# RinceWND/extPOM

Measured on AMD Instinct MI355X. Metric: 3D cell-updates/sec on internal mode (one internal step = the 3-D baroclinic step and its isplit 2-D external substeps; whole-step wall time), higher is better.
Workload: dtype f64

## Files before the change

### extpom_amd/csrc/k_adv.hip

```cpp
#include "pomgpu_internal.hpp"

#define dt_(i, j) F2(dt, i, j)
#define dx_(i, j) F2(dx, i, j)
#define dy_(i, j) F2(dy, i, j)
#define h_(i, j) F2(h, i, j)
#define u_(i, j, k) F3(u, i, j, k)
#define v_(i, j, k) F3(v, i, j, k)
#define ub_(i, j, k) F3(ub, i, j, k)
#define vb_(i, j, k) F3(vb, i, j, k)
#define w_(i, j, k) F3(w, i, j, k)
#define aam_(i, j, k) F3(aam, i, j, k)

#define MARCH3(call)                                                                  \
  const int g_ = (int)(blockIdx.x * blockDim.x + threadIdx.x);    \
  const int L_ = g_ >> 6, xcd_ = L_ & 7, m_ = L_ >> 3;                                \
  const int bpl_ = P.g_bpl, nbx_ = P.g_nbx;                                           \
  const int p_ = m_ % bpl_, t_ = m_ / bpl_;                                           \
  const int k = t_ % P.kb + 1;                                                        \
  const int band_ = (t_ / P.kb) * 8 + xcd_;                                           \
  const int i = (p_ % nbx_) * 64 + (g_ & 63) + 1;                                     \
  const int j = band_ * P.g_rb + (p_ / nbx_) * 4 + (int)threadIdx.y + 1;              \
  if (i > P.iml || j > P.jml) return;                                                 \
  call;
__device__ __forceinline__ void c_advct_a(const KP &P, const int i, const int j, const int k);
// ... 286 lines not shown
  G3(a, i, j, k) = G3(a, i, j, k) * G2(m2, i, j);
}
__device__ __forceinline__ void c_smol(const KP &P, const int i, const int j, const int k, const double *ff);
__global__ void k_smol(KP P, const double *ff) {
  MARCH3(c_smol(P, i, j, k, ff))
}
__device__ __forceinline__ void c_smol(const KP &P, const int i, const int j, const int k, const double *ff) {
  if (i > P.im || j > P.jm) return;
  const double value_min = 1.e-9, epsilon = 1.0e-14;
  double *xm = P.s3[0], *ym = P.s3[1], *zw = P.s3[2];
  const double fc = G3(ff, i, j, k);
  if (k <= P.kbm1 && j >= 2 && j <= P.jmm1 && i >= 2) {
    const double fw = G3(ff, i - 1, j, k);
    double r = 0.;
    if (!(fc < value_min || fw < value_min)) {
      const double m = G3(xm, i, j, k);
      const double udx = fabs(m);
      const double u2dt = P.dti2 * m * m * 2. / (F2(aru, i, j) * (dt_(i - 1, j) + dt_(i, j)));
      const double mol = (fc - fw) / (fw + fc + epsilon);
      r = (udx - u2dt) * mol * P.sw;
      if (fabs(udx) < fabs(u2dt)) r = 0.;
    }
    G3(xm, i, j, k) = r;
  }
  if (k <= P.kbm1 && j >= 2 && i >= 2 && i <= P.imm1) {
    const double fs = G3(ff, i, j - 1, k);
    double r = 0.;
    if (!(fc < value_min || fs < value_min)) {
      const double m = G3(ym, i, j, k);
      const double vdy = fabs(m);
      const double v2dt = P.dti2 * m * m * 2. / (F2(arv, i, j) * (dt_(i, j - 1) + dt_(i, j)));
      const double mol = (fc - fs) / (fs + fc + epsilon);
      r = (vdy - v2dt) * mol * P.sw;
      if (fabs(vdy) < fabs(v2dt)) r = 0.;
    }
    G3(ym, i, j, k) = r;
  }
  if (k >= 2 && k <= P.kbm1 && i >= 2 && i <= P.imm1 && j >= 2 && j <= P.jmm1) {
    const double fu = G3(ff, i, j, k - 1);
    double r = 0.;
    if (!(fc < value_min || fu < value_min)) {
      const double m = G3(zw, i, j, k);
      const double wdz = fabs(m);
      const double w2dt = P.dti2 * m * m / (F1(dzz, k - 1) * dt_(i, j));
      const double mol = (fu - fc) / (fc + fu + epsilon);
      r = (wdz - w2dt) * mol * P.sw;
      if (fabs(wdz) < fabs(w2dt)) r = 0.;
    }
    G3(zw, i, j, k) = r;
  }
}
__device__ __forceinline__ void c_copy3(const KP &P, const int i, const int j, const int k, double *dst, const double *src);
__global__ void k_copy3(KP P, double *dst, const double *src) {
  MARCH3(c_copy3(P, i, j, k, dst, src))
}
__device__ __forceinline__ void c_copy3(const KP &P, const int i, const int j, const int k, double *dst, const double *src) {
  G3(dst, i, j, k) = G3(src, i, j, k);
}
__device__ __forceinline__ double advt2_xdiff(const KP &P, const double *fb, const double *fc, int i, int j, int k) {
  const double am = 0.5 * (aam_(i, j, k) + aam_(i - 1, j, k));
  return -am * (h_(i, j) + h_(i - 1, j)) * P.tprni *
         ((G3(fb, i, j, k) - G3(fc, i, j, k)) - (G3(fb, i - 1, j, k) - G3(fc, i - 1, j, k))) * F2(dum, i, j) *
         (dy_(i, j) + dy_(i - 1, j)) * 0.5 / (dx_(i, j) + dx_(i - 1, j));
}
__device__ __forceinline__ double advt2_ydiff(const KP &P, const double *fb, const double *fc, int i, int j, int k) {
  const double am = 0.5 * (aam_(i, j, k) + aam_(i, j - 1, k));
  return -am * (h_(i, j) + h_(i, j - 1)) * P.tprni *
         ((G3(fb, i, j, k) - G3(fc, i, j, k)) - (G3(fb, i, j - 1, k) - G3(fc, i, j - 1, k))) * F2(dvm, i, j) *
         (dx_(i, j) + dx_(i, j - 1)) * 0.5 / (dy_(i, j) + dy_(i, j - 1));
}
__device__ __forceinline__ void c_advt2_diff(const KP &P, const int i, const int j, const int k, const double *fb, const double *fc, double *ff);
__global__ void k_advt2_diff(KP P, const double *fb, const double *fc, double *ff) {
  MARCH3(c_advt2_diff(P, i, j, k, fb, fc, ff))
}
__device__ __forceinline__ void c_advt2_diff(const KP &P, const int i, const int j, const int k, const double *fb, const double *fc, double *ff) {
  if (k > P.kbm1 || i < 2 || i > P.imm1 || j < 2 || j > P.jmm1) return;
  G3(ff, i, j, k) = G3(ff, i, j, k) -
                    P.dti2 * (advt2_xdiff(P, fb, fc, i + 1, j, k) - advt2_xdiff(P, fb, fc, i, j, k) +
                              advt2_ydiff(P, fb, fc, i, j + 1, k) - advt2_ydiff(P, fb, fc, i, j, k)) /
                        ((h_(i, j) + F2(etf, i, j)) * F2(art, i, j));
}

__device__ __forceinline__ double dens_point(const KP &P, double si, double ti, int i, int j, int k);
template <int TAU> __device__ __forceinline__ void c_ts_update(const KP &P, const int i, const int j, const int k, double fold, double fnew, int rt, int store_rst, double tau_b, double tau_f);
template <int TAU> __global__ void k_ts_update(KP P, double fold, double fnew, int rt, int store_rst, double tau_b, double tau_f) {
  MARCH3(c_ts_update<TAU>(P, i, j, k, fold, fnew, rt, store_rst, tau_b, tau_f))
}
__global__ void k_ts_update_same(KP P, double fold, double fnew, int rt, int store_rst) {
  MARCH3(c_ts_update<2>(P, i, j, k, fold, fnew, rt, store_rst, 0., 0.))
}
template <int TAU> __device__ __forceinline__ void c_ts_update(const KP &P, const int i, const int j, const int k, double fold, double fnew, int rt, int store_rst, double tau_b, double tau_f) {
  const bool act = (i <= P.im && j <= P.jm), lev = (k <= P.kbm1);
  const pomgpu_ct m = F2(fsm, i, j);
  pomgpu_ct uf = F3(uf, i, j, k), vf = F3(vf, i, j, k);
  if (lev && act) {
    uf = uf * m;
    vf = vf * m;
  }
  pomgpu_ct tb = F3(tb, i, j, k), sb = F3(sb, i, j, k);
  if (rt) {
    const pomgpu_ct tc = F3(tclim, i, j, k), sc = F3(sclim, i, j, k);
    tb = (tb - tc) + tc;
    sb = (sb - sc) + sc;
  }
  const pomgpu_ct t0 = F3(t, i, j, k), s0 = F3(s, i, j, k);
  pomgpu_ct tbn = t0 + CT(.5) * CT(P.smoth) * (uf + tb - CT(2.) * t0);
  pomgpu_ct sbn = s0 + CT(.5) * CT(P.smoth) * (vf + sb - CT(2.) * s0);
  pomgpu_ct tn = uf, sn = vf;
  if (lev) {
    if (act) {
      const pomgpu_ct tr = CT(fold) * CT(F3(trstrb, i, j, k)) + CT(fnew) * CT(F3(trstrf, i, j, k));
      const pomgpu_ct sr = CT(fold) * CT(F3(srstrb, i, j, k)) + CT(fnew) * CT(F3(srstrf, i, j, k));
      pomgpu_ct ta;
      if (TAU == 1) ta = CT(fold) * CT(tau_b) + CT(fnew) * CT(tau_f);
      else if (TAU == 2) { const pomgpu_ct x = CT(F3(taurstrf, i, j, k)); ta = CT(fold) * x + CT(fnew) * x; }
      else ta = CT(fold) * CT(F3(taurstrb, i, j, k)) + CT(fnew) * CT(F3(taurstrf, i, j, k));
      if (store_rst) {
        F3(trstr, i, j, k) = tr;
        F3(srstr, i, j, k) = sr;
        F3(taurstr, i, j, k) = ta;
      }
      const pomgpu_ct c = CT(2.) * CT(P.dti) / CT(86400.);
      tn = tn + c * ta * (tr - tn);
      tbn = tbn + c * ta * (tr - tbn);
      sn = sn + c * ta * (sr - sn);
      sbn = sbn + c * ta * (sr - sbn);
    }
    tn = tn * m; tbn = tbn * m; sn = sn * m; sbn = sbn * m;
  }
  F3(t, i, j, k) = tn;
  F3(tb, i, j, k) = tbn;
  F3(s, i, j, k) = sn;
  F3(sb, i, j, k) = sbn;
  if (lev && act) F3(rho, i, j, k) = dens_point(P, sn, tn, i, j, k);
}
template <int NF> struct TrUpds { TrUpd u[NF]; };
template <int NF> __device__ __forceinline__ void c_tr_update(const KP &P, const int i, const int j, const int k, const TrUpds<NF> &A, int rt) {
  const bool msk = (i <= P.im && j <= P.jm && k <= P.kbm1);
  const double m = F2(fsm, i, j);
#pragma unroll
  for (int f = 0; f < NF; f++) {
    const TrUpd &u = A.u[f];
    double ff = G3(u.ff, i, j, k);
    if (msk) ff = ff * m;
    double fb = G3(u.fb, i, j, k);
    if (rt) {
      const double fc = G3(u.fc, i, j, k);
      fb = (fb - fc) + fc;
    }
    const double f0 = G3(u.f, i, j, k);
    G3(u.fb, i, j, k) = f0 + .5 * P.smoth * (ff + fb - 2. * f0);
    G3(u.f, i, j, k) = ff;
  }
}
template <int NF> __global__ void k_tr_update(KP P, TrUpds<NF> A, int rt) {
  MARCH3(c_tr_update<NF>(P, i, j, k, A, rt))
}
__device__ __forceinline__ void c_tr_source(const KP &P, const int i, const int j, const int k, double *ff, const double *fb, const double *fc, const double *q, double lam) {
  if (k > P.kbm1 || i > P.im || j > P.jm) return;
  double x = G3(fb, i, j, k);
  if (fc) { const double y = G3(fc, i, j, k); x = (x - y) + y; }
  const double a = lam * x;
  const double b = (q ? (double)G3(q, i, j, k) : 0.) - a;
  const double d = P.dti2 * b;
  G3(ff, i, j, k) = (double)G3(ff, i, j, k) + d;
}
__global__ void k_tr_source(KP P, double *ff, const double *fb, const double *fc, const double *q, double lam) {
  MARCH3(c_tr_source(P, i, j, k, ff, fb, fc, q, lam))
}
__device__ __forceinline__ void c_mask_ts(const KP &P, const int i, const int j, const int k);
__global__ void k_mask_ts(KP P) {
  MARCH3(c_mask_ts(P, i, j, k))
}
__device__ __forceinline__ void c_mask_ts(const KP &P, const int i, const int j, const int k) {
  if (k > P.kbm1 || i > P.im || j > P.jm) return;
  const double m = F2(fsm, i, j);
  F3(uf, i, j, k) = F3(uf, i, j, k) * m;
  F3(vf, i, j, k) = F3(vf, i, j, k) * m;
}
__device__ __forceinline__ void c_mask_uv(const KP &P, const int i, const int j, const int k);
__global__ void k_mask_uv(KP P) {
  MARCH3(c_mask_uv(P, i, j, k))
}
// ... 304 lines not shown
  const int iw = ia > 1 ? ia - 1 : 1, ie = ib < P.iml ? ib + 1 : P.iml;
  const double2 dx = *(const double2 *)&F2(dx, ia, j), dy = *(const double2 *)&F2(dy, ia, j);
#ifndef AAM_PLAIN_DIV
  const double2 rdx = *(const double2 *)&K2(RDX, ia, j), rdy = *(const double2 *)&K2(RDY, ia, j);
  const InvD dxa = {dx.x, rdx.x}, dya = {dy.x, rdy.x}, dxb = {dx.y, rdx.y}, dyb = {dy.y, rdy.y};
#endif
  auto lev = [&](int k) {
    AamLev L;
    L.u_s = LD2(A3(u), ia, j - 1, k); L.u_0 = LD2(A3(u), ia, j, k); L.u_n = LD2(A3(u), ia, j + 1, k);
    L.v_0 = LD2(A3(v), ia, j, k); L.v_n = LD2(A3(v), ia, j + 1, k);
    return L;
  };
  AamLev cur = lev(k0);
  for (int k = k0; k <= k1; k++) {
    const AamLev nxt = lev(k < k1 ? k + 1 : k1);
    const double2 u_s = cur.u_s, u_0 = cur.u_0, u_n = cur.u_n, v_0 = cur.v_0, v_n = cur.v_n;
    const double uE_s = halo_e(u_s.x, [&] { return u_(ie, j - 1, k); }), uE_0 = halo_e(u_0.x, [&] { return u_(ie, j, k); }),
                 uE_n = halo_e(u_n.x, [&] { return u_(ie, j + 1, k); });
    const double vE_0 = halo_e(v_0.x, [&] { return v_(ie, j, k); }), vE_n = halo_e(v_n.x, [&] { return v_(ie, j + 1, k); });
    const double vW_0 = halo_w(v_0.y, [&] { return v_(iw, j, k); }), vW_n = halo_w(v_n.y, [&] { return v_(iw, j + 1, k); });
#ifndef AAM_PLAIN_DIV
    const double aa = aam_point_r(P, dxa, dya, u_0.x, u_0.y, u_n.x, u_n.y, u_s.x, u_s.y, v_0.x, v_n.x, v_0.y, v_n.y, vW_0, vW_n);
    const double ab = aam_point_r(P, dxb, dyb, u_0.y, uE_0, u_n.y, uE_n, u_s.y, uE_s, v_0.y, v_n.y, vE_0, vE_n, v_0.x, v_n.x);
#else
    const double aa = aam_point(P, dx.x, dy.x, u_0.x, u_0.y, u_n.x, u_n.y, u_s.x, u_s.y, v_0.x, v_n.x, v_0.y, v_n.y, vW_0, vW_n);
    const double ab = aam_point(P, dx.y, dy.y, u_0.y, uE_0, u_n.y, uE_n, u_s.y, uE_s, v_0.y, v_n.y, vE_0, vE_n, v_0.x, v_n.x);
#endif
    if (out && ia0 >= 2 && ia0 <= P.imm1) F3(aam, ia0, j, k) = aa;
    if (out && ia0 + 1 <= P.imm1) F3(aam, ia0 + 1, j, k) = ab;
    cur = nxt;
  }
}
#undef LD2
#undef A3


void launch_advct_a(pomgpu_ctx *c) { LAUNCH(c, k_advct_a, gridm(c->P), blk2(), c->P); }
void launch_advct_b(pomgpu_ctx *c) { LAUNCH(c, k_advct_b, gridm(c->P), blk2(), c->P); }
void launch_advct_c(pomgpu_ctx *c) { LAUNCH(c, k_advct_c, gridm(c->P), blk2(), c->P); }
void launch_aam(pomgpu_ctx *c) {
  const KP &P = c->P;
#ifdef POMGPU_STORE_F32
  const bool pair_ok = false;
#else
  const bool pair_ok = true;
#endif
  if (pair_ok && P.iml % 2 == 0 && !SW(c, NO_PAIR)) {
    const long nbands = (P.jml + P.g_rb - 1) / P.g_rb, rounds = (nbands + 7) / 8;
    const long bpl = (long)((P.iml / 2 + 61) / 62) * (P.g_rb / 4);
    const long nch = (P.kbm1 + AAM_KCH - 1) / AAM_KCH;
    LAUNCHN(c, "k_aam_pair", k_aam_pair, dim3((unsigned)(8 * rounds * nch * bpl), 1, 1), blk2(), c->P);
  } else {
    LAUNCH(c, k_aam, gridm(c->P), blk2(), c->P);
  }
}
void launch_roundtrip(pomgpu_ctx *c, double *a, const double *b, int fix_kb) { LAUNCH(c, k_roundtrip, gridm(c->P), blk2(), c->P, a, b, fix_kb); }
void launch_roundtrip_level(pomgpu_ctx *c, double *a, const double *b, int k) { LAUNCH(c, k_roundtrip_level, grid2(c->P), blk2(), c->P, a, b, k); }
void launch_advq_flux(pomgpu_ctx *c, const double *q, const double *qb, double *xf, double *yf) {
  LAUNCH(c, k_advq_flux, gridm(c->P), blk2(), c->P, q, qb, xf, yf);
}
void launch_advq_step(pomgpu_ctx *c, const double *q, const double *qb, double *qf, const double *xf, const double *yf, int zero_else) {
  LAUNCH(c, k_advq_step, gridm(c->P), blk2(), c->P, q, qb, qf, xf, yf, zero_else);
}
void launch_q_filter(pomgpu_ctx *c, int mask) { LAUNCH(c, k_q_filter, gridm(c->P), blk2(), c->P, mask); }
void launch_q_filter_rim(pomgpu_ctx *c) {
  const KP &P = c->P;
  const int len = P.im > P.jm ? P.im : P.jm;
  LAUNCH(c, k_q_filter_rim, dim3((len + 63) / 64, 8, P.kb), dim3(64, 1, 1), c->P);
}
void launch_mask_q(pomgpu_ctx *c) { LAUNCH(c, k_mask_q, gridm(c->P), blk2(), c->P); }
void launch_advt1(pomgpu_ctx *c, double *fb, double *f, const double *fclim, double *ff) {
  LAUNCH(c, k_advt1, gridm(c->P), blk2(), c->P, (const double *)fb, (const double *)f, fclim, ff);
  LAUNCH(c, k_copy_kb, grid2(c->P), blk2(), c->P, f, (double *)NULL);
}
void launch_copy_kb(pomgpu_ctx *c, double *f, double *g) { LAUNCH(c, k_copy_kb, grid2(c->P), blk2(), c->P, f, g); }
void launch_advt2_mass(pomgpu_ctx *c) { LAUNCH(c, k_advt2_mass, gridm(c->P), blk2(), c->P); }
void launch_advt2_step(pomgpu_ctx *c, const double *fbmem, const double *f, const double *eta, double *ff, int itera) {
  LAUNCH(c, k_advt2_step, gridm(c->P), blk2(), c->P, fbmem, f, eta, ff, itera);
}
void launch_mask3(pomgpu_ctx *c, double *a, const double *m2) { LAUNCH(c, k_mask3, gridm(c->P), blk2(), c->P, a, m2); }
void launch_smol(pomgpu_ctx *c, const double *ff) { LAUNCH(c, k_smol, gridm(c->P), blk2(), c->P, ff); }
void launch_copy3(pomgpu_ctx *c, double *dst, const double *src) { LAUNCH(c, k_copy3, gridm(c->P), blk2(), c->P, dst, src); }
void launch_advt2_diff(pomgpu_ctx *c, const double *fb, const double *fc, double *ff) { LAUNCH(c, k_advt2_diff, gridm(c->P), blk2(), c->P, fb, fc, ff); }
void launch_ts_update(pomgpu_ctx *c, double fold, double fnew, int rt, int store_rst) {
  if (c->tau_known[0] && c->tau_known[1] && !c->tau_handed && !SW(c, TAU_ARRAYS))
    LAUNCHN(c, "k_ts_update", (k_ts_update<1>), gridm(c->P), blk2(), c->P, fold, fnew, rt, store_rst, c->tau_val[0], c->tau_val[1]);
  else if (c->tau_same && !c->tau_handed && !SW(c, TAU_ARRAYS))
    LAUNCH(c, k_ts_update_same, gridm(c->P), blk2(), c->P, fold, fnew, rt, store_rst);
  else
    LAUNCHN(c, "k_ts_update", (k_ts_update<0>), gridm(c->P), blk2(), c->P, fold, fnew, rt, store_rst, 0., 0.);
}
void launch_restore_fields(pomgpu_ctx *c, double fold, double fnew) { LAUNCH(c, k_restore_fields, gridm(c->P), blk2(), c->P, fold, fnew); }
void launch_mask_ts(pomgpu_ctx *c) { LAUNCH(c, k_mask_ts, gridm(c->P), blk2(), c->P); }
void launch_tr_update(pomgpu_ctx *c, const TrUpd *u, int nf, int rt) {
  if (nf == 2) {
    TrUpds<2> A; A.u[0] = u[0]; A.u[1] = u[1];
    LAUNCHN(c, "k_tr_update2", (k_tr_update<2>), gridm(c->P), blk2(), c->P, A, rt);
  } else {
    TrUpds<1> A; A.u[0] = u[0];
    LAUNCHN(c, "k_tr_update", (k_tr_update<1>), gridm(c->P), blk2(), c->P, A, rt);
  }
}
void launch_tr_source(pomgpu_ctx *c, double *ff, const double *fb, const double *fc, const double *q, double lam) {
  LAUNCH(c, k_tr_source, gridm(c->P), blk2(), c->P, ff, fb, fc, q, lam);
}
void launch_mask_uv(pomgpu_ctx *c) { LAUNCH(c, k_mask_uv, gridm(c->P), blk2(), c->P); }
void launch_mask_w(pomgpu_ctx *c) { LAUNCH(c, k_mask_w, gridm(c->P), blk2(), c->P); }
void launch_restore(pomgpu_ctx *c, double fold, double fnew) { LAUNCH(c, k_restore, gridm(c->P), blk2(), c->P, fold, fnew); }
void launch_restore_shift(pomgpu_ctx *c) { LAUNCH(c, k_restore_shift, gridm(c->P), blk2(), c->P); }
void launch_restore_load(pomgpu_ctx *c, const double *tr, const double *sr, double tau, const double *taur, int fill_tau) { LAUNCH(c, k_restore_load, gridm(c->P), blk2(), c->P, tr, sr, tau, taur, fill_tau); }
void launch_probe_gpow15(pomgpu_ctx *c, long n, const double *x, double *out) { LAUNCH(c, k_probe_gpow15, dim3((unsigned)((n + 255) / 256), 1, 1), dim3(256, 1, 1), n, x, out); }
void launch_dens(pomgpu_ctx *c, const double *si, const double *ti, double *rhoo) { LAUNCH(c, k_dens, gridm(c->P), blk2(), c->P, si, ti, rhoo); }
void launch_realvertvl(pomgpu_ctx *c, int etf_is_et) {
  if (SW(c, REALVERTVL_CELLS)) LAUNCH(c, k_realvertvl, gridm(c->P), blk2(), c->P, etf_is_et);
  else LAUNCHN(c, "k_realvertvl_col", k_realvertvl_col, grid2(c->P), blk2(), c->P, etf_is_et);
}
```

### extpom_amd/csrc/k_tile.hip

```cpp
#include "pomgpu_internal.hpp"


__global__ void k_coef_static(KP P) {
  const int i = TID_I, j = TID_J;
  if (i > P.iml || j > P.jml) return;
  const int iw = i > 1 ? i - 1 : 1, js = j > 1 ? j - 1 : 1;
  P.m8[IX2(i, j)] = (unsigned char)((F2(fsm, i, j) != 0. ? 1 : 0) | (F2(dum, i, j) != 0. ? 2 : 0) | (F2(dvm, i, j) != 0. ? 4 : 0));
  K2(HSX, i, j) = F2(h, i, j) + F2(h, iw, j);
  K2(HSY, i, j) = F2(h, i, j) + F2(h, i, js);
  K2(DYSX, i, j) = F2(dy, i, j) + F2(dy, iw, j);
  K2(DXSX, i, j) = F2(dx, i, j) + F2(dx, iw, j);
  K2(DXSY, i, j) = F2(dx, i, j) + F2(dx, i, js);
  K2(DYSY, i, j) = F2(dy, i, j) + F2(dy, i, js);
  K2(DX4, i, j) = F2(dx, i, j) + F2(dx, iw, j) + F2(dx, i, js) + F2(dx, iw, js);
  K2(DY4, i, j) = F2(dy, i, j) + F2(dy, iw, j) + F2(dy, i, js) + F2(dy, iw, js);
  const int ie = i < P.iml ? i + 1 : P.iml, jn = j < P.jml ? j + 1 : P.jml;
  K2(CVA, i, j) = F2(dy, ie, j) - F2(dy, iw, j);
  K2(CVB, i, j) = F2(dx, i, jn) - F2(dx, i, js);
  K2(R2DXSX, i, j) = 2.0 / (F2(dx, i, j) + F2(dx, iw, j));
  K2(R2DYSY, i, j) = 2.0 / (F2(dy, i, j) + F2(dy, i, js));
  K2(RDX, i, j) = 1.0 / F2(dx, i, j);
  K2(RDY, i, j) = 1.0 / F2(dy, i, j);
  if (j == 1)
    for (int n = i - 1; n < POM_NBLK1D * P.kb; n += P.iml) P.r1[n] = 1.0 / P.b1[n];
}
__global__ void k_coef_dt(KP P) {
  const int i = TID_I, j = TID_J;
  if (i > P.iml || j > P.jml) return;
  const int iw = i > 1 ? i - 1 : 1, js = j > 1 ? j - 1 : 1;
  K2(CMX, i, j) = 0.25 * (F2(dy, iw, j) + F2(dy, i, j)) * (F2(dt, iw, j) + F2(dt, i, j));
  K2(CMY, i, j) = 0.25 * (F2(dx, i, js) + F2(dx, i, j)) * (F2(dt, i, js) + F2(dt, i, j));
  K2(DTSX, i, j) = F2(dt, i, j) + F2(dt, iw, j);
  K2(DTSY, i, j) = F2(dt, i, j) + F2(dt, i, js);
  K2(DT4, i, j) = F2(dt, i, j) + F2(dt, iw, j) + F2(dt, i, js) + F2(dt, iw, js);
}
__global__ void k_coef_eta(KP P, int uvm) {
  const int i = TID_I, j = TID_J;
  if (i > P.iml || j > P.jml) return;
  K2(HEA, i, j) = (F2(h, i, j) + F2(etb, i, j)) * F2(art, i, j);
  K2(HFA, i, j) = (F2(h, i, j) + F2(etf, i, j)) * F2(art, i, j);
  if (uvm) {
    const unsigned long long mb = UVM_MARK;
    double mark;
    __builtin_memcpy(&mark, &mb, sizeof mark);
    const int iw = i > 1 ? i - 1 : 1, js = j > 1 ? j - 1 : 1;
    const double cu = (F2(utb, i, j) + F2(utf, i, j)) / (F2(dt, i, j) + F2(dt, iw, j));
    const double cv = (F2(vtb, i, j) + F2(vtf, i, j)) / (F2(dt, i, j) + F2(dt, i, js));
    K2(UCOR, i, j) = (i >= 2 && i <= P.im && j <= P.jm) ? cu : mark;
    K2(VCOR, i, j) = (j >= 2 && j <= P.jm && i <= P.im) ? cv : mark;
  }
}

__device__ __forceinline__ pomgpu_ct upw_(pomgpu_ct m, pomgpu_ct lo, pomgpu_ct hi) {
  return CT(0.5) * ((m + fabs(m)) * lo + (m - fabs(m)) * hi);
}
struct FaceT { pomgpu_ct adv, dif; };
struct TFields { const double *fb[2], *f[2], *fcl[2]; double *ff[2]; };
template <int NF> struct LevT { pomgpu_ct c[2 * NF + 2], o[2], h[ROWSHARE_SLOTS(2 * NF + 2)]; };
template <int NS> struct NbrT { pomgpu_ct s[NS], n[NS]; };
struct CoefT { pomgpu_ct cm, hs, msk, ds_num; InvDc den; };
__device__ __forceinline__ CoefT coef_x(const KP &P, int i, int j) {
  CoefT c; c.cm = K2(CMX, i, j); c.hs = K2(HSX, i, j); c.msk = F2(dum, i, j); c.ds_num = K2(DYSX, i, j); c.den = inv_of(CT(K2(DXSX, i, j))); return c;
}
__device__ __forceinline__ CoefT coef_y(const KP &P, int i, int j) {
  CoefT c; c.cm = K2(CMY, i, j); c.hs = K2(HSY, i, j); c.msk = F2(dvm, i, j); c.ds_num = K2(DXSY, i, j); c.den = inv_of(CT(K2(DYSY, i, j))); return c;
}
__device__ __forceinline__ FaceT advt2_face(const pomgpu_ct tprni, const CoefT &c, pomgpu_ct vel, pomgpu_ct fb_hi, pomgpu_ct fb_lo, pomgpu_ct fc_hi,
                                            pomgpu_ct fc_lo, pomgpu_ct am_hi, pomgpu_ct am_lo) {
  FaceT f;
  f.adv = upw_(c.cm * vel, fb_lo, fb_hi);
  const pomgpu_ct am = CT(0.5) * (am_hi + am_lo);
  f.dif = divi(-am * c.hs * tprni * ((fb_hi - fc_hi) - (fb_lo - fc_lo)) * c.msk * c.ds_num * CT(0.5), c.den);
  return f;
}
#if COL_WX != 1
#error "the row-sharing column kernels keep one wavefront per workgroup row (COL_WX == 1)"
#endif
template <int NF, bool UM = false>
__global__ void __launch_bounds__(64 * LDS_ROWS) k_advt2_col(KP P, TFields A) {
  constexpr int NS = 2 * NF + 2, NH = ROWSHARE_SLOTS(NS), AM = 2 * NF, VV = 2 * NF + 1;
  HALO_XCD_DECODE_R(LDS_ROWS)
  const int r = WAVE_UNIFORM((int)threadIdx.y), j0w = j - r;
  const bool jrow = j <= P.jml;
  const int jc = jrow ? j : P.jml;
  const bool icol = jrow && (lane >= 1 && lane <= 62 && i0 <= P.iml);
#ifdef POMGPU_EMU
  if (!icol) return;
#endif
  const int i = i0 < 1 ? 1 : (i0 > P.iml ? P.iml : i0);
  const int iw = i > 1 ? i - 1 : 1, ie = i < P.iml ? i + 1 : P.iml;
  const int js = jc > 1 ? jc - 1 : 1, jn = jc < P.jml ? jc + 1 : P.jml;
  const bool in = icol && (i >= 2 && i <= P.imm1 && jc >= 2 && jc <= P.jmm1);
  const pomgpu_ct fsm = F2(fsm, i, jc);
  const CoefT cw = coef_x(P, i, jc), cs = coef_y(P, i, jc), cn = coef_y(P, i, jn);
  const pomgpu_ct art = F2(art, i, jc), hea = K2(HEA, i, jc);
  const InvDc hfa = inv_of(CT(K2(HFA, i, jc)));
  const pomgpu_ct tprni = P.tprni, dti2 = P.dti2;
  BufA bs[NS], bo[2], bff[NF], bh[NH];
  const double *ps[NS];
#pragma unroll
  for (int f = 0; f < NF; f++) { ps[f] = A.fb[f]; ps[NF + f] = A.fcl[f]; bff[f] = BUF3(A.ff[f]); }
  ps[AM] = A3(aam); ps[VV] = A3(v); bo[0] = BUF3(A3(u)); bo[1] = BUF3(A3(w));
#pragma unroll
  for (int x = 0; x < NS; x++) bs[x] = BUF3(ps[x]);
  const RowShare<NS> S = rowshare_setup<NS>(P, r, j, j0w, i);
#pragma unroll
  for (int q = 0; q < NH; q++) bh[q] = BUF3(rowshare_pick<NS>(ps, S.hop[q]));
  const UvmC mu = UM ? uvm_of<0>(P, i, jc) : uvm_none(), mv = UM ? uvm_of<1>(P, i, jc) : uvm_none();
  UvmC mh[NH];
#pragma unroll
  for (int q = 0; q < NH; q++) mh[q] = UM ? rowshare_uvm<1, NS, LDS_ROWS>(P, S, q, VV, j0w, i) : uvm_none();
  const unsigned oc = BOFF2(i, jc), lvb = LVB;
  const unsigned ost = in ? oc : BOFF_NONE;
#ifndef POMGPU_EMU
  __shared__ pomgpu_ct slab[2][NS][ROWSHARE_ROWS][64];
#else
  const unsigned os = BOFF2(i, js), on = BOFF2(i, jn);
#endif
  auto load = [&](LevT<NF> &L, unsigned lv) {
#pragma unroll
    for (int x = 0; x < NS; x++) L.c[x] = bldc(bs[x], oc, lv);
    L.o[0] = bldc(bo[0], oc, lv); L.o[1] = bldc(bo[1], oc, lv);
#pragma unroll
    for (int q = 0; q < NH; q++) L.h[q] = bldc(bh[q], S.hoff[q], lv);
  };
  pomgpu_ct f1[NF];
#pragma unroll
  for (int f = 0; f < NF; f++) f1[f] = G3(A.f[f], i, jc, 1);
  const int kbm1 = P.kbm1;
  pomgpu_ct p_adv[NF], p_dif[NF], p_fb[NF], p_zu[NF];
#pragma unroll
  for (int f = 0; f < NF; f++) p_adv[f] = p_dif[f] = p_fb[f] = p_zu[f] = 0.;
  auto step = [&](const int L, const int par, const LevT<NF> &cur, LevT<NF> &nxt) {
    load(nxt, (unsigned)(L < kbm1 ? L : kbm1 - 1) * lvb);
    NbrT<NS> nb;
    const pomgpu_ct v_c = uvm_fix(cur.c[VV], mv);
#ifndef POMGPU_EMU
#pragma unroll
    for (int x = 0; x < NS; x++) slab[par][x][r + 1][lane] = x == VV ? v_c : cur.c[x];
#pragma unroll
    for (int q = 0; q < NH; q++) slab[par][S.hop[q]][S.hrow[q]][lane] = uvm_fix(cur.h[q], mh[q]);
    __syncthreads();
#pragma unroll
    for (int x = 0; x < NS; x++) { nb.s[x] = slab[par][x][S.ss][lane]; nb.n[x] = slab[par][x][S.sn][lane]; }
#else
    const unsigned lvc = (unsigned)((L <= kbm1 ? L : kbm1) - 1) * lvb;
#pragma unroll
    for (int x = 0; x < NS; x++) { nb.s[x] = bldc(bs[x], os, lvc); nb.n[x] = bldc(bs[x], on, lvc); }
    nb.s[VV] = uvm_fix(nb.s[VV], uvm_of<1>(P, i, js)); nb.n[VV] = uvm_fix(nb.n[VV], uvm_of<1>(P, i, jn));
#endif
    const pomgpu_ct am_c = cur.c[AM], u_c = uvm_fix(cur.o[0], mu), w_c = cur.o[1];
    const pomgpu_ct am_w = halo_w(am_c, [&] { return F3(aam, iw, jc, L); });
    InvDc dzk; dzk.b = dzk.y = 0.;
    if (L >= 2) { dzk.b = F1(dz, L - 1); dzk.y = R1(dz, L - 1); }
#pragma unroll
    for (int f = 0; f < NF; f++) {
      const pomgpu_ct fb_c = cur.c[f], fc_c = cur.c[NF + f];
      pomgpu_ct zu = 0.;
      pomgpu_ct s_adv = 0., s_dif = 0.;
      if (L <= kbm1) {
        const pomgpu_ct fb_w = halo_w(fb_c, [&] { return G3(A.fb[f], iw, jc, L); });
        const pomgpu_ct fc_w = halo_w(fc_c, [&] { return G3(A.fcl[f], iw, jc, L); });
        const FaceT xw = advt2_face(tprni, cw, u_c, fb_c, fb_w, fc_c, fc_w, am_c, am_w);
        auto east = [&] {
          return advt2_face(tprni, coef_x(P, ie, jc), uvm_ld<0>(P, ie, jc, L), G3(A.fb[f], ie, jc, L), fb_c, G3(A.fcl[f], ie, jc, L), fc_c,
                            F3(aam, ie, jc, L), am_c);
        };
        FaceT xe;
        xe.adv = halo_e(xw.adv, [&] { return east().adv; });
        xe.dif = halo_e(xw.dif, [&] { return east().dif; });
        const FaceT ys = advt2_face(tprni, cs, v_c, fb_c, nb.s[f], fc_c, nb.s[NF + f], am_c, nb.s[AM]);
        const FaceT yn = advt2_face(tprni, cn, nb.n[VV], nb.n[f], fb_c, nb.n[NF + f], fc_c, nb.n[AM], am_c);
        s_adv = xe.adv - xw.adv + yn.adv - ys.adv;
        s_dif = xe.dif - xw.dif + yn.dif - ys.dif;
        zu = (L == 1) ? w_c * f1[f] * art : upw_(w_c, fb_c, p_fb[f]) * art;
      }
      {
        pomgpu_ct rr = p_adv[f] + divi(p_zu[f] - zu, dzk);
        rr = divi(p_fb[f] * hea - dti2 * rr, hfa);
        rr = rr * fsm;
        rr = rr - divi(dti2 * p_dif[f], hfa);
        bstc(bff[f], (L >= 2 && L <= kbm1 + 1) ? ost : BOFF_NONE, (unsigned)(L >= 2 ? L - 2 : 0) * lvb, rr);
      }
      p_adv[f] = s_adv; p_dif[f] = s_dif; p_fb[f] = fb_c; p_zu[f] = zu;
    }
  };
  LevT<NF> ra, rb;
  load(ra, 0u);
  rb = ra;
  for (int L = 1; L <= kbm1 + 1; L += 2) {
    step(L, 1, ra, rb);
    step(L + 1, 0, rb, ra);
  }
  if (icol) {
    for (int k = in ? P.kb : 1; k <= P.kb; k++) {
#pragma unroll
      for (int f = 0; f < NF; f++) G3(A.ff[f], i, jc, k) = CT(G3(A.ff[f], i, jc, k)) * fsm;
    }
  }
}

struct QFields { const double *q[2], *qb[2]; double *qf[2]; };
template <int NF, int NO = 2> struct LevQa { pomgpu_ct c[2 * NF + 2], o[NO], h[ROWSHARE_SLOTS(2 * NF + 2)]; };
struct CoefQ { pomgpu_ct dts, hs, msk, ds_num; InvDc den; };
__device__ __forceinline__ CoefQ coefq_x(const KP &P, int i, int j) {
  CoefQ c; c.dts = K2(DTSX, i, j); c.hs = K2(HSX, i, j); c.msk = F2(dum, i, j); c.den = inv_of(CT(K2(DXSX, i, j))); c.ds_num = K2(DYSX, i, j); return c;
}
__device__ __forceinline__ CoefQ coefq_y(const KP &P, int i, int j) {
  CoefQ c; c.dts = K2(DTSY, i, j); c.hs = K2(HSY, i, j); c.msk = F2(dvm, i, j); c.den = inv_of(CT(K2(DYSY, i, j))); c.ds_num = K2(DXSY, i, j); return c;
}
__device__ __forceinline__ pomgpu_ct advq_face(const CoefQ &c, pomgpu_ct q_hi, pomgpu_ct q_lo, pomgpu_ct vel_k, pomgpu_ct vel_km1, pomgpu_ct am_hi_k,
                                               pomgpu_ct am_lo_k, pomgpu_ct am_hi_m, pomgpu_ct am_lo_m, pomgpu_ct qb_hi, pomgpu_ct qb_lo) {
  pomgpu_ct x = CT(.125) * (q_hi + q_lo) * c.dts * (vel_k + vel_km1);
  x = x - divi(CT(.25) * (am_hi_k + am_lo_k + am_hi_m + am_lo_m) * c.hs * (qb_hi - qb_lo) * c.msk, c.den);
  return CT(.5) * c.ds_num * x;
}
template <int NF, bool WF = false, bool UM = false>
__global__ void __launch_bounds__(64 * LDS_ROWS) k_advq_col(KP P, QFields A, int zero_else) {
  constexpr int NS = 2 * NF + 2, NH = ROWSHARE_SLOTS(NS), AM = 2 * NF, VV = 2 * NF + 1;
  typedef LevQa<NF, WF ? 1 : 2> Lev;
  HALO_XCD_DECODE_R(LDS_ROWS)
  const int r = WAVE_UNIFORM((int)threadIdx.y), j0w = j - r;
  const bool jrow = j <= P.jml;
  const int jc = jrow ? j : P.jml;
  const bool icol = jrow && (lane >= 1 && lane <= 62 && i0 <= P.iml);
#ifdef POMGPU_EMU
  if (!icol) return;
#endif
  const int i = i0 < 1 ? 1 : (i0 > P.iml ? P.iml : i0);
  const int iw = i > 1 ? i - 1 : 1, ie = i < P.iml ? i + 1 : P.iml;
  const int js = jc > 1 ? jc - 1 : 1, jn = jc < P.jml ? jc + 1 : P.jml;
  const bool in = icol && (i >= 2 && i <= P.imm1 && jc >= 2 && jc <= P.jmm1);
  const CoefQ cw = coefq_x(P, i, jc), cs = coefq_y(P, i, jc), cn = coefq_y(P, i, jn);
  const pomgpu_ct art = F2(art, i, jc), hea = K2(HEA, i, jc);
  const InvDc hfa = inv_of(CT(K2(HFA, i, jc)));
  const int kb = P.kb, kbm1 = P.kbm1;
  BufA bs[NS], bo[2], bqf[NF], bh[NH];
// ... 510 lines not shown
    bstc(buf, ost, lv, ru);
    bstc(bvf, ost, lv, rv);
    fu_k = fu_n; fv_k = fv_n;
    u_k = u_c; v_k = v_c;
  };
  LevUV ra, rb;
  load(ra, 1);
  rb = ra;
  for (int k = 1; k <= kbm1; k += 6) {
    step(k, 1, ra, rb);
    if (k + 1 <= kbm1) step(k + 1, 2, rb, ra);
    if (k + 2 <= kbm1) step(k + 2, 0, ra, rb);
    if (k + 3 <= kbm1) step(k + 3, 1, rb, ra);
    if (k + 4 <= kbm1) step(k + 4, 2, ra, rb);
    if (k + 5 <= kbm1) step(k + 5, 0, rb, ra);
  }
  if (out) { F3(uf, i, jc, kb) = 0.; F3(vf, i, jc, kb) = 0.; }
}

void launch_coef_static(pomgpu_ctx *c) { LAUNCH(c, k_coef_static, grid2(c->P), blk2(), c->P); }
void launch_coef_dt(pomgpu_ctx *c) { LAUNCH(c, k_coef_dt, grid2(c->P), blk2(), c->P); }
void launch_coef_eta(pomgpu_ctx *c, int uvm) { LAUNCH(c, k_coef_eta, grid2(c->P), blk2(), c->P, uvm); }
void launch_advq_col(pomgpu_ctx *c, const double *q, const double *qb, double *qf, int zero_else) {
  QFields A; A.q[0] = A.q[1] = q; A.qb[0] = A.qb[1] = qb; A.qf[0] = A.qf[1] = qf;
  LAUNCHN(c, "k_advq_col", (k_advq_col<1>), grid1_halo_r(c->P, LDS_ROWS), blk_col_r(LDS_ROWS), c->P, A, zero_else);
}
void launch_advq2_col(pomgpu_ctx *c, const double *q, const double *qb, double *qf, const double *ql, const double *qlb, double *qlf, int zero_else) {
  QFields A; A.q[0] = q; A.qb[0] = qb; A.qf[0] = qf; A.q[1] = ql; A.qb[1] = qlb; A.qf[1] = qlf;
  LAUNCHN(c, "k_advq2_col", (k_advq_col<2>), grid1_halo_r(c->P, LDS_ROWS), blk_col_r(LDS_ROWS), c->P, A, zero_else);
}
#if POMGPU_W_FUSE
void launch_advq2w_col(pomgpu_ctx *c, const double *q, const double *qb, double *qf, const double *ql, const double *qlb, double *qlf, int zero_else) {
  QFields A; A.q[0] = q; A.qb[0] = qb; A.qf[0] = qf; A.q[1] = ql; A.qb[1] = qlb; A.qf[1] = qlf;
#if POMGPU_UVM_ONLOAD
  if (c->P.uvm) { LAUNCHN(c, "k_advq2_col", (k_advq_col<2, true, true>), grid1_halo_r(c->P, LDS_ROWS), blk_col_r(LDS_ROWS), c->P, A, zero_else); return; }
#endif
  LAUNCHN(c, "k_advq2_col", (k_advq_col<2, true>), grid1_halo_r(c->P, LDS_ROWS), blk_col_r(LDS_ROWS), c->P, A, zero_else);
}
#endif
void launch_advct_col(pomgpu_ctx *c, int sum2d) {
  const bool rows4 = SW(c, ADVCT_ROWS4) || (!SW(c, ADVCT_ROWS8) && c->P.jml <= 400 && c->exch);
  sum2d = (sum2d ? 1 : 0) | (POMGPU_UVM_ONLOAD && !c->exch && !c->tp.on && !c->wide.on && !(c->flags & POMGPU_CTX_2D) ? 2 : 0);
  if (rows4) LAUNCHN(c, "k_advct_col", (k_advct_col<4>), grid1_halo_r(c->P, 4), blk_col_r(4), c->P, sum2d);
  else LAUNCHN(c, "k_advct_col", (k_advct_col<LDS_ROWS>), grid1_halo_r(c->P, LDS_ROWS), blk_col_r(LDS_ROWS), c->P, sum2d);
}
__global__ void k_advct_fix2d(KP P, int west, int south) {
  const int t = TID_I;
  if (west && t >= 2 && t <= P.jmm1) {
    double a = 0.;
#pragma unroll 8
    for (int k = 1; k <= P.kbm1; k++) a = a + F3(advx, 2, t, k) * F1(dz, k);
    F2(adx2d, 2, t) = a;
  }
  if (south && t >= 2 && t <= P.imm1) {
    double a = 0.;
#pragma unroll 8
    for (int k = 1; k <= P.kbm1; k++) a = a + F3(advy, t, 2, k) * F1(dz, k);
    F2(ady2d, t, 2) = a;
  }
}
void launch_advct_fix2d(pomgpu_ctx *c, int west, int south) {
  const KP &P = c->P;
  const int len = P.im > P.jm ? P.im : P.jm;
  LAUNCH(c, k_advct_fix2d, dim3((len + 63) / 64, 1, 1), dim3(64, 1, 1), c->P, west, south);
}
void launch_advct_edge(pomgpu_ctx *c, double *to_e, double *to_n) {
  const KP &P = c->P;
  const int len = P.im > P.jm ? P.im : P.jm;
  LAUNCH(c, k_advct_edge, dim3((len + 63) / 64, P.kbm1, 1), dim3(64, 1, 1), c->P, to_e, to_n);
}
void launch_advct_fix(pomgpu_ctx *c, const double *from_w, const double *from_s) {
  const KP &P = c->P;
  const int len = P.im > P.jm ? P.im : P.jm;
  LAUNCH(c, k_advct_fix, dim3((len + 63) / 64, P.kbm1, 1), dim3(64, 1, 1), c->P, from_w, from_s);
}
void launch_advuv_col(pomgpu_ctx *c) {
#if POMGPU_UVM_ONLOAD
  if (c->P.uvm) { LAUNCHN(c, "k_advuv_col", (k_advuv_col<true>), grid1_halo_r(c->P, LDS_ROWS), blk_col_r(LDS_ROWS), c->P); return; }
#endif
  LAUNCHN(c, "k_advuv_col", (k_advuv_col<false>), grid1_halo_r(c->P, LDS_ROWS), blk_col_r(LDS_ROWS), c->P);
}
void launch_advt2_rows(pomgpu_ctx *c, const double *fb, const double *f, const double *fc, double *ff) {
  {
    TFields A; A.fb[0] = A.fb[1] = fb; A.f[0] = A.f[1] = f; A.fcl[0] = A.fcl[1] = fc; A.ff[0] = A.ff[1] = ff;
#if POMGPU_UVM_ONLOAD
    if (c->P.uvm) { LAUNCHN(c, "k_advt2_col", (k_advt2_col<1, true>), grid1_halo_r(c->P, LDS_ROWS), blk_col_r(LDS_ROWS), c->P, A); return; }
#endif
    LAUNCHN(c, "k_advt2_col", (k_advt2_col<1>), grid1_halo_r(c->P, LDS_ROWS), blk_col_r(LDS_ROWS), c->P, A);
  }
}
void launch_advt2x2_col(pomgpu_ctx *c, const double *tb, const double *t, const double *tc, double *tf, const double *sb, const double *s_,
                        const double *sc, double *sf) {
  TFields A; A.fb[0] = tb; A.f[0] = t; A.fcl[0] = tc; A.ff[0] = tf; A.fb[1] = sb; A.f[1] = s_; A.fcl[1] = sc; A.ff[1] = sf;
#if POMGPU_UVM_ONLOAD
  if (c->P.uvm) { LAUNCHN(c, "k_advt2x2_col", (k_advt2_col<2, true>), grid1_halo_r(c->P, LDS_ROWS), blk_col_r(LDS_ROWS), c->P, A); return; }
#endif
  LAUNCHN(c, "k_advt2x2_col", (k_advt2_col<2>), grid1_halo_r(c->P, LDS_ROWS), blk_col_r(LDS_ROWS), c->P, A);
}
```

### extpom_amd/csrc/k_vert.hip

```cpp
#include <type_traits>
#include "pomgpu_internal.hpp"
#include "dd_exp.h"

#define dt_(i, j) F2(dt, i, j)
#define dx_(i, j) F2(dx, i, j)
#define dy_(i, j) F2(dy, i, j)
#define h_(i, j) F2(h, i, j)
#define u_(i, j, k) F3(u, i, j, k)
#define v_(i, j, k) F3(v, i, j, k)
#define w_(i, j, k) F3(w, i, j, k)

#define ROWS_PROFUV 1
#define ROWS_PROFT 1
#ifndef ROWS_UVF
#define ROWS_UVF 8
#endif
#ifndef ROWS_UVM
#define ROWS_UVM 4
#endif
#define COL2                               \
  const int i = TID_I, j = TID_J;          \
  if (i > P.iml || j > P.jml) return;

__global__ void k_baropg(KP P, int sum2d) {
  COL2
  if (i < 2 || i > P.imm1 || j < 2 || j > P.jmm1) {
    if (sum2d) {
      double rx = 0., ry = 0.;
      if (i <= P.im && j <= P.jm)
        for (int k = 1; k <= P.kbm1; k++) {
          const double dzk = F1(dz, k);
          rx = rx + F3(drhox, i, j, k) * dzk;
          ry = ry + F3(drhoy, i, j, k) * dzk;
        }
      F2(drx2d, i, j) = rx;
      F2(dry2d, i, j) = ry;
    }
    return;
  }
  const double dtc = dt_(i, j), dtw = dt_(i - 1, j), dts = dt_(i, j - 1);
  const double sx = .25 * (dtc + dtw), sy = .25 * (dtc + dts);
  const double mx = F2(dum, i, j), my = F2(dvm, i, j);
  const double ex = dy_(i, j) + dy_(i - 1, j), ey = dx_(i, j) + dx_(i, j - 1);
  double rc0 = F3(rho, i, j, 1) - F3(rmean, i, j, 1);
  double rw0 = F3(rho, i - 1, j, 1) - F3(rmean, i - 1, j, 1);
  double rs0 = F3(rho, i, j - 1, 1) - F3(rmean, i, j - 1, 1);
  double ax = .5 * P.grav * (-F1(zz, 1)) * (dtc + dtw) * (rc0 - rw0);
  double ay = .5 * P.grav * (-F1(zz, 1)) * (dtc + dts) * (rc0 - rs0);
  double ox = P.ramp * (sx * ax * mx * ex), oy = P.ramp * (sy * ay * my * ey);
  F3(drhox, i, j, 1) = ox;
  F3(drhoy, i, j, 1) = oy;
  double rx = 0., ry = 0.;
  rx = rx + ox * F1(dz, 1);
  ry = ry + oy * F1(dz, 1);
  for (int k = 2; k <= P.kbm1; k++) {
    PACE_BARRIER();
    const double rc = F3(rho, i, j, k) - F3(rmean, i, j, k);
    const double rw = F3(rho, i - 1, j, k) - F3(rmean, i - 1, j, k);
    const double rs = F3(rho, i, j - 1, k) - F3(rmean, i, j - 1, k);
    const double zm = F1(zz, k - 1) - F1(zz, k), zp = F1(zz, k - 1) + F1(zz, k);
    ax = ax + P.grav * .25 * zm * (dtc + dtw) * (rc - rw + rc0 - rw0) +
         P.grav * .25 * zp * (dtc - dtw) * (rc + rw - rc0 - rw0);
    ay = ay + P.grav * .25 * zm * (dtc + dts) * (rc - rs + rc0 - rs0) +
         P.grav * .25 * zp * (dtc - dts) * (rc + rs - rc0 - rs0);
    ox = P.ramp * (sx * ax * mx * ex); oy = P.ramp * (sy * ay * my * ey);
    F3(drhox, i, j, k) = ox;
    F3(drhoy, i, j, k) = oy;
    rx = rx + ox * F1(dz, k);
    ry = ry + oy * F1(dz, k);
    rc0 = rc; rw0 = rw; rs0 = rs;
  }
  if (sum2d) { F2(drx2d, i, j) = rx; F2(dry2d, i, j) = ry; }
  F3(drhox, i, j, P.kb) = P.ramp * F3(drhox, i, j, P.kb);
  F3(drhoy, i, j, P.kb) = P.ramp * F3(drhoy, i, j, P.kb);
}

#ifndef BPG_ROWS
#define BPG_ROWS 16
#endif
static_assert(COL_WX == 1, "k_baropg_rs / k_vertvl_rs take threadIdx.y as the row inside the workgroup: one wavefront per workgroup row");
__global__ void __launch_bounds__(64 * BPG_ROWS) k_baropg_rs(KP P, int sum2d) {
  HALO_XCD_DECODE_R(BPG_ROWS)
  const int r = WAVE_UNIFORM((int)threadIdx.y);
  const bool jvalid = j <= P.jml;
  const int jc = jvalid ? j : P.jml;
  const bool own = jvalid && lane >= 1 && lane <= 62 && i0 >= 1 && i0 <= P.iml;
#ifdef POMGPU_EMU
  if (!own) return;
#endif
  const int i = i0 < 1 ? 1 : (i0 > P.iml ? P.iml : i0);
  const int iw = i > 1 ? i - 1 : 1, js = jc > 1 ? jc - 1 : 1;
  const bool in = own && i0 >= 2 && i0 <= P.imm1 && jc >= 2 && jc <= P.jmm1;
  const int kbm1 = P.kbm1;
  const double dtc = dt_(i, jc), dts = dt_(i, js);
  const double dtw = halo_w(dtc, [&] { return dt_(iw, jc); });
  const double sx = .25 * (dtc + dtw), sy = .25 * (dtc + dts);
  const double mx = F2(dum, i, jc), my = F2(dvm, i, jc);
  const double dyc = dy_(i, jc);
  const double ex = dyc + halo_w(dyc, [&] { return dy_(iw, jc); }), ey = dx_(i, jc) + dx_(i, js);
  const BufA brho = BUF3(A3(rho)), brm = BUF3(A3(rmean)), box = BUF3(A3(drhox)), boy = BUF3(A3(drhoy));
  const unsigned oc = BOFF2(i, jc), lvb = LVB;
  const unsigned osh = (r == 0) ? BOFF2(i, js) : BOFF_NONE;
  const unsigned ost = in ? oc : BOFF_NONE;
#ifndef POMGPU_EMU
  __shared__ double slab[2][BPG_ROWS + 1][64];
#endif
  struct Lev { double rho, rm, rho_s, rm_s; };
  auto load = [&](Lev &L, int k) {
    const unsigned lv = (unsigned)WAVE_UNIFORM(k - 1) * lvb;
    L.rho = bld(brho, oc, lv); L.rm = bld(brm, oc, lv);
    L.rho_s = bld(brho, osh, lv); L.rm_s = bld(brm, osh, lv);
  };
  double rc0 = 0., rw0 = 0., rs0 = 0., ax = 0., ay = 0., rx = 0., ry = 0.;
  auto step = [&](const int k, const Lev &cur, Lev &nxt) {
    const int par = k & 1;
    load(nxt, k + 2 <= kbm1 ? k + 2 : kbm1);
    const double rc = cur.rho - cur.rm;
#ifndef POMGPU_EMU
    slab[par][r + 1][lane] = rc;
    if (r == 0) slab[par][0][lane] = cur.rho_s - cur.rm_s;
    __syncthreads();
    const double rs = slab[par][r][lane];
#else
    (void)par;
    const double rs = F3(rho, i, js, k) - F3(rmean, i, js, k);
#endif
    const double rw = halo_w(rc, [&] { return F3(rho, iw, jc, k) - F3(rmean, iw, jc, k); });
    if (k == 1) {
      ax = .5 * P.grav * (-F1(zz, 1)) * (dtc + dtw) * (rc - rw);
      ay = .5 * P.grav * (-F1(zz, 1)) * (dtc + dts) * (rc - rs);
    } else {
      const double zm = F1(zz, k - 1) - F1(zz, k), zp = F1(zz, k - 1) + F1(zz, k);
      ax = ax + P.grav * .25 * zm * (dtc + dtw) * (rc - rw + rc0 - rw0) +
           P.grav * .25 * zp * (dtc - dtw) * (rc + rw - rc0 - rw0);
      ay = ay + P.grav * .25 * zm * (dtc + dts) * (rc - rs + rc0 - rs0) +
           P.grav * .25 * zp * (dtc - dts) * (rc + rs - rc0 - rs0);
    }
    const double ox = P.ramp * (sx * ax * mx * ex), oy = P.ramp * (sy * ay * my * ey);
    const unsigned lv = (unsigned)WAVE_UNIFORM(k - 1) * lvb;
    bst(box, ost, lv, ox);
    bst(boy, ost, lv, oy);
    rx = rx + ox * F1(dz, k);
    ry = ry + oy * F1(dz, k);
    rc0 = rc; rw0 = rw; rs0 = rs;
  };
  Lev ra, rb, rc_;
  load(ra, 1);
  load(rb, 2 <= kbm1 ? 2 : kbm1);
  rc_ = ra;
  for (int k = 1; k <= kbm1; k += 3) {
    step(k, ra, rc_);
    if (k + 1 <= kbm1) step(k + 1, rb, ra);
    if (k + 2 <= kbm1) step(k + 2, rc_, rb);
  }
  if (!own) return;
  if (in) {
    if (sum2d) { F2(drx2d, i, jc) = rx; F2(dry2d, i, jc) = ry; }
    F3(drhox, i, jc, P.kb) = P.ramp * F3(drhox, i, jc, P.kb);
    F3(drhoy, i, jc, P.kb) = P.ramp * F3(drhoy, i, jc, P.kb);
  } else if (sum2d) {
    double qx = 0., qy = 0.;
    if (i <= P.im && jc <= P.jm)
      for (int k = 1; k <= kbm1; k++) {
        const double dzk = F1(dz, k);
        qx = qx + F3(drhox, i, jc, k) * dzk;
        qy = qy + F3(drhoy, i, jc, k) * dzk;
      }
    F2(drx2d, i, jc) = qx;
    F2(dry2d, i, jc) = qy;
  }
}

#define RA(ii, jj, kk) (F3(rho, ii, jj, kk) - F3(rmean, ii, jj, kk))
__global__ void k_order_pack(KP P, double *send_e, double *send_n) {
  const int t = TID_I, k = (int)blockIdx.y;
  if (t <= P.jml && send_e) send_e[(size_t)k * P.jml + (t - 1)] = k == 0 ? F2(d, P.iml - 2, t) : RA(P.iml - 2, t, k);
  if (t <= P.iml && send_n) send_n[(size_t)k * P.iml + (t - 1)] = k == 0 ? F2(d, t, P.jml - 2) : RA(t, P.jml - 2, k);
}
__global__ void k_baropg_mcc(KP P, int sum2d) {
  COL2
  if (i < 2 || i > P.imm1 || j < 2 || j > P.jmm1) {
    if (sum2d) {
      double rx = 0., ry = 0.;
      if (i <= P.im && j <= P.jm)
        for (int k = 1; k <= P.kbm1; k++) {
          const double dzk = F1(dz, k);
          rx = rx + F3(drhox, i, j, k) * dzk;
          ry = ry + F3(drhoy, i, j, k) * dzk;
        }
      F2(drx2d, i, j) = rx;
      F2(dry2d, i, j) = ry;
    }
    return;
  }
  const double c24 = (double)(1.f / 24.f), c16 = (double)(1.f / 16.f);
  const bool cx = (i >= (P.W ? 3 : 2)), cy = (j >= (P.S ? 3 : 2));
  const bool gx = (i == 2), gy = (j == 2);
  const double *gw3 = P.g4[0], *gs3 = P.g4[1], *gw2 = P.g4[2], *gs2 = P.g4[3];
  const int iww = gx ? 1 : i - 2, jss = gy ? 1 : j - 2;
  const double mxc = F2(dum, i, j), mxe = F2(dum, i + 1, j), mxw = F2(dum, i - 1, j);
  const double myc = F2(dvm, i, j), myn = F2(dvm, i, j + 1), mys = F2(dvm, i, j - 1);
  const double dc = F2(d, i, j), de = F2(d, i + 1, j), dw = F2(d, i - 1, j), dn = F2(d, i, j + 1), ds = F2(d, i, j - 1);
  const double dww = gx ? gw2[j - 1] : F2(d, iww, j), dss = gy ? gs2[i - 1] : F2(d, i, jss);
  double ddxx = (dc - dw) * mxc, d4x = .5 * (dc + dw) * mxc;
  if (cx) {
    ddxx = ddxx - c24 * (mxe * (de - dc) - 2 * (dc - dw) + mxw * (dw - dww));
    d4x = d4x + c16 * (mxe * (dc - de) + mxw * (dw - dww));
  }
  double ddxy = (dc - ds) * myc, d4y = .5 * (dc + ds) * myc;
  if (cy) {
    ddxy = ddxy - c24 * (myn * (dn - dc) - 2 * (dc - ds) + mys * (ds - dss));
    d4y = d4y + c16 * (myn * (dc - dn) + mys * (ds - dss));
  }
  const double sx = .25 * (dt_(i, j) + dt_(i - 1, j)), ex = dy_(i, j) + dy_(i - 1, j);
  const double sy = .25 * (dt_(i, j) + dt_(i, j - 1)), ey = dx_(i, j) + dx_(i, j - 1);
  double ax = 0., ay = 0., drx_m = 0., rux_m = 0., dry_m = 0., ruy_m = 0., rx = 0., ry = 0.;
  for (int k = 1; k <= P.kbm1; k++) {
    const double rc = RA(i, j, k), re = RA(i + 1, j, k), rw = RA(i - 1, j, k), rn = RA(i, j + 1, k), rs = RA(i, j - 1, k);
    const double rww = gx ? gw3[(size_t)(k - 1) * P.jml + (j - 1)] : RA(iww, j, k);
    const double rss = gy ? gs3[(size_t)(k - 1) * P.iml + (i - 1)] : RA(i, jss, k);
    double drx = (rc - rw) * mxc, rux = 0.5 * (rc + rw) * mxc;
    if (cx) {
      drx = drx - c24 * (mxe * (re - rc) - 2 * (rc - rw) + mxw * (rw - rww));
      rux = rux + c16 * (mxe * (rc - re) + mxw * (rw - rww));
    }
    double dry = (rc - rs) * myc, ruy = .5 * (rc + rs) * myc;
    if (cy) {
      dry = dry - c24 * (myn * (rn - rc) - 2 * (rc - rs) + mys * (rs - rss));
      ruy = ruy + c16 * (myn * (rc - rn) + mys * (rs - rss));
    }
    if (k == 1) {
      ax = P.grav * (-F1(zz, 1)) * d4x * drx;
      ay = P.grav * (-F1(zz, 1)) * d4y * dry;
    } else {
      ax = ax + P.grav * 0.5 * F1(dzz, k - 1) * d4x * (drx_m + drx) +
           P.grav * 0.5 * (F1(zz, k - 1) + F1(zz, k)) * ddxx * (rux - rux_m);
      ay = ay + P.grav * 0.5 * F1(dzz, k - 1) * d4y * (dry_m + dry) +
           P.grav * 0.5 * (F1(zz, k - 1) + F1(zz, k)) * ddxy * (ruy - ruy_m);
// ... 142 lines not shown
  double cc = 1449.1 + .00821 * p + 4.55 * tp - .045 * sq(tp) + 1.34 * (sp - 35.0);
  cc = cc / sqrt((1. - .01642 * p / cc) * (1. - 0.40 * p / sq(cc)));
  return cc;
}
__device__ __forceinline__ double profq_cc_v(const KP &P, double t, double s_, double hij, int k) {
  const double tp = t + P.tbias;
  const double sp = s_ + P.sbias;
  const double p = P.grav * P.rhoref * (-F1(zz, k) * hij) * 1.e-4;
  double cc = 1449.1 + .00821 * p + 4.55 * tp - .045 * sq(tp) + 1.34 * (sp - 35.0);
  cc = cc / sqrt((1. - .01642 * p / cc) * (1. - 0.40 * p / sq(cc)));
  return cc;
}
__device__ __forceinline__ double profq_rho(const KP &P, int i, int j, int k, int rho_rt) {
  const double r = F3(rho, i, j, k);
  if (!rho_rt) return r;
  const double m = F3(rmean, i, j, k);
  return (r - m) + m;
}
__device__ __forceinline__ double profq_boygr(const KP &P, int i, int j, int k, double ccm, double cck, int rho_rt = 0) {
  return P.grav * (profq_rho(P, i, j, k - 1, rho_rt) - profq_rho(P, i, j, k, rho_rt)) / (F1(dzz, k - 1) * h_(i, j)) +
         sq(P.grav) * 2. / (sq(ccm) + sq(cck));
}
__global__ void k_profq_prod(KP P, int rho_rt) {
  COL2
  if (i > P.im || j > P.jm) return;
  double *prod = P.s3[0];
  G3(prod, i, j, 1) = 0.;
  G3(prod, i, j, P.kb) = 0.;
  const bool in = (i >= 2 && i <= P.imm1 && j >= 2 && j <= P.jmm1);
  if (!in) {
    for (int k = 2; k <= P.kbm1; k++) G3(prod, i, j, k) = 0.;
    return;
  }
  const double dh = h_(i, j) + F2(etf, i, j);
  const double sef = 1., shiw = 0.;
  double ccm = profq_cc(P, i, j, 1);
  for (int k = 2; k <= P.kbm1; k++) {
    const double cck = profq_cc(P, i, j, k);
    const double bg = profq_boygr(P, i, j, k, ccm, cck, rho_rt);
    const double km = F3(km, i, j, k);
    double p = km * .25 * sef *
                   (sq(u_(i, j, k) - u_(i, j, k - 1) + u_(i + 1, j, k) - u_(i + 1, j, k - 1)) +
                    sq(v_(i, j, k) - v_(i, j, k - 1) + v_(i, j + 1, k) - v_(i, j + 1, k - 1))) /
                   sq(F1(dzz, k - 1) * dh) -
               shiw * km * bg;
    p = p + F3(kh, i, j, k) * bg;
    G3(prod, i, j, k) = p;
    ccm = cck;
  }
}
__global__ void k_profq_prod_lines(KP P, int rho_rt) {
  const int t = TID_I, line = (int)blockIdx.y, k = (int)blockIdx.z + 1;
  int i, j;
  if (line < 4) { if (t > P.jm) return; j = t; i = line == 0 ? 1 : (line == 1 ? 2 : (line == 2 ? P.imm1 : P.im)); }
  else { if (t > P.im) return; i = t; j = line == 4 ? 1 : (line == 5 ? 2 : (line == 6 ? P.jmm1 : P.jm)); }
  double *prod = P.s3[0];
  double p = 0.;
  const bool wanted = line == 1 ? !P.W : (line == 2 ? !P.E : (line == 5 ? !P.S : (line == 6 ? !P.N : true)));
  if (!wanted) return;
  if (k >= 2 && k <= P.kbm1 && i >= 2 && i <= P.imm1 && j >= 2 && j <= P.jmm1) {
    const double dh = h_(i, j) + F2(etf, i, j);
    const double sef = 1., shiw = 0.;
    const double ccm = profq_cc(P, i, j, k - 1), cck = profq_cc(P, i, j, k);
    const double bg = profq_boygr(P, i, j, k, ccm, cck, rho_rt);
    const double km = F3(km, i, j, k);
    p = km * .25 * sef *
            (sq(u_(i, j, k) - u_(i, j, k - 1) + u_(i + 1, j, k) - u_(i + 1, j, k - 1)) +
             sq(v_(i, j, k) - v_(i, j, k - 1) + v_(i, j + 1, k) - v_(i, j + 1, k - 1))) /
            sq(F1(dzz, k - 1) * dh) -
        shiw * km * bg;
    p = p + F3(kh, i, j, k) * bg;
  }
  G3(prod, i, j, k) = p;
}
struct LevQ { double t, s, rho, rm, q2b, q2lb, q2, km, kh, uf, vf, uc, ue, vc, vn, kq1, prod; };
struct LevB { double e1, g1, e2, g2, qb, qlb, q, ql; };
#ifndef PROFQ_KL
#define PROFQ_KL 19
#endif
#ifndef PROFQ_BIG
#define PROFQ_BIG 8
#endif
template <int FP, int FF, int ROWS, int LD = 1>
__global__ void __launch_bounds__(64 * ROWS) k_profq(KP P, int rho_rt_pace, int jfirst, int jlast) {
#ifndef POMGPU_EMU
  constexpr int KL = ROWS >= 8 ? PROFQ_KL : (PROFQ_KL < 9 ? PROFQ_KL : 9);
  __shared__ double evec[2 * KL][ROWS][64];
#endif
  const int i = TID_I, j = TID_J + jfirst - 1;
  if (i > P.iml || j > P.jml || j > jlast) return;
  const int rho_rt = rho_rt_pace & 1, pace = rho_rt_pace & 2;
  const int ty = (int)threadIdx.y, tx = (int)threadIdx.x;
  if (i > P.im || j > P.jm) return;
  const double a1 = 0.92, b1 = 16.6, a2 = 0.74, b2 = 10.1, c1 = 0.08, e1 = 1.8, e2 = 1.33, surfl = 2.e5;
  const int kb = P.kb, kbm1 = P.kbm1;
  const double dh = h_(i, j) + F2(etf, i, j);
  const double utau2 = G2(P.s2[4], i, j);
  const double l0 = surfl * utau2 / P.grav;
  const double umol2 = 2. * P.umol;
  const double z1 = F1(z, 1), zkb = F1(z, kb);
  const double coef4 = 18. * a1 * a1 + 9. * a1 * a2, coef5 = 9. * a1 * a2;
  const double coef1 = a2 * (1. - 6. * a1 / b1 * 1.), coef2 = 3. * a2 * b2 / 1. + 18. * a1 * a2,
               coef3 = a1 * (1. - 3. * c1 - 6. * a1 / b1 * 1.);
  const bool repl = (P.W && i == 1) || (P.E && i == P.im) || (P.S && j == 1) || (P.N && j == P.jm);
  const int ti = (P.W && i == 2) ? 1 : ((P.E && i == P.imm1) ? P.im : 0);
  const int tj = (P.S && j == 2) ? 1 : ((P.N && j == P.jmm1) ? P.jm : 0);
  const double fsm_c = F2(fsm, i, j);
  const double m_ti = F2(fsm, ti ? ti : i, j), m_tj = F2(fsm, i, tj ? tj : j), m_tij = F2(fsm, ti ? ti : i, tj ? tj : j);
  const bool pin = FP && (i >= 2 && i <= P.imm1 && j >= 2 && j <= P.jmm1);
  const bool ffil = FF && (i >= 3 && i <= P.imm1 - 1 && j >= 3 && j <= P.jmm1 - 1);
  const int ie = i < P.iml ? i + 1 : i, jn = j < P.jml ? j + 1 : j;
  const double hij = h_(i, j);
  const InvD dhk = inv_of(dh * P.kappa);
  UvmC m_uc = uvm_none(), m_ue = uvm_none(), m_vc = uvm_none(), m_vn = uvm_none();
#if POMGPU_UVM_ONLOAD
  if (FP == 1 && P.uvm) {
    m_uc.s = K2(USUM, i, j); m_uc.c = K2(UCOR, i, j); m_ue.s = K2(USUM, ie, j); m_ue.c = K2(UCOR, ie, j);
    m_vc.s = K2(VSUM, i, j); m_vc.c = K2(VCOR, i, j); m_vn.s = K2(VSUM, i, jn); m_vn.c = K2(VCOR, i, jn);
    m_uc.on = m_ue.on = m_vc.on = m_vn.on = true;
  }
#endif
#define bt BUF3(A3(t))
#define bs_ BUF3(A3(s))
#define brho BUF3(A3(rho))
#define bq2b BUF3(A3(q2b))
#define bq2lb BUF3(A3(q2lb))
#define bq2 BUF3(A3(q2))
#define bq2l BUF3(A3(q2l))
#define bkm BUF3(A3(km))
#define bkh BUF3(A3(kh))
#define bkq BUF3(A3(kq))
#define buf BUF3(A3(uf))
#define bvf BUF3(A3(vf))
#define bu BUF3(A3(u))
#define bv BUF3(A3(v))
#define bl BUF3(A3(l))
#define bdt BUF3(A3(dtef))
#define bpr BUF3(P.s3[0])
#define be1 BUF3(P.s3[4])
#define be2 BUF3(P.s3[5])
  const unsigned oc = BOFF2(i, j), oe = BOFF2(ie, j), on = BOFF2(i, jn), lvb = LVB;
  const unsigned o_k = repl ? BOFF_NONE : oc;
  const unsigned o_abs = ffil ? BOFF_NONE : oc;
  const unsigned o_fil = ffil ? oc : BOFF_NONE, o_uv = ffil ? BOFF_NONE : oc;
  const unsigned o_pr = (FP == 0 || (FP == 2 && !pin)) ? oc : BOFF_NONE;
  const unsigned o_rm = rho_rt ? oc : BOFF_NONE;
#ifdef PROFQ_OLDWALK
  const double vbot = P.kappa * (1 + F1(z, kbm1)) * dh * F3(q2, i, j, kbm1);
  const double ufbot = F3(uf, i, j, kb);
#else
  double ufbot;
#endif
  double e1p = 0., g1p = P.cb_profq * utau2;
  double e2p = 0., g2p = 0.;
  double ccm = 0., rhom = 0.;
  double kqm = 0., kqc = F3(kq, i, j, 1);
  double ucm = 0., uem = 0., vcm = 0., vnm = 0.;
#ifdef PROFQ_OLDWALK
  auto lev = [&](LevQ &L, int k) {
    const unsigned lv = (unsigned)WAVE_UNIFORM(k - 1) * lvb;
    L.t = bld(bt, oc, lv); L.s = bld(bs_, oc, lv); L.rho = bld(brho, oc, lv); L.rm = bld(BUF3(A3(rmean)), o_rm, lv);
    L.q2b = bld(bq2b, oc, lv); L.q2lb = bld(bq2lb, oc, lv); L.q2 = bld(bq2, oc, lv);
    L.km = bld(bkm, oc, lv); L.kh = bld(bkh, oc, lv);
    L.uf = bld(buf, oc, lv); L.vf = bld(bvf, oc, lv);
    if (FP) { L.uc = bld(bu, oc, lv); L.ue = bld(bu, oe, lv); L.vc = bld(bv, oc, lv); L.vn = bld(bv, on, lv); }
    else L.uc = L.ue = L.vc = L.vn = 0.;
    L.kq1 = bld(bkq, oc, (unsigned)WAVE_UNIFORM(k < kb ? k : kb - 1) * lvb);
    L.prod = (FP != 1) ? bld(bpr, o_pr, lv) : 0.;
  };
  auto step = [&](const int k, const LevQ &cur, LevQ &nxt) {
    lev(nxt, k + 1 <= kb ? k + 1 : kb);
    const bool mid = (k >= 2 && k <= kbm1);
    const unsigned lv = (unsigned)WAVE_UNIFORM(k - 1) * lvb;
    const double kqp = cur.kq1;
    double cck = 0., rhok = 0.;
    if (k <= kbm1) { cck = profq_cc_v(P, cur.t, cur.s, hij, k); rhok = rho_rt ? (cur.rho - cur.rm) + cur.rm : cur.rho; }
    double q2b = cur.q2b;
    double l, gh = 0.;
    double uck = 0., uek = 0., vck = 0., vnk = 0., bg = 0.;
    if (pin && k <= kbm1) { uck = uvm_fix(cur.uc, m_uc); uek = uvm_fix(cur.ue, m_ue); vck = uvm_fix(cur.vc, m_vc); vnk = uvm_fix(cur.vn, m_vn); }
    double q2lb = 0.;
    if (mid) {
      q2b = fabs(q2b);
      q2lb = fabs(cur.q2lb);
      bg = P.grav * (rhom - rhok) / (F1(dzz, k - 1) * hij) + sq(P.grav) * 2. / (sq(ccm) + sq(cck));
      l = fabs(q2lb / q2b);
      if (F1(z, k) > -0.5) l = fmax(l, P.kappa * l0);
      gh = fmin(sq(l) * bg / q2b, .028);
    } else {
      l = (k == 1) ? P.kappa * l0 : 0.;
    }
    bst(bq2b, mid ? o_abs : BOFF_NONE, lv, q2b);
    bst(bq2lb, mid ? o_abs : BOFF_NONE, lv, q2lb);
    if (LD) bst(bl, oc, lv, l);
    const double dtef1 = sqrt(fabs(q2b)) * 1. / (b1 * l + P.small_);
    double dtef2 = dtef1;
    if (mid) dtef2 = dtef1 * (1. + e2 * sq(divi((1. / fabs(F1(z, k) - z1) + 1. / fabs(F1(z, k) - zkb)) * l, dhk)));
    if (LD) bst(bdt, oc, lv, dtef2);
    if (mid) {
      const double a = -P.dti2 * (kqp + kqc + umol2) * .5 / (F1(dzz, k - 1) * F1(dz, k) * dh * dh);
      const double c = -P.dti2 * (kqm + kqc + umol2) * .5 / (F1(dzz, k - 1) * F1(dz, k - 1) * dh * dh);
      double pr;
      if (FP == 0 || (FP == 2 && !pin)) {
        pr = cur.prod;
      } else if (pin) {
        const double sef = 1., shiw = 0.;
        const double km = cur.km;
        pr = km * .25 * sef * (sq(uck - ucm + uek - uem) + sq(vck - vcm + vnk - vnm)) / sq(F1(dzz, k - 1) * dh) - shiw * km * bg;
        pr = pr + cur.kh * bg;
      } else {
        pr = 0.;
      }
      const double g = 1. / (a + c * (1. - e1p) - (2. * P.dti2 * dtef1 + 1.));
      e1p = a * g;
      g1p = (-2. * P.dti2 * pr + c * g1p - cur.uf) * g;
      if (k == 2) {
        e2p = 0.;
        g2p = -P.kappa * F1(z, 2) * dh * cur.q2;
      } else {
        const double rhs = (k == kbm1) ? vbot : cur.vf;
        const double g2 = 1. / (a + c * (1. - e2p) - (P.dti2 * dtef2 + 1.));
        e2p = a * g2;
        g2p = (P.dti2 * (-pr * l * e1) + c * g2p - rhs) * g2;
      }
    }
    {
      const unsigned ov = (k <= kbm1) ? oc : BOFF_NONE;
#ifndef POMGPU_EMU
      const bool inl = k <= KL;
      if (inl) { evec[k - 1][ty][tx] = e1p; evec[KL + k - 1][ty][tx] = e2p; }
      const unsigned oe_ = inl ? BOFF_NONE : ov;
#else
      const unsigned oe_ = ov;
#endif
      bst(be1, oe_, lv, e1p); bst(buf, ov, lv, g1p); bst(be2, oe_, lv, e2p); bst(bvf, ov, lv, g2p);
    }
    double kq_n = 0., km_n = 0., kh_n = 0.;
    {
      const double sh = coef1 / (1. - coef2 * gh);
      double sm = coef3 + sh * coef4 * gh;
      sm = sm / (1. - coef5 * gh);
      const double pl = l * sqrt(fabs(cur.q2));
      kq_n = (pl * .41 * sh + kqc) * .5;
      km_n = (pl * sm + cur.km) * .5;
      kh_n = (pl * sh + cur.kh) * .5;
      bst(bkq, o_k, lv, kq_n * fsm_c);
      bst(bkm, o_k, lv, km_n * fsm_c);
      bst(bkh, o_k, lv, kh_n * fsm_c);
    }
    if ((ti | tj) && !repl) {
#define PUT(ii, jj, m)                               \
  {                                                  \
    G3(P.s3[1], ii, jj, k) = km_n * m;               \
    G3(P.s3[2], ii, jj, k) = kh_n * m;               \
    G3(P.s3[3], ii, jj, k) = kq_n * m;               \
  }
      if (ti) PUT(ti, j, m_ti)
      if (tj) PUT(i, tj, m_tj)
      if (ti && tj) PUT(ti, tj, m_tij)
#undef PUT
    }
    ccm = cck; rhom = rhok;
    ucm = uck; uem = uek; vcm = vck; vnm = vnk;
    kqm = kqc; kqc = kqp;
  };
  {
    LevQ ra, rb;
    lev(ra, 1);
    rb = ra;
    for (int k = 1; k <= kb; k += 2) {
      if (pace) PACE_BARRIER();
      step(k, ra, rb);
      if (k + 1 <= kb) step(k + 1, rb, ra);
    }
  }
#else
  enum { PH_1, PH_2, PH_LDS, PH_MEM, PH_KBM1, PH_KB };
  auto lev = [&](LevQ &L, int k) {
    const unsigned lv = (unsigned)WAVE_UNIFORM(k - 1) * lvb;
    L.t = bld(bt, oc, lv); L.s = bld(bs_, oc, lv); L.rho = bld(brho, oc, lv); L.rm = bld(BUF3(A3(rmean)), o_rm, lv);
    L.q2b = bld(bq2b, oc, lv); L.q2lb = bld(bq2lb, oc, lv); L.q2 = bld(bq2, oc, lv);
    L.km = bld(bkm, oc, lv); L.kh = bld(bkh, oc, lv);
    L.uf = bld(buf, oc, lv); L.vf = bld(bvf, oc, lv);
    if (FP) { L.uc = bld(bu, oc, lv); L.ue = bld(bu, oe, lv); L.vc = bld(bv, oc, lv); L.vn = bld(bv, on, lv); }
    else L.uc = L.ue = L.vc = L.vn = 0.;
    L.kq1 = bld(bkq, oc, (unsigned)WAVE_UNIFORM(k < kb ? k : kb - 1) * lvb);
    L.prod = (FP != 1) ? bld(bpr, o_pr, lv) : 0.;
  };
  auto step = [&](auto ph, const int k, const LevQ &cur, LevQ &nxt) {
    constexpr int PH = decltype(ph)::value;
    constexpr bool mid = (PH != PH_1 && PH != PH_KB);
    if (PH != PH_KB) lev(nxt, k + 1);
    const unsigned lv = (unsigned)WAVE_UNIFORM(k - 1) * lvb;
    const double kqp = cur.kq1;
    double cck = 0., rhok = 0.;
    if (PH != PH_KB) { cck = profq_cc_v(P, cur.t, cur.s, hij, k); rhok = rho_rt ? (cur.rho - cur.rm) + cur.rm : cur.rho; }
    double q2b = cur.q2b;
    double l, gh = 0.;
    double uck = 0., uek = 0., vck = 0., vnk = 0., bg = 0.;
    if (PH != PH_KB) {
      uck = pin ? uvm_fix(cur.uc, m_uc) : 0.; uek = pin ? uvm_fix(cur.ue, m_ue) : 0.;
      vck = pin ? uvm_fix(cur.vc, m_vc) : 0.; vnk = pin ? uvm_fix(cur.vn, m_vn) : 0.;
    }
    double q2lb = 0.;
    if (mid) {
      q2b = fabs(q2b);
      q2lb = fabs(cur.q2lb);
      bg = P.grav * (rhom - rhok) / (F1(dzz, k - 1) * hij) + sq(P.grav) * 2. / (sq(ccm) + sq(cck));
      l = fabs(q2lb / q2b);
      const double lmx = fmax(l, P.kappa * l0);
      l = (F1(z, k) > -0.5) ? lmx : l;
      gh = fmin(sq(l) * bg / q2b, .028);
      bst(bq2b, o_abs, lv, q2b);
      bst(bq2lb, o_abs, lv, q2lb);
    } else {
      l = (PH == PH_1) ? P.kappa * l0 : 0.;
    }
    if (LD) bst(bl, oc, lv, l);
    const double dtef1 = sqrt(fabs(q2b)) * 1. / (b1 * l + P.small_);
    double dtef2 = dtef1;
    if (mid) dtef2 = dtef1 * (1. + e2 * sq(divi((1. / fabs(F1(z, k) - z1) + 1. / fabs(F1(z, k) - zkb)) * l, dhk)));
    if (LD) bst(bdt, oc, lv, dtef2);
    if (mid) {
      const double a = -P.dti2 * (kqp + kqc + umol2) * .5 / (F1(dzz, k - 1) * F1(dz, k) * dh * dh);
      const double c = -P.dti2 * (kqm + kqc + umol2) * .5 / (F1(dzz, k - 1) * F1(dz, k - 1) * dh * dh);
      double pr;
      if (FP == 0) {
        pr = cur.prod;
      } else {
        const double sef = 1., shiw = 0.;
        const double km = cur.km;
        pr = km * .25 * sef * (sq(uck - ucm + uek - uem) + sq(vck - vcm + vnk - vnm)) / sq(F1(dzz, k - 1) * dh) - shiw * km * bg;
        pr = pr + cur.kh * bg;
        pr = pin ? pr : (FP == 2 ? cur.prod : 0.);
      }
      const double g = 1. / (a + c * (1. - e1p) - (2. * P.dti2 * dtef1 + 1.));
      e1p = a * g;
      g1p = (-2. * P.dti2 * pr + c * g1p - cur.uf) * g;
      if (PH == PH_2) {
        e2p = 0.;
        g2p = -P.kappa * F1(z, 2) * dh * cur.q2;
      } else {
        const double rhs = (PH == PH_KBM1) ? P.kappa * (1 + F1(z, kbm1)) * dh * cur.q2 : cur.vf;
        const double g2 = 1. / (a + c * (1. - e2p) - (P.dti2 * dtef2 + 1.));
        e2p = a * g2;
        g2p = (P.dti2 * (-pr * l * e1) + c * g2p - rhs) * g2;
      }
    }
    if (PH != PH_KB) {
#ifndef POMGPU_EMU
      if (PH == PH_1 || PH == PH_2 || PH == PH_LDS) {
        evec[k - 1][ty][tx] = e1p; evec[KL + k - 1][ty][tx] = e2p;
      } else if (PH == PH_MEM) {
        bst(be1, oc, lv, e1p); bst(be2, oc, lv, e2p);
      } else {
        const bool inl = k <= KL;
        if (inl) { evec[k - 1][ty][tx] = e1p; evec[KL + k - 1][ty][tx] = e2p; }
        const unsigned oe_ = inl ? BOFF_NONE : oc;
        bst(be1, oe_, lv, e1p); bst(be2, oe_, lv, e2p);
      }
#else
      bst(be1, oc, lv, e1p); bst(be2, oc, lv, e2p);
#endif
      bst(buf, oc, lv, g1p); bst(bvf, oc, lv, g2p);
    }
    double kq_n = 0., km_n = 0., kh_n = 0.;
    {
      const double sh = coef1 / (1. - coef2 * gh);
      double sm = coef3 + sh * coef4 * gh;
      sm = sm / (1. - coef5 * gh);
      const double pl = l * sqrt(fabs(cur.q2));
      kq_n = (pl * .41 * sh + kqc) * .5;
      km_n = (pl * sm + cur.km) * .5;
      kh_n = (pl * sh + cur.kh) * .5;
      bst(bkq, o_k, lv, kq_n * fsm_c);
      bst(bkm, o_k, lv, km_n * fsm_c);
      bst(bkh, o_k, lv, kh_n * fsm_c);
    }
    if ((ti | tj) && !repl) {
// ... 804 lines not shown
        dk[k - 1] = d;
        if (k <= kbm1) {
          su = su + d * F1(dz, k);
          G3(c, i, j, k) = uf;
        }
      }
    }
    SCHED_FENCE();
  }
#pragma unroll
  for (int k = 1; k <= NL; k++)
    if (k <= kbm1) G3(b, i, j, k) = uo[k - 1] + .5 * P.smoth * (dk[k - 1] - su);
  G3(b, i, j, kb) = c_kb;
  G3(c, i, j, kb) = f_kb;
  if (V) F2(tps, i, j) = su;
#undef KC
}
template <int KBT>
__global__ void __launch_bounds__(64 * ROWS_UVF) k_uv_filter_reg2(KP P, int own) {
  if (blockIdx.z == 0) d_uv_filter_reg<KBT, 0>(P, own);
  else d_uv_filter_reg<KBT, 1>(P, own);
}

template <int V>
static __device__ __forceinline__ void d_uv_filter_rim(const KP &P) {
  const int t = (int)(blockIdx.x * blockDim.x + threadIdx.x), line = (int)blockIdx.y;
  int i, j;
  if (line == 0) {
    const int il = t & 7;
    j = (t >> 3) + 1;
    if (il == 7 || j > P.jm) return;
    i = il < 4 ? il + 1 : P.im - 6 + il;
  } else {
    i = t + 5;
    if (i > P.im - 3) return;
    j = line <= 4 ? line : P.jm - 7 + line;
  }
  const double *f = P.b3 + (size_t)(V ? P3_vf : P3_uf) * P.a3;
  double *b = P.b3 + (size_t)(V ? P3_vb : P3_ub) * P.a3, *c = P.b3 + (size_t)(V ? P3_v : P3_u) * P.a3;
  const int kb = P.kb, kbm1 = P.kbm1;
  constexpr int CH = 8;
  double xf[CH], xb[CH], xc[CH];
  const UvmC mc = uvm_of<V>(P, i, j);
#define KC(k) ((k) < kbm1 ? (k) : kbm1)
  double su = 0.;
  for (int k0 = 1; k0 <= kbm1; k0 += CH) {
#pragma unroll
    for (int q = 0; q < CH; q++) { xf[q] = G3(f, i, j, KC(k0 + q)); xb[q] = G3(b, i, j, KC(k0 + q)); xc[q] = G3(c, i, j, KC(k0 + q)); }
#pragma unroll
    for (int q = 0; q < CH; q++) xc[q] = uvm_fix(xc[q], mc);
#pragma unroll
    for (int q = 0; q < CH; q++)
      if (k0 + q <= kbm1) su = su + (xf[q] + xb[q] - 2. * xc[q]) * F1(dz, k0 + q);
  }
  for (int k0 = 1; k0 <= kbm1; k0 += CH) {
#pragma unroll
    for (int q = 0; q < CH; q++) { xf[q] = G3(f, i, j, KC(k0 + q)); xb[q] = G3(b, i, j, KC(k0 + q)); xc[q] = G3(c, i, j, KC(k0 + q)); }
#pragma unroll
    for (int q = 0; q < CH; q++) xc[q] = uvm_fix(xc[q], mc);
#pragma unroll
    for (int q = 0; q < CH; q++)
      if (k0 + q <= kbm1) {
        G3(b, i, j, k0 + q) = xc[q] + .5 * P.smoth * ((xf[q] + xb[q] - 2. * xc[q]) - su);
        G3(c, i, j, k0 + q) = xf[q];
      }
  }
  const double c_kb = G3(c, i, j, kb), f_kb = G3(f, i, j, kb);
  G3(b, i, j, kb) = c_kb;
  G3(c, i, j, kb) = f_kb;
  if (V) F2(tps, i, j) = su;
#undef KC
}
__global__ void k_uv_filter_rim(KP P) {
  if (blockIdx.z == 0) d_uv_filter_rim<0>(P);
  else d_uv_filter_rim<1>(P);
}

static inline dim3 colblk() { return dim3(64, 2, 1); }
static inline dim3 rowblk(int rows) { return dim3(64, rows, 1); }
static inline dim3 rowgrid(const KP &P, int rows) { return dim3((P.iml + 63) / 64, (P.jml + rows - 1) / rows, 1); }
static inline dim3 colgrid(const KP &P) { return dim3((P.iml + 63) / 64, (P.jml + 1) / 2, 1); }
#define COLV_G(P) dim3(((P).iml + 63) / 64, ((P).jml + 3) / 4, 1)
#define COLV_B dim3(64, 4, 1)
void launch_baropg(pomgpu_ctx *c, int sum2d) {
  if (SW(c, BAROPG_CELLS)) { LAUNCH(c, k_baropg, COLV_G(c->P), COLV_B, c->P, sum2d); return; }
  LAUNCHN(c, "k_baropg", k_baropg_rs, grid1_halo_r(c->P, BPG_ROWS), blk_col_r(BPG_ROWS), c->P, sum2d);
}
void launch_baropg_mcc(pomgpu_ctx *c, int sum2d) { LAUNCH(c, k_baropg_mcc, colgrid(c->P), colblk(), c->P, sum2d); }
void launch_order_pack(pomgpu_ctx *c, double *send_e, double *send_n) {
  const KP &P = c->P;
  const int len = P.iml > P.jml ? P.iml : P.jml;
  LAUNCH(c, k_order_pack, dim3((len + 63) / 64, P.kb + 1, 1), dim3(64, 1, 1), c->P, send_e, send_n);
}
static inline dim3 twin(dim3 g) { g.z = 2; return g; }
template <class F> static void with_kbt(int kb, F f) {
  if (kb <= 24) f(std::integral_constant<int, 24>{});
  else if (kb <= 32) f(std::integral_constant<int, 32>{});
  else if (kb <= 40) f(std::integral_constant<int, 40>{});
  else if (kb <= 44) f(std::integral_constant<int, 44>{});
  else if (kb <= 50) f(std::integral_constant<int, 50>{});
  else if (kb <= 56) f(std::integral_constant<int, 56>{});
  else f(std::integral_constant<int, 64>{});
}
#define KBT_OF(t) decltype(t)::value
void launch_int_uvmean(pomgpu_ctx *c) {
  if (!pomgpu_reg_kb(c)) { LAUNCH(c, k_int_uvmean, colgrid(c->P), colblk(), c->P); return; }
  with_kbt(c->P.kb, [&](auto t) { LAUNCHN(c, "k_int_uvmean_reg2", (k_int_uvmean_reg2<KBT_OF(t)>), twin(rowgrid(c->P, ROWS_UVM)), rowblk(ROWS_UVM), c->P); });
}
void launch_vertvl(pomgpu_ctx *c, int mask) {
  if (SW(c, VERTVL_CELLS)) { LAUNCH(c, k_vertvl, COLV_G(c->P), COLV_B, c->P, mask); return; }
  LAUNCHN(c, "k_vertvl", k_vertvl_rs, grid1_halo_r(c->P, VVL_ROWS), blk_col_r(VVL_ROWS), c->P, mask);
}
void launch_profq_bc(pomgpu_ctx *c) { LAUNCH(c, k_profq_bc, colgrid(c->P), colblk(), c->P); }
void launch_profq_prod(pomgpu_ctx *c, int lines_only, int rho_rt) {
  if (!lines_only) { LAUNCH(c, k_profq_prod, colgrid(c->P), colblk(), c->P, rho_rt); return; }
  const KP &P = c->P;
  const int len = P.im > P.jm ? P.im : P.jm;
  LAUNCH(c, k_profq_prod_lines, dim3((len + 63) / 64, 8, P.kb), dim3(64, 1, 1), c->P, rho_rt);
}
void launch_profq(pomgpu_ctx *c, int fuse_prod, int fuse_filter, int rho_rt, int jfirst, int jlast, int store_ld) {
  if (jlast < jfirst) { jfirst = 1; jlast = c->P.jml; }
  const int ld = store_ld || fuse_prod != 1 || !fuse_filter;
  if (ld && c->prof_on) {
    const int s = pomgpu_prof_slot(c, "profq_ld_store");
    if (s >= 0) (c->parent ? c->parent : c)->prof[s].launches++;
  }
  const int nrows = jlast - jfirst + 1;
  const int rows8 = !SW(c, PROFQ_ROWS2) && (SW(c, PROFQ_ROWS8) || (long)((c->P.iml + 63) / 64) * ((c->P.jml + 7) / 8) >= 3 * 256);
  rho_rt = (rho_rt ? 1 : 0) | (SW(c, PROFQ_NOPACE) ? 0 : 2);
#define PQ(FP, FF, LD)                                                                                                                   \
  do {                                                                                                                                   \
    if (rows8) LAUNCHN(c, "k_profq", (k_profq<FP, FF, PROFQ_BIG, LD>), dim3((c->P.iml + 63) / 64, (nrows + PROFQ_BIG - 1) / PROFQ_BIG, 1), dim3(64, PROFQ_BIG, 1), c->P, rho_rt, jfirst, jlast); \
    else LAUNCHN(c, "k_profq", (k_profq<FP, FF, 2, LD>), dim3((c->P.iml + 63) / 64, (nrows + 1) / 2, 1), dim3(64, 2, 1), c->P, rho_rt, jfirst, jlast);       \
  } while (0)
  if (fuse_filter) { if (fuse_prod == 0) PQ(0, 1, 1); else if (fuse_prod == 1) { if (ld) PQ(1, 1, 1); else PQ(1, 1, 0); } else PQ(2, 1, 1); }
  else { if (fuse_prod == 0) PQ(0, 0, 1); else if (fuse_prod == 1) PQ(1, 0, 1); else PQ(2, 0, 1); }
#undef PQ
  const KP &P = c->P;
  if (P.W || P.E || P.S || P.N) {
    const int len = P.im > P.jm ? P.im : P.jm;
    LAUNCH(c, k_profq_rim, dim3((len + 63) / 64, 4, P.kb), dim3(64, 1, 1), c->P);
  }
}
template <int KBT>
static void launch_proft_reg(pomgpu_ctx *c, double *f, const double *wfsurf, const double *fsurf, int nbc) {
  if (nbc == 2 || nbc == 4) LAUNCHN(c, "k_proft_reg", (k_proft_reg<KBT, 1>), rowgrid(c->P, ROWS_PROFT), rowblk(ROWS_PROFT), c->P, f, wfsurf, fsurf, nbc);
  else LAUNCHN(c, "k_proft_reg", (k_proft_reg<KBT, 0>), rowgrid(c->P, ROWS_PROFT), rowblk(ROWS_PROFT), c->P, f, wfsurf, fsurf, nbc);
}
void launch_proft(pomgpu_ctx *c, double *f, const double *wfsurf, const double *fsurf, int nbc) {
  if (!pomgpu_reg_kb(c)) { LAUNCH(c, k_proft, colgrid(c->P), colblk(), c->P, f, wfsurf, fsurf, nbc); return; }
  with_kbt(c->P.kb, [&](auto t) { launch_proft_reg<KBT_OF(t)>(c, f, wfsurf, fsurf, nbc); });
}
#define PROFT_TS_KBMAX 56
template <int KBT>
static void launch_proft2_reg(pomgpu_ctx *c, const ProftArgs &a0, const ProftArgs &a1, int sw, int lane) {
  if constexpr (KBT <= PROFT_TS_KBMAX) {
    if (lane) {
      if (c->prof_on) {
        const int s = pomgpu_prof_slot(c, "proft_ts_lane");
        if (s >= 0) (c->parent ? c->parent : c)->prof[s].launches++;
      }
      LAUNCHN(c, "k_proft_reg2", (k_proft_ts_reg<KBT>), rowgrid(c->P, ROWS_PROFT), rowblk(ROWS_PROFT), c->P, a0, a1);
      return;
    }
  }
  if (sw) LAUNCHN(c, "k_proft_reg2", (k_proft_reg2<KBT, 1>), twin(rowgrid(c->P, ROWS_PROFT)), rowblk(ROWS_PROFT), c->P, a0, a1);
  else LAUNCHN(c, "k_proft_reg2", (k_proft_reg2<KBT, 0>), twin(rowgrid(c->P, ROWS_PROFT)), rowblk(ROWS_PROFT), c->P, a0, a1);
}
int launch_proft2(pomgpu_ctx *c, double *f0, const double *wfsurf0, const double *fsurf0, int nbc0, double *f1, const double *wfsurf1, const double *fsurf1, int nbc1) {
  const int sw0 = (nbc0 == 2 || nbc0 == 4), sw1 = (nbc1 == 2 || nbc1 == 4);
  if (!pomgpu_reg_kb(c) || sw0 != sw1) return 0;
  const ProftArgs a0 = {f0, wfsurf0, fsurf0, nbc0}, a1 = {f1, wfsurf1, fsurf1, nbc1};
  const int lane = !SW(c, PROFT_TWIN) && !sw0 && (nbc0 <= 2) == (nbc1 <= 2);
  with_kbt(c->P.kb, [&](auto t) { launch_proft2_reg<KBT_OF(t)>(c, a0, a1, sw0, lane); });
  return 1;
}
void launch_advu_profu(pomgpu_ctx *c, int do_adv, int do_prof) { LAUNCH(c, k_advu_profu, colgrid(c->P), colblk(), c->P, do_adv, do_prof); }
void launch_advv_profv(pomgpu_ctx *c, int do_adv, int do_prof) { LAUNCH(c, k_advv_profv, colgrid(c->P), colblk(), c->P, do_adv, do_prof); }
int launch_profuv_reg(pomgpu_ctx *c) {
  const KP &P = c->P;
  if (!pomgpu_reg_kb(c)) return 0;
  with_kbt(P.kb, [&](auto t) {
    LAUNCHN(c, "k_profuv_reg2", (k_profuv_reg2<KBT_OF(t)>), dim3((P.iml + 61) / 62, (P.jml + ROWS_PROFUV - 1) / ROWS_PROFUV, 2), rowblk(ROWS_PROFUV), c->P);
  });
  return 1;
}
void launch_profuv_filter_reg(pomgpu_ctx *c, double *ubk, double *vbk) {
  const KP &P = c->P;
  LAUNCH(c, k_uvb_bottom, grid2(P), blk2(), c->P, ubk, vbk);
  with_kbt(P.kb, [&](auto t) {
    LAUNCHN(c, "k_profuv_filter_reg2", (k_profuv_filter_reg2<KBT_OF(t)>), dim3((P.iml + 61) / 62, (P.jml + ROWS_PROFUV - 1) / ROWS_PROFUV, 2), rowblk(ROWS_PROFUV),
            c->P, (const double *)ubk, (const double *)vbk);
  });
}
void launch_uv_filter_rim(pomgpu_ctx *c) {
  const KP &P = c->P;
  const int len = 8 * P.jm > P.im - 7 ? 8 * P.jm : P.im - 7;
  LAUNCH(c, k_uv_filter_rim, dim3((len + 63) / 64, 8, 2), dim3(64, 1, 1), c->P);
}
void launch_uvf_copy(pomgpu_ctx *c) {
  const KP &P = c->P;
  const dim3 g((P.im - 7 + 63) / 64, (P.jm - 7 + 3) / 4, P.kbm1);
  LAUNCH(c, k_uvf_copy, g, blk2(), c->P, P.b3 + (size_t)P3_uf * P.a3, (const double *)(P.b3 + (size_t)P3_u * P.a3));
  LAUNCH(c, k_uvf_copy, g, blk2(), c->P, P.b3 + (size_t)P3_vf * P.a3, (const double *)(P.b3 + (size_t)P3_v * P.a3));
}
void launch_uv_filter(pomgpu_ctx *c, int own) {
  if (!pomgpu_reg_kb(c)) { LAUNCH(c, k_uv_filter, colgrid(c->P), colblk(), c->P, own); return; }
  with_kbt(c->P.kb, [&](auto t) { LAUNCHN(c, "k_uv_filter_reg2", (k_uv_filter_reg2<KBT_OF(t)>), twin(rowgrid(c->P, ROWS_UVF)), rowblk(ROWS_UVF), c->P, own); });
}

__global__ void k_probe_divi(long n, const double *a, const double *b, double *out, int f32) {
  const long e = (long)blockIdx.x * blockDim.x + threadIdx.x;
  if (e >= n) return;
  if (f32) out[e] = (double)divi((float)a[e], inv_of((float)b[e]));
  else out[e] = divi(a[e], inv_of(b[e]));
}
// ... 12 lines not shown
```

### extpom_amd/csrc/pomgpu_api.hip

```cpp
#include <math.h>
#include <stdarg.h>
#include <stdio.h>
#include <stdlib.h>
#include <string.h>
#include <vector>
#include "pomgpu.h"
#include "pomgpu_internal.hpp"

struct ProfPair { int slot; hipEvent_t a, b; };
struct ProfState { std::vector<ProfPair> pending; std::vector<ProfPair> free_; char filter[64]; };
static ProfState *PS(pomgpu_ctx *c) { return (ProfState *)c->prof_state; }

#define SLOT2(c, n) ((c)->P.b2 + (size_t)(n) * (c)->P.n2)
#define SLOT3(c, n) ((c)->P.b3 + (size_t)(n) * (c)->P.a3)
#define D2(c, name) SLOT2(c, P2_##name)
#define D3(c, name) SLOT3(c, P3_##name)
#define LEV3(c, p, lev) ((double *)((pomgpu_st *)(p) + (size_t)(lev) * (c)->P.n2))

int pomgpu_fail(pomgpu_ctx *c, int code, const char *fmt, ...) {
  if (c && c->parent) c = c->parent;
  if (c) {
    va_list ap;
    va_start(ap, fmt);
    vsnprintf(c->err, sizeof c->err, fmt, ap);
// ... 101 lines not shown
  if (c->wide.x) c->wide.x->prof_on = false;
  return POMGPU_OK;
}
extern "C" int pomgpu_prof_count(pomgpu_ctx *c) { return c ? c->nprof : 0; }
extern "C" int pomgpu_prof_get(pomgpu_ctx *c, int k, const char **name, long *launches, double *total_ms) {
  if (!c || k < 0 || k >= c->nprof) return POMGPU_EINVAL;
  if (name) *name = c->prof[k].name;
  if (launches) *launches = c->prof[k].launches;
  if (total_ms) *total_ms = c->prof[k].ms;
  return POMGPU_OK;
}

static void sync_scalars(pomgpu_ctx *c) {
  KP &P = c->P;
  const pom_blkcon &k = c->con;
  P.alpha = k.alpha; P.dte = k.dte; P.dti = k.dti; P.dti2 = k.dti2; P.dte2 = k.dte2; P.grav = k.grav;
  P.kappa = k.kappa; P.ramp = k.ramp; P.rfe = k.rfe; P.rfn = k.rfn; P.rfs = k.rfs; P.rfw = k.rfw;
  P.rhoref = k.rhoref; P.sbias = k.sbias; P.small_ = k.small; P.tbias = k.tbias; P.tprni = k.tprni;
  P.umol = k.umol; P.horcon = k.horcon; P.ispi = k.ispi; P.isp2i = k.isp2i; P.smoth = k.smoth; P.sw = k.sw;
  P.time = k.time; P.vmaxl = k.vmaxl;
  P.mode = k.mode; P.ntp = k.ntp; P.nadv = k.nadv; P.nbct = k.nbct; P.nbcs = k.nbcs; P.nitera = k.nitera;
  P.npg = k.npg; P.isplit = k.isplit; P.iext = k.iext; P.iint = k.iint; P.iend = k.iend;
  P.const1_profq = pow(16.6, 2. / 3.) * 1.;
  P.cb_profq = pow((double)15.8f * 100., (double)(2.f / 3.f));
}

static void tracers_free(pomgpu_ctx *c);
#ifndef POMGPU_BUILD_ID
#define POMGPU_BUILD_ID "unknown"
#endif
extern "C" const char *pomgpu_build_id(void) { return POMGPU_BUILD_ID; }
#ifdef POMGPU_STORE_F32
#ifdef POMGPU_COMPUTE_F32
extern "C" const char *pomgpu_version(void) { return "extpom_amd pomgpu 0.2 (gfx950) fp32-storage fp32-arithmetic variant"; }
#else
extern "C" const char *pomgpu_version(void) { return "extpom_amd pomgpu 0.2 (gfx950) fp32-storage variant"; }
#endif
#define F32_REFUSE(c, what) return fail(c, POMGPU_EINVAL, what ": not in the fp32-storage variant (3-D arrays are not doubles there)")
#else
extern "C" const char *pomgpu_version(void) { return "extpom_amd pomgpu 0.2 (gfx950)"; }
#define F32_REFUSE(c, what)
#endif
#ifdef POMGPU_STORE_F32
__global__ void k_cvt_to_st(pomgpu_st *dst, const double *src, size_t n) {
  const size_t t = (size_t)blockIdx.x * blockDim.x + threadIdx.x;
  if (t < n) dst[t] = (pomgpu_st)src[t];
}
__global__ void k_cvt_from_st(double *dst, const pomgpu_st *src, size_t n) {
  const size_t t = (size_t)blockIdx.x * blockDim.x + threadIdx.x;
  if (t < n) dst[t] = (double)src[t];
}
#endif
static int copy3_h2d(pomgpu_ctx *c, double *slot, const double *host) {
  const size_t n3 = c->P.n3;
#ifdef POMGPU_STORE_F32
  double *stage = c->P.s3[POMGPU_NSCR3 - 1];
  HIPCHK(c, hipMemcpyAsync(stage, host, sizeof(double) * n3, hipMemcpyHostToDevice, c->stream));
  hipLaunchKernelGGL(k_cvt_to_st, dim3((unsigned)((n3 + 255) / 256)), dim3(256), 0, c->stream, (pomgpu_st *)slot, (const double *)stage, n3);
#else
  HIPCHK(c, hipMemcpyAsync(slot, host, sizeof(double) * n3, hipMemcpyHostToDevice, c->stream));
#endif
  return POMGPU_OK;
}
static int copy3_d2h(pomgpu_ctx *c, double *host, const double *slot) {
  const size_t n3 = c->P.n3;
#ifdef POMGPU_STORE_F32
  double *stage = c->P.s3[POMGPU_NSCR3 - 1];
  hipLaunchKernelGGL(k_cvt_from_st, dim3((unsigned)((n3 + 255) / 256)), dim3(256), 0, c->stream, stage, (const pomgpu_st *)slot, n3);
  HIPCHK(c, hipMemcpyAsync(host, stage, sizeof(double) * n3, hipMemcpyDeviceToHost, c->stream));
  HIPCHK(c, hipStreamSynchronize(c->stream));
#else
  HIPCHK(c, hipMemcpyAsync(host, slot, sizeof(double) * n3, hipMemcpyDeviceToHost, c->stream));
#endif
  return POMGPU_OK;
}

static const int X2_SLOT[POMGPU_NGEN] = {P2_ua, P2_va, P2_d, P2_el, P2_elb, P2_uab, P2_vab};
static void ext_buffers(pomgpu_ctx *c) {
  KP &P = c->P;
  for (int n = 0; n < POMGPU_NGEN; n++) P.x2[n] = P.y2[n] = c->ext_parity ? c->alt2[n] : P.b2 + (size_t)X2_SLOT[n] * P.n2;
}
static void rho_materialize(pomgpu_ctx *c) {
  if (!c->rho_rt_pending || (c->flags & POMGPU_CTX_2D)) return;
  c->rho_rt_pending = 0;
  launch_roundtrip(c, SLOT3(c, P3_rho), SLOT3(c, P3_rmean), 2);
}
static void side_join(pomgpu_ctx *c);
static void side_begin(pomgpu_ctx *c);
static void side_end(pomgpu_ctx *c, hipEvent_t ev);
static int rim_side(pomgpu_ctx *c);
static void early_invalidate(pomgpu_ctx *c);
void pomgpu_wr_materialize(pomgpu_ctx *c) {
  if (!c->wr_pending) return;
  c->wr_pending = 0;
  (void)hipSetDevice(c->device);
  if (!(c->flags & POMGPU_CTX_2D)) launch_realvertvl(c, 1);
}
static bool wr_on_demand(const pomgpu_ctx *c) {
  return !c->exch && !c->tp.on && !c->wide.on && !c->parent && !(c->flags & POMGPU_CTX_2D) && !c->wr_eager && !SW(c, WR_NODEFER);
}
static bool uv_fused(const pomgpu_ctx *c) {
  const KP &P = c->P;
  return !c->exch && !c->tp.on && !c->wide.on && !c->parent && !(c->flags & POMGPU_CTX_2D) && !c->wr_eager && pomgpu_reg_kb(c) &&
         P.im >= 8 && P.jm >= 8 && !SW(c, UV_NOFUSE);
}
static bool w_fused(const pomgpu_ctx *c) {
  return POMGPU_W_FUSE && !c->exch && !c->tp.on && !c->wide.on && !(c->flags & POMGPU_CTX_2D) && !SW(c, ADVQ_SINGLE) && !SW(c, ADVQ_EXCHANGE) &&
         !SW(c, VERTVL_CELLS) && !SW(c, W_NOFUSE);
}
static bool uvm_onload(const pomgpu_ctx *c) {
  const pom_blkcon &k = c->con;
  return POMGPU_UVM_ONLOAD && w_fused(c) && uv_fused(c) && c->uvm_valid && !SW(c, UVMEAN_PASS) &&
         (k.mode == 4 || (k.nadv == 2 && c->P.nitera == 1 && !SW(c, ADVT2_SINGLE))) &&
         (!c->ntr || (k.nadv == 2 && c->P.nitera == 1));
}
static bool ld_on_demand(const pomgpu_ctx *c) {
  return !c->exch && !c->tp.on && !c->wide.on && !c->parent && !(c->flags & POMGPU_CTX_2D) && !c->wr_eager && !SW(c, LD_EAGER);
}
static bool next_step_fetches_record(const pomgpu_ctx *c) {
  if (!c->frc_on && !c->lat_on && !c->wat_on) return false;
  const pom_blkcon &k = c->con;
  const int isrf = (int)(.125 * 86400. / k.dti), ibc = (int)((double)(1.f / 24.f) * 86400. / k.dti), iwater = (int)(86400. / k.dti);
  const int next = k.iint + 1 + k.cont_bry;
  return (c->frc_on && (isrf < 1 || next % isrf == 0)) || (c->lat_on && (ibc < 1 || next % ibc == 0)) ||
         (c->wat_on && (iwater < 1 || (k.iint + 1) % iwater == 0));
}
static void uvf_materialize(pomgpu_ctx *c) {
  if (!c->uvf_pending) return;
  c->uvf_pending = 0;
  launch_uvf_copy(c);
}
static void restore_materialize(pomgpu_ctx *c) {
  c->uvm_valid = 0;
  side_join(c);
  rho_materialize(c);
  pomgpu_wr_materialize(c);
  uvf_materialize(c);
  if (!c->rst_pending) return;
  c->rst_pending = 0;
  launch_restore_fields(c, c->rst_fold, c->rst_fnew);
}
static void ext_flush_deferred(pomgpu_ctx *c);
static void ext_canonical(pomgpu_ctx *c) {
  ext_flush_deferred(c);
  if (!c->ext_parity) return;
  KP &P = c->P;
  for (int n = 0; n < POMGPU_NGEN; n++) launch_copy2(c, P.b2 + (size_t)X2_SLOT[n] * P.n2, c->alt2[n]);
  c->ext_parity = 0;
  ext_buffers(c);
}
static int ctx_create(pomgpu_ctx **out, const pomgpu_dims *d, int device, void *stream, int flags);
extern "C" int pomgpu_create(pomgpu_ctx **out, const pomgpu_dims *d, int device, void *stream) {
  return ctx_create(out, d, device, stream, 0);
}
static int ctx_create(pomgpu_ctx **out, const pomgpu_dims *d, int device, void *stream, int flags) {
  if (!out || !d) return POMGPU_EINVAL;
  *out = NULL;
  if (d->kb < 4 || d->kb > POMGPU_KBMAX || d->im < 5 || d->jm < 5 || d->im > d->im_local || d->jm > d->jm_local) {
    fprintf(stderr, "pomgpu_create: unsupported extents im=%d jm=%d kb=%d (need im,jm>=5, 4<=kb<=%d)\n", d->im, d->jm,
            d->kb, POMGPU_KBMAX);
    return POMGPU_EINVAL;
  }
  if ((size_t)d->im_local * d->jm_local * d->kb * sizeof(double) >= ((size_t)1 << 32)) {
    fprintf(stderr, "pomgpu_create: a 3-D array of this tile has %zu bytes; the column kernels address a level with 32-bit offsets "
                    "(< 4 GiB per array): split the domain into more tiles\n", (size_t)d->im_local * d->jm_local * d->kb * sizeof(double));
    return POMGPU_EINVAL;
  }
  int ndev = 0;
  if (hipGetDeviceCount(&ndev) != hipSuccess || ndev <= 0 || device < 0 || device >= ndev) {
    fprintf(stderr, "pomgpu_create: no usable HIP device (count=%d, asked %d); the hot path has no CPU fallback\n", ndev,
            device);
    return POMGPU_ENODEV;
  }
  pomgpu_ctx *c = (pomgpu_ctx *)calloc(1, sizeof(pomgpu_ctx));
  if (!c) return POMGPU_ENOMEM;
  c->device = device;
  c->flags = flags;
  c->lbry_sides = POMGPU_SIDE_EAST | POMGPU_SIDE_SOUTH;
  if (hipSetDevice(device) != hipSuccess) { free(c); return POMGPU_EHIP; }
  KP &P = c->P;
  P.im = d->im; P.jm = d->jm; P.kb = d->kb; P.imm1 = d->im - 1; P.jmm1 = d->jm - 1; P.kbm1 = d->kb - 1; P.kbm2 = d->kb - 2;
  P.iml = d->im_local; P.jml = d->jm_local;
  P.W = d->n_west == -1; P.E = d->n_east == -1; P.S = d->n_south == -1; P.N = d->n_north == -1;
  P.n2 = (size_t)P.iml * P.jml; P.n3 = P.n2 * P.kb;
  pomgpu_switches_read(c->sw);
  {
    const long pages = SW(c, PAD3) ? SWV(c, PAD3) : 0;
    P.a3 = P.n3 + (pages > 0 ? (size_t)pages * 512 : 0);
  }
  set_band_geometry(P, c->sw);
  size_t off = 0; int s = 0;
#define BD_(name, shape) P.bdoff[s++] = off; off += BDN_##shape;
#define BDN_J ((size_t)P.jml)
#define BDN_I ((size_t)P.iml)
#define BDN_JK ((size_t)P.jml * P.kb)
#define BDN_IK ((size_t)P.iml * P.kb)
  POM_BDRY(BD_)
#undef BD_
  const size_t nbd = off;
  c->con.error_status = 0;
  if (stream) { c->stream = (hipStream_t)stream; c->own_stream = false; }
  else {
    if (hipStreamCreateWithFlags(&c->stream, hipStreamNonBlocking) != hipSuccess) { free(c); return POMGPU_EHIP; }
    c->own_stream = true;
  }
  c->cur = c->stream;
  c->prof_state = new ProfState();
  PS(c)->filter[0] = 0;
  bool ok = true;
  auto alloc = [&](double **p, size_t n) {
    if (!ok) return;
    if (hipMalloc((void **)p, n * sizeof(double)) != hipSuccess) { ok = false; *p = NULL; return; }
    if (hipMemsetAsync(*p, 0, n * sizeof(double), c->stream) != hipSuccess) ok = false;
  };
  alloc(&P.b1, (size_t)POM_NBLK1D * P.kb);
  alloc(&P.r1, (size_t)POM_NBLK1D * P.kb);
  alloc(&P.b2, (size_t)POM_NBLK2D * P.n2);
  const bool only2d = (flags & POMGPU_CTX_2D) != 0;
  if (!only2d) alloc(&P.b3, (size_t)POM_NBLK3D * P.a3);
  alloc(&P.bd, nbd);
  for (int n = 0; n < POMGPU_NSCR3 && !only2d; n++) alloc(&P.s3[n], P.n3);
  for (int n = 0; n < POMGPU_NSCR2; n++) alloc(&P.s2[n], P.n2);
  for (int n = 0; n < 2 && !only2d; n++) alloc(&c->uvb_bot[n], P.n2);
  for (int n = 0; n < POMGPU_NCOEF2; n++) alloc(&P.c2[n], P.n2);
  alloc(&c->alt2[0], (size_t)POMGPU_NGEN * P.n2);
  for (int n = 1; n < POMGPU_NGEN && ok; n++) c->alt2[n] = c->alt2[0] + (size_t)n * P.n2;
  { double *m = NULL; alloc(&m, (P.n2 + 7) / 8 + 1); P.m8 = (unsigned char *)m; }
  for (int n = 0; n < 2; n++) {
    const size_t len = (size_t)(P.kb + 1) * (n == 0 ? P.jml : P.iml);
    alloc(&c->ord_send[n], len);
    alloc(&c->ord_recv[n], len);
  }
  if (ok) { P.g4[2] = c->ord_recv[0]; P.g4[0] = c->ord_recv[0] + P.jml; P.g4[3] = c->ord_recv[1]; P.g4[1] = c->ord_recv[1] + P.iml; }
  alloc(&c->d_vel, 4);
  alloc(&c->d_stats, 8);
  if (ok && hipMalloc((void **)&c->d_err, sizeof(int)) != hipSuccess) ok = false;
  if (ok && hipMalloc((void **)&c->d_areas, sizeof(int)) != hipSuccess) ok = false;
  if (ok && hipMemsetAsync(c->d_areas, 0, sizeof(int), c->stream) != hipSuccess) ok = false;
  if (ok && hipMemsetAsync(c->d_err, 0, sizeof(int), c->stream) != hipSuccess) ok = false;
  if (SW(c, DEBUG_ALLOC))
    fprintf(stderr, "pomgpu_create: b1 %p r1 %p b2 %p b3 %p bd %p s3[0] %p s3[4] %p s2[0] %p c2[0] %p\n", (void *)P.b1, (void *)P.r1, (void *)P.b2,
            (void *)P.b3, (void *)P.bd, (void *)P.s3[0], (void *)P.s3[4], (void *)P.s2[0], (void *)P.c2[0]);
  if (!ok) {
    fprintf(stderr, "pomgpu_create: device allocation failed (%zu MB per 3-D array)\n", P.n3 * 8 >> 20);
    pomgpu_destroy(c);
    return POMGPU_ENOMEM;
  }
  c->ext_parity = 0;
  c->rst_pending = 0;
  ext_buffers(c);
  (void)hipStreamSynchronize(c->stream);
  *out = c;
  return POMGPU_OK;
}

static void wide_free(pomgpu_ctx *c);
extern "C" void pomgpu_destroy(pomgpu_ctx *c) {
  if (!c) return;
  (void)hipSetDevice(c->device);
  if (c->stream) (void)hipStreamSynchronize(c->stream);
  if (c->side) (void)hipStreamSynchronize(c->side);
  if (pomgpu_io_wait(c) != POMGPU_OK)
    fprintf(stderr, "pomgpu_destroy: the output / restart file still being written could not be completed -- call pomgpu_io_wait (or pomgpu_sync) "
                    "before pomgpu_destroy to get its status\n");
  wide_free(c);
  pomgpu_tp_free(c);
  pomgpu_ff_free(c);
  KP &P = c->P;
  (void)hipFree(P.r1);
  if (c->tune_block) {
    (void)hipFree(c->tune_block);
    c->tune_block = NULL; P.b3 = NULL;
    for (int n = 0; n < POMGPU_NSCR3; n++) P.s3[n] = NULL;
  }
  (void)hipFree(P.b1); (void)hipFree(P.b2); (void)hipFree(P.b3); (void)hipFree(P.bd);
  for (int n = 0; n < POMGPU_NSCR3; n++) (void)hipFree(P.s3[n]);
  for (int n = 0; n < POMGPU_NSCR2; n++) (void)hipFree(P.s2[n]);
  (void)hipFree(c->uvb_bot[0]); (void)hipFree(c->uvb_bot[1]);
  for (int n = 0; n < POMGPU_NCOEF2; n++) (void)hipFree(P.c2[n]);
  (void)hipFree(c->alt2[0]); (void)hipFree(c->alt3[0]);
  (void)hipFree(P.m8);
  for (int n = 0; n < 2; n++) { (void)hipFree(c->ord_send[n]); (void)hipFree(c->ord_recv[n]); }
  for (int n = 0; n <= POMGPU_MAXREC; n++) { (void)hipFree(c->rec_t[n]); (void)hipFree(c->rec_s[n]); (void)hipFree(c->rec_tau[n]); }
  (void)hipFree(c->d_vel); (void)hipFree(c->d_err); (void)hipFree(c->d_areas); (void)hipFree(c->d_stats); (void)hipFree(c->ext_bar);
  for (int k = 0; k < 3; k++) for (int sl = 0; sl < 4; sl++) { (void)hipFree(c->frc_dev[k][sl][0]); (void)hipFree(c->frc_dev[k][sl][1]); }
  for (int sl = 0; sl < 4; sl++) { (void)hipFree(c->lat_dev[sl]); (void)hipFree(c->wat_dev[sl]); }
  (void)hipFree(c->mean_acc);
  tracers_free(c);
  ProfState *ps = PS(c);
  if (ps) {
    for (auto &p : ps->pending) { (void)hipEventDestroy(p.a); (void)hipEventDestroy(p.b); }
    for (auto &p : ps->free_) { (void)hipEventDestroy(p.a); (void)hipEventDestroy(p.b); }
    delete ps;
  }
  if (c->side) {
    (void)hipEventDestroy(c->ev_fork); (void)hipEventDestroy(c->ev_early);
    for (auto &e : c->side_ev) (void)hipEventDestroy(e.ev);
    (void)hipStreamDestroy(c->side);
  }
  if (c->own_stream && c->stream) (void)hipStreamDestroy(c->stream);
  free(c);
}

extern "C" int pomgpu_debug_switch(pomgpu_ctx *c, const char *name, const char *value) {
  if (!c || !name) return POMGPU_EINVAL;
  if (strncmp(name, "POMGPU_", 7) == 0) name += 7;
  for (int n = 0; n < SW__count; n++)
    if (strcmp(POMGPU_SW_NAMES[n], name) == 0) {
      pomgpu_ctx *two[2] = {c, c->wide.x};
      for (pomgpu_ctx *t : two)
        if (t) { t->sw.on[n] = value ? 1 : 0; t->sw.val[n] = value ? atol(value) : 0; }
      return POMGPU_OK;
    }
  return fail(c, POMGPU_EINVAL, "debug_switch: no switch named %s", name);
}
extern "C" const char *pomgpu_last_error(const pomgpu_ctx *c) { return c ? c->err : "null context"; }
extern "C" void *pomgpu_stream(pomgpu_ctx *c) { return c ? (void *)c->stream : NULL; }
extern "C" void *pomgpu_current_stream(pomgpu_ctx *c) { return c ? (void *)c->cur : NULL; }

static int pull_err(pomgpu_ctx *c) {
  if (c->launch_err) return POMGPU_EHIP;
  int e = 0;
  HIPCHK(c, hipMemcpyAsync(&e, c->d_err, sizeof(int), hipMemcpyDeviceToHost, c->stream));
  HIPCHK(c, hipStreamSynchronize(c->stream));
  if (e) c->con.error_status = 1;
  if (e & POMGPU_DERR_BARRIER) {
    pomgpu_ctx *two[2] = {c, c->wide.x};
    for (pomgpu_ctx *t : two)
      if (t && t->ext_bar) {
        (void)hipMemsetAsync(t->ext_bar, 0, 2 * sizeof(unsigned), c->stream);
        t->ext_bar_base = 0;
        t->ext_loop_off = 1;
      }
  }
  return POMGPU_OK;
}
extern "C" int pomgpu_sync(pomgpu_ctx *c) {
  if (!c) return POMGPU_EINVAL;
  side_join(c);
  HIPCHK(c, hipStreamSynchronize(c->stream));
  { const int rio = pomgpu_io_wait(c); if (rio) return rio; }
  return c->launch_err ? POMGPU_EHIP : POMGPU_OK;
}

extern "C" int pomgpu_set_con(pomgpu_ctx *c, const pom_blkcon *con, int lramp) {
  if (!c || !con) return POMGPU_EINVAL;
  if (c->wr_pending && con->dti2 != c->P.dti2) pomgpu_wr_materialize(c);
  c->con = *con;
  c->lramp = lramp;
  sync_scalars(c);
  return POMGPU_OK;
}
extern "C" int pomgpu_get_con(pomgpu_ctx *c, pom_blkcon *con) {
  if (!c || !con) return POMGPU_EINVAL;
  int rc = pull_err(c);
  if (rc) return rc;
  *con = c->con;
  return POMGPU_OK;
}
static int check_masks(pomgpu_ctx *c, const double *blk2d) {
  const int slots[3] = {P2_fsm, P2_dum, P2_dvm};
// ... 184 lines not shown
extern "C" int pomgpu_halo_pack8(pomgpu_ctx *c, double *const *dev, const int *nz, int count, double *const *to) {
  if (!c || !dev || !nz || !to) return POMGPU_EINVAL;
  return launch_halo_pack8(c, dev, nz, count, to) ? fail(c, POMGPU_EINVAL, "halo_pack8: bad array list") : POMGPU_OK;
}
extern "C" int pomgpu_halo_unpack8(pomgpu_ctx *c, double *const *dev, const int *nz, int count, const double *const *from) {
  if (!c || !dev || !nz || !from) return POMGPU_EINVAL;
  return launch_halo_unpack8(c, dev, nz, count, from) ? fail(c, POMGPU_EINVAL, "halo_unpack8: bad array list") : POMGPU_OK;
}

static double *dev3(pomgpu_ctx *c, const double *host) {
  if (!c->host3 || !host) return NULL;
  const ptrdiff_t off = host - c->host3;
  if (off < 0 || (size_t)off >= (size_t)POM_NBLK3D * c->P.n3 || (size_t)off % c->P.n3) return NULL;
  if ((size_t)off / c->P.n3 == P3_taurstrb) pomgpu_tau_touched(c, 0);
  if ((size_t)off / c->P.n3 == P3_taurstrf) pomgpu_tau_touched(c, 1);
  return SLOT3(c, (size_t)off / c->P.n3);
}
static double *dev2(pomgpu_ctx *c, const double *host) {
  if (!c->host2 || !host) return NULL;
  const ptrdiff_t off = host - c->host2;
  if (off < 0 || (size_t)off >= (size_t)POM_NBLK2D * c->P.n2 || (size_t)off % c->P.n2) return NULL;
  return c->P.b2 + off;
}

static void xch(pomgpu_ctx *c, int count, ...) {
  if (!c->exch) return;
  double *ptr[8];
  int nz[8];
  va_list ap;
  va_start(ap, count);
  for (int n = 0; n < count; n++) { ptr[n] = va_arg(ap, double *); nz[n] = va_arg(ap, int); }
  va_end(ap);
  c->exch(c->exch_user, ptr, nz, count);
}

static void seq_advave(pomgpu_ctx *c) {
  KP &P = c->P;
  if (!c->exch && P.mode != 2) { launch_advave_fused(c); return; }
  launch_advave_a(c);
  xch(c, 2, P.s2[0], 1, P.s2[1], 1);
  launch_advave_b(c);
  xch(c, 3, D2(c, advua), 1, D2(c, fluxua), 1, D2(c, fluxva), 1);
  launch_advave_c(c);
  xch(c, 1, D2(c, advva), 1);
  if (P.mode == 2) {
    launch_advave_m2a(c);
    xch(c, 1, P.s2[2], 1);
    launch_advave_m2b(c);
  }
}
static void seq_advct(pomgpu_ctx *c, int sum2d = 0, int defer_xch = 0) {
  KP &P = c->P;
  if (!c->exch) {
    launch_advct_col(c, sum2d);
    c->uvm_valid = POMGPU_UVM_ONLOAD && !c->tp.on && !c->wide.on && !(c->flags & POMGPU_CTX_2D);
    return;
  }
  if (c->tp.on && !SW(c, ADVCT_SPLIT)) {
    pomgpu_transport &T = c->tp;
    const size_t ne = 2 * (size_t)P.kbm1 * P.jm, nn = 2 * (size_t)P.kbm1 * P.im;
    const size_t sc[8] = {0, T.nbr[1] >= 0 ? ne : 0, 0, T.nbr[3] >= 0 ? nn : 0, 0, 0, 0, 0};
    const size_t rc[8] = {T.nbr[0] >= 0 ? ne : 0, 0, T.nbr[2] >= 0 ? nn : 0, 0, 0, 0, 0, 0};
    const bool side = rim_side(c);
    double *const *snd = side ? T.send2 : T.send, *const *rcv = side ? T.recv2 : T.recv;
    if (side) side_begin(c);
    launch_advct_edge(c, T.nbr[1] >= 0 ? snd[1] : NULL, T.nbr[3] >= 0 ? snd[3] : NULL);
    const int rcm = side ? pomgpu_tp_move_side(c, sc, rc) : pomgpu_tp_move(c, sc, rc);
    if (side) side_end(c, c->side_ev[SIDE_R1].ev);
    if (rcm) return;
    launch_advct_col(c, sum2d);
    if (side) (void)hipStreamWaitEvent(c->stream, c->side_ev[SIDE_R1].ev, 0);
    launch_advct_fix(c, T.nbr[0] >= 0 ? rcv[0] : NULL, T.nbr[2] >= 0 ? rcv[2] : NULL);
    if (sum2d) launch_advct_fix2d(c, T.nbr[0] >= 0, T.nbr[2] >= 0);
    if (!defer_xch) xch(c, 2, D3(c, advx), P.kb, D3(c, advy), P.kb);
    return;
  }
  launch_advct_a(c);
  xch(c, 2, P.s3[0], P.kbm1, P.s3[1], P.kbm1);
  launch_advct_b(c);
  xch(c, 2, D3(c, advx), P.kb, P.s3[4], P.kbm1);
  launch_advct_c(c);
  xch(c, 1, D3(c, advy), P.kb);
}
static void seq_rho_roundtrip(pomgpu_ctx *c, int defer_rt) {
  if (defer_rt) {
    launch_roundtrip_level(c, D3(c, rho), D3(c, rmean), c->P.kb);
    c->rho_rt_pending = 1;
  } else {
    launch_roundtrip(c, D3(c, rho), D3(c, rmean), 0);
  }
}
static void seq_baropg(pomgpu_ctx *c, int sum2d = 0, int defer_rt = 0) {
  launch_baropg(c, sum2d);
  seq_rho_roundtrip(c, defer_rt);
}
static void seq_baropg_mcc(pomgpu_ctx *c, int sum2d = 0, int defer_rt = 0) {
  KP &P = c->P;
  if (c->order) {
    launch_order_pack(c, c->ord_send[0], c->ord_send[1]);
    c->order(c->order_user, c->ord_send[0], (P.kb + 1) * P.jml, c->ord_send[1], (P.kb + 1) * P.iml, c->ord_recv[0], c->ord_recv[1]);
  }
  launch_baropg_mcc(c, sum2d);
  seq_rho_roundtrip(c, defer_rt);
}
static void seq_advq(pomgpu_ctx *c, double *qb, double *q, double *qf, int pair, int zero_else) {
  KP &P = c->P;
  if (!c->exch) { launch_coef_eta(c); launch_advq_col(c, q, qb, qf, zero_else); return; }
  double *xf = P.s3[pair ? 2 : 0], *yf = P.s3[pair ? 3 : 1];
  launch_advq_flux(c, q, qb, xf, yf);
  xch(c, 2, xf, P.kbm1, yf, P.kbm1);
  launch_advq_step(c, q, qb, qf, xf, yf, zero_else);
}
static void seq_profq(pomgpu_ctx *c, int fuse_filter = 0, int with_w = 0, int store_ld = 1) {
  KP &P = c->P;
  launch_profq_bc(c);
  double *ufkb = LEV3(c, D3(c, uf), P.kb - 1);
  const int lines = c->exch && c->tp.on && !SW(c, PROD_FULL);
  if (lines) {
    launch_profq_prod(c, 1, c->rho_rt_pending);
    if (with_w) xch(c, 4, P.s2[4], 1, ufkb, 1, LEV3(c, P.s3[0], 1), P.kbm2, D3(c, w), P.kb);
    else xch(c, 3, P.s2[4], 1, ufkb, 1, LEV3(c, P.s3[0], 1), P.kbm2);
    launch_profq(c, 2, fuse_filter, c->rho_rt_pending);
    return;
  }
  if (with_w) xch(c, 3, P.s2[4], 1, ufkb, 1, D3(c, w), P.kb);
  else xch(c, 2, P.s2[4], 1, ufkb, 1);
  if (!c->exch) { launch_profq(c, 1, fuse_filter, c->rho_rt_pending, 0, -1, store_ld); return; }
  launch_profq_prod(c, 0, c->rho_rt_pending);
  xch(c, 1, LEV3(c, P.s3[0], 1), P.kbm2);
  launch_profq(c, 0, fuse_filter, c->rho_rt_pending);
}
static void seq_fb_fix(pomgpu_ctx *c, double *fb, const double *fclim) {
  launch_copy_kb(c, fb);
  launch_roundtrip(c, fb, fclim, 0);
}
static void seq_advt1(pomgpu_ctx *c, double *fb, double *f, const double *fclim, double *ff) {
  launch_advt1(c, fb, f, fclim, ff);
  seq_fb_fix(c, fb, fclim);
}
static void seq_advt2(pomgpu_ctx *c, double *fb, double *f, const double *fclim, double *ff, bool defer_roundtrip = false) {
  KP &P = c->P;
  if (P.nitera == 1) {
    launch_coef_eta(c);
    launch_advt2_rows(c, fb, f, fclim, ff);
  } else {
    launch_advt2_mass(c);
    const double *fbmem = fb, *eta = D2(c, etb);
    for (int itera = 1; itera <= P.nitera; itera++) {
      launch_advt2_step(c, fbmem, f, eta, ff, itera);
      xch(c, 1, ff, P.kbm1);
      launch_mask3(c, ff, D2(c, fsm));
      launch_smol(c, ff);
      eta = D2(c, etf);
      launch_copy3(c, P.s3[3], ff);
      fbmem = P.s3[3];
    }
    launch_advt2_diff(c, fb, fclim, ff);
  }
  xch(c, 1, ff, P.kbm1);
  if (defer_roundtrip) launch_copy_kb(c, fb);
  else seq_fb_fix(c, fb, fclim);
}
static int restore_prepare(pomgpu_ctx *c, double *fold_out, double *fnew_out) {
  const pom_blkcon &k = c->con;
  const double trst = 30.;
  const int irst = (int)(trst * 86400. / k.dti);
  const int ntime = (int)(k.time / trst);
  auto load = [&](int n) -> int {
    const int rfile = pomgpu_ff_has(c, 3), steady = rfile && pomgpu_ff_rate_steady(c);
    if (rfile) { const int rc = pomgpu_ff_rate_have(c, n); if (rc) return rc; }
    const double *tr, *sr;
    if (pomgpu_ff_has(c, 2)) {
      const int rc = pomgpu_ff_fetch_restore(c, n);
      if (rc) return rc;
      tr = c->rec_t[0]; sr = c->rec_s[0];
    } else {
      if (n < 1 || n > POMGPU_MAXREC || !c->rec_t[n])
// ... 43 lines not shown
}

static void side_begin(pomgpu_ctx *c) {
  (void)hipEventRecord(c->ev_fork, c->stream);
  (void)hipStreamWaitEvent(c->side, c->ev_fork, 0);
  c->cur = c->side;
  if (c->wide.x) c->wide.x->cur = c->side;
}
static void side_end(pomgpu_ctx *c, hipEvent_t ev) {
  (void)hipEventRecord(ev, c->side);
  c->cur = c->stream;
  if (c->wide.x) c->wide.x->cur = c->stream;
}
static void side_post(pomgpu_ctx *c, side_round r) {
  side_end(c, c->side_ev[r].ev);
  c->side_ev[r].pending = 1;
}
static void side_wait(pomgpu_ctx *c, side_round r) {
  if (!c->side_ev[r].pending) return;
  (void)hipStreamWaitEvent(c->stream, c->side_ev[r].ev, 0);
  c->side_ev[r].pending = 0;
}
static void side_join(pomgpu_ctx *c) {
  if (c->early_started) (void)hipStreamWaitEvent(c->stream, c->ev_early, 0);
  for (int r = 0; r < SIDE__count; r++) side_wait(c, (side_round)r);
}
static int rim_side(pomgpu_ctx *c) { return c->tp.on && c->exch && c->wide.on && c->wide.split && !SW(c, RIM_MAIN); }
static int round8(pomgpu_ctx *c, int side, double *const *dev, const int *nz, int count, double *const *dev2 = NULL) {
  const KP &P = c->P;
  pomgpu_transport &T = c->tp;
  const char *what = side ? "exchange (side stream)" : "exchange";
  double *const *snd = side ? T.send2 : T.send, *const *rcv = side ? T.recv2 : T.recv;
  const size_t *cap = side ? T.cap2 : T.cap;
  size_t total = 0;
  for (int a = 0; a < count; a++) total += (size_t)nz[a];
  const size_t len[8] = {(size_t)P.jm, (size_t)P.jm, (size_t)P.im, (size_t)P.im, 1, 1, 1, 1};
  size_t cnt[8];
  for (int d = 0; d < 8; d++) {
    cnt[d] = T.nbr[d] >= 0 ? total * len[d] : 0;
    if (cnt[d] > cap[d]) return fail(c, POMGPU_EINVAL, "%s: %zu doubles exceed the staging buffer", what, cnt[d]);
  }
  if (launch_halo_pack8(c, dev, nz, count, snd)) return fail(c, POMGPU_EINVAL, "%s: bad array list", what);
  const int rc = side ? pomgpu_tp_move_side(c, cnt, cnt) : pomgpu_tp_move(c, cnt, cnt);
  if (rc) return rc;
  (void)launch_halo_unpack8(c, dev, nz, count, rcv);
  if (dev2) (void)launch_halo_unpack8(c, dev2, nz, count, rcv);
  return POMGPU_OK;
}
static int rim_round(pomgpu_ctx *c, side_round r, double *const *dev, const int *nz, int count, double *const *dev2 = NULL) {
  side_begin(c);
  const int rc = round8(c, 1, dev, nz, count, dev2);
  side_post(c, r);
  return rc;
}
static void early_invalidate(pomgpu_ctx *c) {
  if (c->early_started) { (void)hipStreamWaitEvent(c->stream, c->ev_early, 0); c->early_started = 0; }
}
int pomgpu_side_stream(pomgpu_ctx *c) {
  if (c->side) return 1;
  if (hipStreamCreateWithFlags(&c->side, hipStreamNonBlocking) != hipSuccess) { c->side = NULL; return 0; }
  bool ok = hipEventCreateWithFlags(&c->ev_fork, hipEventDisableTiming) == hipSuccess && hipEventCreateWithFlags(&c->ev_early, hipEventDisableTiming) == hipSuccess;
  for (auto &e : c->side_ev) ok = ok && hipEventCreateWithFlags(&e.ev, hipEventDisableTiming) == hipSuccess;
  if (!ok) {
    (void)hipStreamDestroy(c->side);
    c->side = NULL;
    return 0;
  }
#ifdef POMGPU_EMU
  emu_stream_defer(c->side);
#endif
  return 1;
}
#define NEED_RAW(c) if (!(c)) return POMGPU_EINVAL; if ((c)->broken) return POMGPU_EHIP; (void)hipSetDevice((c)->device)
static void wide_flush(pomgpu_ctx *c);
#define NEED_HOT(c) NEED_RAW(c); ext_canonical(c); wide_flush(c)
#define NEED(c) NEED_HOT(c); side_join(c); restore_materialize(c)

int pomgpu_materialize(pomgpu_ctx *c) {
  NEED(c);
  return POMGPU_OK;
}
void pomgpu_mirrors_written(pomgpu_ctx *c) {
  c->uvm_valid = 0;
  c->wide.static_done = 0;
  early_invalidate(c);
  refresh_coefs(c);
}
void pomgpu_cold_tail(pomgpu_ctx *c, void (*update_initial)(pomgpu_ctx *), void (*sums)(pomgpu_ctx *)) {
  launch_dens(c, D3(c, sclim), D3(c, tclim), D3(c, rmean));
  launch_dens(c, D3(c, sb), D3(c, tb), D3(c, rho));
  update_initial(c);
  if (c->con.npg == 2) seq_baropg_mcc(c); else seq_baropg(c);
  sums(c);
  pomgpu_tau_touched(c, 0); pomgpu_tau_touched(c, 1);
  pomgpu_mirrors_written(c);
}
extern "C" int pomgpu_get_time(pomgpu_ctx *c) {
  NEED_HOT(c);
  pom_blkcon &k = c->con;
  k.time = k.dti * (double)(float)k.iint / 86400. + k.time0;
  if (k.iint >= k.iswtch) k.iprint = (int)lround(k.prtd2 * 24. * 3600. / k.dti);
  if (c->lramp) { k.ramp = k.time / k.period; if (k.ramp > 1.) k.ramp = 1.; }
  else k.ramp = 1.;
  sync_scalars(c);
  return POMGPU_OK;
}
static int lateral_viscosity(pomgpu_ctx *c, int sum2d, int defer_rt = 0) {
  NEED_HOT(c);
  side_wait(c, SIDE_RTS);
  rho_materialize(c);
  KP &P = c->P;
  if (P.mode != 2) {
    const bool lib_x = c->tp.on && c->exch && !SW(c, ADVCT_SPLIT);
    auto pressure_gradient = [&]() {
      if (P.npg == 1) seq_baropg(c, sum2d, defer_rt);
      else if (P.npg == 2) seq_baropg_mcc(c, sum2d, defer_rt);
      else {
        fprintf(stderr, "\nError: invalid value for npg\n");
        c->con.error_status = 1;
      }
    };
    const bool pg_first = c->side_ev[SIDE_R8].pending != 0;
    if (pg_first) pressure_gradient();
    side_wait(c, SIDE_R8);
    seq_advct(c, sum2d, lib_x);
    if (!pg_first) pressure_gradient();
    launch_aam(c);
    if (lib_x && sum2d && rim_side(c)) {
      double *arr[3] = {D3(c, advx), D3(c, advy), D3(c, aam)};
      const int nz[3] = {P.kb, P.kb, P.kbm1};
      side_begin(c);
      const int rc2 = round8(c, 1, arr, nz, 3);
      if (!rc2) launch_vint(c, 1, -1);
      side_post(c, SIDE_R2);
      if (rc2) return rc2;
    }
    else if (lib_x) xch(c, 3, D3(c, advx), P.kb, D3(c, advy), P.kb, D3(c, aam), P.kbm1);
    else xch(c, 1, D3(c, aam), P.kbm1);
  }
  return POMGPU_OK;
}
static int wide_early_start(pomgpu_ctx *c);
extern "C" int pomgpu_lateral_viscosity(pomgpu_ctx *c) {
  NEED_HOT(c);
  const int rc = wide_early_start(c);
  const pom_blkcon &k0 = c->con;
  const int defer_rt = k0.mode == 3 && (k0.iint != 1 || k0.time0 != 0.) && !SW(c, RHO_ROUNDTRIP);
  return rc ? rc : lateral_viscosity(c, 0, defer_rt);
}
static int wide_begin(pomgpu_ctx *c);
static int mode_interaction(pomgpu_ctx *c, int sums_done) {
  NEED_HOT(c);
  if (c->wide.on) {
    if (c->P.mode != 2) launch_vint(c, sums_done, sums_done && c->side_ev[SIDE_R2].pending ? 1 : 0);
    return wide_begin(c);
  }
  if (c->P.mode != 2) {
    launch_vint(c, sums_done);
    seq_advave(c);
  }
  launch_modeint_tail(c);
  xch(c, 2, D2(c, utf), 1, D2(c, vtf), 1);
  return POMGPU_OK;
}
static KP row_window(const KP &P, int lo, int hi) {
  KP Q = P;
// ... 486 lines not shown
      launch_proft(c, a.trf, a.wsurf, a.surf, a.nbc);
      if (nf == 2) launch_proft(c, b.trf, b.wsurf, b.surf, b.nbc);
    }
    const TrEdge e[2] = {{a.trf, a.tr, a.bd[0], a.bd[1], a.bd[2], a.bd[3]}, {b.trf, b.tr, b.bd[0], b.bd[1], b.bd[2], b.bd[3]}};
    launch_tr_edges(c, e, nf);
    const TrUpd u[2] = {{a.trf, a.clim, a.tr, a.trb}, {b.trf, b.clim, b.tr, b.trb}};
    launch_tr_update(c, u, nf, rt);
    n += nf;
  }
  return POMGPU_OK;
}
static int wr_on_side(pomgpu_ctx *c, int with_kernel) {
  const KP &P = c->P;
  side_wait(c, SIDE_WR);
  side_begin(c);
  if (with_kernel) launch_realvertvl(c);
  double *arr[1] = {D3(c, wr)};
  const int nz[1] = {P.kbm1};
  const int rcw = round8(c, 1, arr, nz, 1);
  side_post(c, SIDE_WR);
  return rcw;
}
static int mode_internal(pomgpu_ctx *c, int defer_wr) {
  NEED_HOT(c);
  KP &P = c->P;
  const pom_blkcon &k = c->con;
  side_wait(c, SIDE_R2);
  side_wait(c, SIDE_R8);
  if ((k.iint != 1 || k.time0 != 0.) && k.mode != 2) {
    c->uvf_pending = 0;
    struct UvmScope { pomgpu_ctx *c; ~UvmScope() { c->P.uvm = 0; c->uvm_valid = 0; } } uvm_scope{c};
    P.uvm = uvm_onload(c) ? 1 : 0;
    if (!P.uvm) launch_int_uvmean(c);
    const bool wf = w_fused(c);
    if (!wf) launch_vertvl(c, 1);
    const bool lib_x = c->tp.on && c->exch;
    const bool rimr = lib_x && rim_side(c) && !SW(c, RIM_RESULTS_MAIN) && !SW(c, ADVQ_EXCHANGE) && !SW(c, PROD_FULL);
    if (rimr) {
      double *aw[1] = {D3(c, w)};
      const int nw[1] = {P.kb};
      const int rcw = rim_round(c, SIDE_RW, aw, nw, 1);
      if (rcw) return rcw;
    }
    else if (!lib_x) xch(c, 1, D3(c, w), P.kb);
    launch_coef_eta(c, P.uvm);
    if (!c->exch || !SW(c, ADVQ_EXCHANGE)) {
      if (SW(c, ADVQ_SINGLE)) {
        launch_advq_col(c, D3(c, q2), D3(c, q2b), D3(c, uf), 1);
        launch_advq_col(c, D3(c, q2l), D3(c, q2lb), D3(c, vf), 1);
#if POMGPU_W_FUSE
      } else if (wf) {
        launch_advq2w_col(c, D3(c, q2), D3(c, q2b), D3(c, uf), D3(c, q2l), D3(c, q2lb), D3(c, vf), 1);
#endif
      } else {
        launch_advq2_col(c, D3(c, q2), D3(c, q2b), D3(c, uf), D3(c, q2l), D3(c, q2lb), D3(c, vf), 1);
      }
    } else {
      double *x0 = P.s3[0], *y0 = P.s3[1], *x1 = P.s3[2], *y1 = P.s3[3];
      launch_advq_flux(c, D3(c, q2), D3(c, q2b), x0, y0);
      launch_advq_flux(c, D3(c, q2l), D3(c, q2lb), x1, y1);
      xch(c, 4, x0, P.kbm1, y0, P.kbm1, x1, P.kbm1, y1, P.kbm1);
      launch_advq_step(c, D3(c, q2), D3(c, q2b), D3(c, uf), x0, y0, 1);
      launch_advq_step(c, D3(c, q2l), D3(c, q2lb), D3(c, vf), x1, y1, 1);
    }
    const int qfuse = !SW(c, QFILTER_SPLIT);
    if (rimr) {
      launch_profq_bc(c);
      launch_profq(c, 1, qfuse, c->rho_rt_pending, P.S ? 1 : 2, P.N ? P.jm : P.jmm1);
    } else {
      seq_profq(c, qfuse, lib_x, !(defer_wr && ld_on_demand(c) && !next_step_fetches_record(c)));
      xch(c, 2, LEV3(c, D3(c, uf), 1), P.kbm2, LEV3(c, D3(c, vf), 1), P.kbm2);
    }
    launch_bcond6_edges(c);
    if (qfuse) launch_q_filter_rim(c);
    else launch_q_filter(c, 1);
    if (rimr) {
      double *aq[9] = {D3(c, q2), D3(c, q2b), D3(c, q2l), D3(c, q2lb), D3(c, km), D3(c, kh), D3(c, kq), D3(c, l), D3(c, dtef)};
      const int nq[9] = {P.kb, P.kb, P.kb, P.kb, P.kb, P.kb, P.kb, P.kb, P.kb};
      const int rcq = rim_round(c, SIDE_RQ, aq, nq, 9);
      if (rcq) return rcq;
    }
    side_wait(c, SIDE_RW);
    if (k.mode != 4) {
      if (k.nadv == 1) {
        seq_advt1(c, D3(c, tb), D3(c, t), D3(c, tclim), D3(c, uf));
        seq_advt1(c, D3(c, sb), D3(c, s), D3(c, sclim), D3(c, vf));
      } else if (k.nadv == 2) {
        if (P.nitera == 1 && !SW(c, ADVT2_SINGLE)) {
          launch_advt2x2_col(c, D3(c, tb), D3(c, t), D3(c, tclim), D3(c, uf), D3(c, sb), D3(c, s), D3(c, sclim), D3(c, vf));
          if (!lib_x) xch(c, 1, D3(c, uf), P.kbm1);
          if (!lib_x) xch(c, 1, D3(c, vf), P.kbm1);
          launch_copy_kb(c, D3(c, tb), D3(c, sb));
        } else {
          seq_advt2(c, D3(c, tb), D3(c, t), D3(c, tclim), D3(c, uf), true);
          seq_advt2(c, D3(c, sb), D3(c, s), D3(c, sclim), D3(c, vf), true);
        }
      } else {
        return fail(c, POMGPU_EINVAL, "Error: invalid value for nadv");
      }
      const bool rts = rimr && k.nadv == 2 && P.nitera == 1 && !SW(c, ADVT2_SINGLE);
      if (!rts) xch(c, 2, D3(c, uf), rimr ? P.kb : P.kbm1, D3(c, vf), P.kbm1);
      if (!rts) side_wait(c, SIDE_RQ);
      if (!launch_proft2(c, D3(c, uf), D2(c, wtsurf), D2(c, tsurf), k.nbct, D3(c, vf), D2(c, wssurf), D2(c, ssurf), k.nbcs)) {
        launch_proft(c, D3(c, uf), D2(c, wtsurf), D2(c, tsurf), k.nbct);
        launch_proft(c, D3(c, vf), D2(c, wssurf), D2(c, ssurf), k.nbcs);
      }
      launch_bcond4_edges(c);
      double fold, fnew;
      int rc = restore_prepare(c, &fold, &fnew);
      if (rc) return rc;
      launch_ts_update(c, fold, fnew, k.nadv == 2, 0);
      c->rho_rt_pending = 0;
      c->rst_pending = 1; c->rst_fold = fold; c->rst_fnew = fnew;
      if (rts) {
        double *at[5] = {D3(c, t), D3(c, tb), D3(c, s), D3(c, sb), D3(c, rho)};
        const int nt[5] = {P.kb, P.kb, P.kb, P.kb, P.kb};
        const int rct = rim_round(c, SIDE_RTS, at, nt, 5);
        if (rct) return rct;
      }
    }
    if (c->ntr) {
      const int rct = tracer_stage(c, lib_x);
      if (rct) return rct;
    }
    side_wait(c, SIDE_RQ);
    const bool fuse = uv_fused(c);
    if (pomgpu_reg_kb(c)) {
      launch_advuv_col(c);
      if (fuse) launch_profuv_filter_reg(c, c->uvb_bot[0], c->uvb_bot[1]);
      else launch_profuv_reg(c);
    } else {
      launch_advu_profu(c, 1, 1);
      launch_advv_profv(c, 1, 1);
    }
    if (!lib_x) xch(c, 2, D2(c, wubot), 1, D2(c, wvbot), 1);
    launch_bcondorl3(c);
    const bool rim78 = lib_x && rim_side(c);
    if (rim78) {
      const int top = P.kb - 1;
      double *a7[4] = {D2(c, wubot), D2(c, wvbot), D3(c, uf), D3(c, vf)}, *b7[4] = {D2(c, wubot), D2(c, wvbot), D3(c, u), D3(c, v)};
      const int n7[4] = {1, 1, P.kbm1, P.kbm1};
      side_begin(c);
      const int rc7 = round8(c, 1, a7, n7, 4, b7);
      side_end(c, c->side_ev[SIDE_R8].ev);
      launch_uv_filter(c, 1);
      double *a8[6] = {D3(c, ub), D3(c, vb), LEV3(c, D3(c, u), top), LEV3(c, D3(c, uf), top), LEV3(c, D3(c, v), top), LEV3(c, D3(c, vf), top)};
      const int n8[6] = {P.kb, P.kb, 1, 1, 1, 1};
      if (rc7) { side_begin(c); side_post(c, SIDE_R8); return rc7; }
      const int rc8 = rim_round(c, SIDE_R8, a8, n8, 6);
      if (rc8) return rc8;
    } else {
      if (lib_x) xch(c, 4, D2(c, wubot), 1, D2(c, wvbot), 1, D3(c, uf), P.kbm1, D3(c, vf), P.kbm1);
      else xch(c, 2, D3(c, uf), P.kbm1, D3(c, vf), P.kbm1);
      if (fuse) { launch_uv_filter_rim(c); c->uvf_pending = 1; }
      else launch_uv_filter(c);
      if (lib_x) {
        const int top = P.kb - 1;
        xch(c, 6, D3(c, ub), P.kb, D3(c, vb), P.kb, LEV3(c, D3(c, u), top), 1, LEV3(c, D3(c, uf), top), 1, LEV3(c, D3(c, v), top), 1, LEV3(c, D3(c, vf), top), 1);
      } else {
        xch(c, 6, D3(c, ub), P.kb, D3(c, u), P.kb, D3(c, uf), P.kb, D3(c, vb), P.kb, D3(c, v), P.kb, D3(c, vf), P.kb);
      }
    }
  }
  launch_int_tail(c);
  const bool side_wr = c->tp.on && c->exch && c->wide.split && c->tp.wr_side;
  if (side_wr && defer_wr && c->wide.on && !SW(c, WR_NODEFER)) {
    c->wr_deferred = 1;
    return POMGPU_OK;
  }
  if (wr_on_demand(c)) { c->wr_pending = 1; return POMGPU_OK; }
  c->wr_pending = 0;
  side_wait(c, SIDE_R8);
  launch_realvertvl(c);
  if (side_wr) return wr_on_side(c, 0);
  xch(c, 1, D3(c, wr), P.kbm1);
  return POMGPU_OK;
}
extern "C" int pomgpu_mode_internal(pomgpu_ctx *c) { return mode_internal(c, 0); }
extern "C" int pomgpu_check_velocity(pomgpu_ctx *c, double *vamax, int *imax, int *jmax) {
  NEED_HOT(c);
  side_join(c);
  launch_check_velocity(c);
  double out[3];
  HIPCHK(c, hipMemcpyAsync(out, c->d_vel, sizeof out, hipMemcpyDeviceToHost, c->stream));
  int rc = pull_err(c);
  if (rc) return rc;
  if (vamax) *vamax = out[0];
  if (imax) *imax = (int)out[1];
  if (jmax) *jmax = (int)out[2];
  if (out[0] > c->con.vmaxl) {
    fprintf(stderr, "Error: velocity condition violated\n iint =%8d vamax =%12.3e   imax,jmax =%5d%5d\n", c->con.iint, out[0],
            (int)out[1], (int)out[2]);
    c->con.error_status = 1;
  }
  return POMGPU_OK;
// ... 678 lines not shown
```

### extpom_amd/csrc/pomgpu_internal.hpp

```cpp
#pragma once
#include <hip/hip_runtime.h>
#include <stddef.h>
#include <stdlib.h>
#include "pom_layout.h"

#ifndef COL_ROWS
#define COL_ROWS 4
#endif
#ifndef COL_WX
#define COL_WX 1
#endif
#define POMGPU_NSCR3 8
#define POMGPU_NSCR2 8
#define POMGPU_NCOEF2 25
#define POMGPU_MAXREC 8
#define POMGPU_TRMAX 8
#define POMGPU_KBMAX 128
#define POMGPU_CTX_2D 1
#define POMGPU_DERR_VELOCITY 1
#define POMGPU_DERR_BARRIER 2
#define POMGPU_NGEN 7

struct KP {
  int im, jm, kb, imm1, jmm1, kbm1, kbm2, iml, jml;
// ... 183 lines not shown
template <class F> __device__ __forceinline__ float halo_e(float x, F) { return wave_dn1(x); }
#endif
#ifdef POMGPU_EMU
#define SCHED_FENCE()
#else
#define SCHED_FENCE() __builtin_amdgcn_sched_barrier(0)
#endif
#ifndef POMGPU_EMU
#define WAVE_UNIFORM(x) __builtin_amdgcn_readfirstlane(x)
#else
#define WAVE_UNIFORM(x) (x)
#endif
#define HALO_LANE (int)((blockIdx.x * blockDim.x + threadIdx.x) & 63)

#ifndef POMGPU_EMU
typedef unsigned int pomgpu_u32x2 __attribute__((ext_vector_type(2)));
struct BufA { __amdgpu_buffer_rsrc_t r; };
__device__ __forceinline__ BufA buf_of(const double *p, size_t doubles) {
  BufA b;
  b.r = __builtin_amdgcn_make_buffer_rsrc((void *)p, 0, (unsigned)(doubles * POMGPU_ST_BYTES), 0x00020000);
  return b;
}
#ifndef POMGPU_STORE_F32
__device__ __forceinline__ double bld(const BufA &b, unsigned voff, unsigned soff) {
  const pomgpu_u32x2 v = __builtin_amdgcn_raw_buffer_load_b64(b.r, (int)voff, (int)soff, 0);
  return __hiloint2double((int)v.y, (int)v.x);
}
__device__ __forceinline__ void bst(const BufA &b, unsigned voff, unsigned soff, double x) {
  pomgpu_u32x2 v;
  v.x = (unsigned)__double2loint(x); v.y = (unsigned)__double2hiint(x);
  __builtin_amdgcn_raw_buffer_store_b64(v, b.r, (int)voff, (int)soff, 0);
}
#else
__device__ __forceinline__ double bld(const BufA &b, unsigned voff, unsigned soff) {
  return (double)__uint_as_float(__builtin_amdgcn_raw_buffer_load_b32(b.r, (int)voff, (int)soff, 0));
}
__device__ __forceinline__ void bst(const BufA &b, unsigned voff, unsigned soff, double x) {
  __builtin_amdgcn_raw_buffer_store_b32(__float_as_uint((float)x), b.r, (int)voff, (int)soff, 0);
}
#endif
#else
struct BufA { double *p; };
static inline BufA buf_of(const double *p, size_t) { BufA b; b.p = (double *)p; return b; }
#ifndef POMGPU_STORE_F32
static inline double bld(const BufA &b, unsigned voff, unsigned soff) { return voff >= 0xFFFFFFF0u ? 0. : b.p[((size_t)voff + soff) >> 3]; }
static inline void bst(const BufA &b, unsigned voff, unsigned soff, double x) { if (voff < 0xFFFFFFF0u) b.p[((size_t)voff + soff) >> 3] = x; }
#else
static inline double bld(const BufA &b, unsigned voff, unsigned soff) {
  return voff >= 0xFFFFFFF0u ? 0. : (double)((const pomgpu_st *)b.p)[((size_t)voff + soff) >> 2];
}
static inline void bst(const BufA &b, unsigned voff, unsigned soff, double x) { if (voff < 0xFFFFFFF0u) ((pomgpu_st *)b.p)[((size_t)voff + soff) >> 2] = (pomgpu_st)x; }
#endif
#endif
#if defined(POMGPU_COMPUTE_F32) && !defined(POMGPU_EMU)
__device__ __forceinline__ pomgpu_ct bldc(const BufA &b, unsigned voff, unsigned soff) {
  return __uint_as_float(__builtin_amdgcn_raw_buffer_load_b32(b.r, (int)voff, (int)soff, 0));
}
__device__ __forceinline__ void bstc(const BufA &b, unsigned voff, unsigned soff, pomgpu_ct x) {
  __builtin_amdgcn_raw_buffer_store_b32(__float_as_uint(x), b.r, (int)voff, (int)soff, 0);
}
#else
__device__ __forceinline__ pomgpu_ct bldc(const BufA &b, unsigned voff, unsigned soff) { return (pomgpu_ct)bld(b, voff, soff); }
__device__ __forceinline__ void bstc(const BufA &b, unsigned voff, unsigned soff, pomgpu_ct x) { bst(b, voff, soff, x); }
#endif
#ifndef POMGPU_EMU
__device__ __forceinline__ BufA buf2_of(const double *p, size_t doubles) {
  BufA b;
  b.r = __builtin_amdgcn_make_buffer_rsrc((void *)p, 0, (unsigned)(doubles * 8), 0x00020000);
  return b;
}
__device__ __forceinline__ double bld2(const BufA &b, unsigned voff, unsigned soff) {
  const pomgpu_u32x2 v = __builtin_amdgcn_raw_buffer_load_b64(b.r, (int)voff, (int)soff, 0);
  return __hiloint2double((int)v.y, (int)v.x);
}
__device__ __forceinline__ void bst2(const BufA &b, unsigned voff, unsigned soff, double x) {
  pomgpu_u32x2 v;
  v.x = (unsigned)__double2loint(x); v.y = (unsigned)__double2hiint(x);
  __builtin_amdgcn_raw_buffer_store_b64(v, b.r, (int)voff, (int)soff, 0);
}
#else
static inline BufA buf2_of(const double *p, size_t) { BufA b; b.p = (double *)p; return b; }
static inline double bld2(const BufA &b, unsigned voff, unsigned soff) { return voff >= 0xFFFFFFF0u ? 0. : b.p[((size_t)voff + soff) >> 3]; }
static inline void bst2(const BufA &b, unsigned voff, unsigned soff, double x) { if (voff < 0xFFFFFFF0u) b.p[((size_t)voff + soff) >> 3] = x; }
#endif
#define BOFF_NONE 0xFFFFFFF0u
#define BUF3(p) buf_of((p), P.n3)
#define BOFF2(i, j) (unsigned)(((unsigned)((j)-1) * (unsigned)P.iml + (unsigned)((i)-1)) * POMGPU_ST_BYTES)
#define LVB (unsigned)(P.n2 * POMGPU_ST_BYTES)

#ifdef POMGPU_EMU
#define PACE_BARRIER() ((void)0)
#else
#define PACE_BARRIER() __builtin_amdgcn_s_barrier()
#endif
#ifndef LDS_ROWS
#define LDS_ROWS 8
#endif
#define ROWSHARE_SLOTS(NS) ((2 * (NS) + LDS_ROWS - 1) / LDS_ROWS)
#define ROWSHARE_ROWS (LDS_ROWS + 3)
template <int NS, int ROWS = LDS_ROWS> struct RowShare {
  static constexpr int SLOTS = (2 * NS + ROWS - 1) / ROWS;
  int r;
  int ss, sn;
  int hop[SLOTS];
  int hrow[SLOTS];
  unsigned hoff[SLOTS];
};
template <int NS, int ROWS = LDS_ROWS> __device__ __forceinline__ RowShare<NS, ROWS> rowshare_setup(const KP &P, int r, int j, int j0w, int i) {
  RowShare<NS, ROWS> S;
  S.r = r;
  S.ss = (j > 1 && j <= P.jml) ? r : r + 1;
  S.sn = (j < P.jml) ? r + 2 : r + 1;
  const int jsouth = j0w > 1 ? j0w - 1 : 1, jnorth = j0w + ROWS <= P.jml ? j0w + ROWS : P.jml;
#pragma unroll
  for (int q = 0; q < RowShare<NS, ROWS>::SLOTS; q++) {
    const int job = q * ROWS + r;
    const bool valid = job < 2 * NS;
    const int side = valid ? job / NS : 0;
    S.hop[q] = valid ? job % NS : 0;
    S.hrow[q] = valid ? (side ? ROWS + 1 : 0) : ROWS + 2;
    S.hoff[q] = valid ? BOFF2(i, side ? jnorth : jsouth) : BOFF_NONE;
  }
  return S;
}
template <int V, int NS, int ROWS> __device__ __forceinline__ UvmC rowshare_uvm(const KP &P, const RowShare<NS, ROWS> &S, int q, int op, int j0w, int i) {
  if (S.hop[q] != op || S.hrow[q] == ROWS + 2) return uvm_none();
  const int jsouth = j0w > 1 ? j0w - 1 : 1, jnorth = j0w + ROWS <= P.jml ? j0w + ROWS : P.jml;
  return uvm_of<V>(P, i, S.hrow[q] == 0 ? jsouth : jnorth);
}
template <int NS> __device__ __forceinline__ const double *rowshare_pick(const double *const (&b)[NS], int op) {
  const double *x = b[0];
#pragma unroll
  for (int o = 1; o < NS; o++)
    if (op == o) x = b[o];
#ifndef POMGPU_EMU
  const unsigned long long v = (unsigned long long)x;
  const unsigned lo = (unsigned)__builtin_amdgcn_readfirstlane((int)(unsigned)v), hi = (unsigned)__builtin_amdgcn_readfirstlane((int)(unsigned)(v >> 32));
  x = (const double *)(((unsigned long long)hi << 32) | lo);
#endif
  return x;
}

template <class T> struct InvDT { T b, y; };
typedef InvDT<double> InvD;
typedef InvDT<pomgpu_ct> InvDc;
__device__ __forceinline__ InvD inv_of(double b) { InvD d; d.b = b; d.y = 1.0 / b; return d; }
__device__ __forceinline__ InvDT<float> inv_of(float b) { InvDT<float> d; d.b = b; d.y = 1.0f / b; return d; }
#ifndef POMGPU_EMU
__device__ __forceinline__ double divi(double a, const InvD &d) {
  const double q0 = a * d.y;
  double r = __builtin_fma(-d.b, q0, a);
  double q = __builtin_fma(r, d.y, q0);
  r = __builtin_fma(-d.b, q, a);
  q = __builtin_fma(r, d.y, q);
  return a == 0. ? q0 : q;
}
__device__ __forceinline__ float divi(float a, const InvDT<float> &d) {
  const float q0 = a * d.y;
  float r = __builtin_fmaf(-d.b, q0, a);
  float q = __builtin_fmaf(r, d.y, q0);
  r = __builtin_fmaf(-d.b, q, a);
  q = __builtin_fmaf(r, d.y, q);
  return a == 0.f ? q0 : q;
}
#else
static inline double divi(double a, const InvD &d) { return a / d.b; }
static inline float divi(float a, const InvDT<float> &d) { return a / d.b; }
#endif
#define HALO_XCD_ORDER                                                                    \
  if (P.g_strip > 0) {                                                                    \
    const int st__ = P.g_strip, nfull__ = nbx__ / st__, wlast__ = nbx__ - nfull__ * st__; \
    int s__ = m__ / (rpx__ * st__);                                                       \
    if (s__ > nfull__) s__ = nfull__;                                                     \
    const int rem__ = m__ - s__ * rpx__ * st__, w__ = s__ < nfull__ ? st__ : (wlast__ > 0 ? wlast__ : 1); \
    byl__ = rem__ / w__; bxg__ = s__ * st__ + rem__ % w__;                                \
    if (bxg__ >= nbx__ || byl__ >= rpx__) return;                                         \
  } else {                                                                                \
    byl__ = m__ / nbx__; bxg__ = m__ % nbx__;                                             \
    if (byl__ >= rpx__) return;                                                           \
  }
#define HALO_XCD_DECODE HALO_XCD_DECODE_R(COL_ROWS)
#define HALO_XCD_DECODE_R(ROWS__)                                                         \
  const int g__ = (int)(blockIdx.x * blockDim.x + threadIdx.x);                           \
  const int L__ = g__ >> 6, nwx__ = (P.iml + 61) / 62, nbx__ = (nwx__ + COL_WX - 1) / COL_WX; \
  const int nby__ = (P.jml + ROWS__ - 1) / ROWS__;                                        \
  const int rpx__ = (nby__ + 7) / 8, m__ = L__ >> 3;                                      \
  int by__, bxg__;                                                                        \
  if (P.g_lin && 10 * nby__ < 72 * rpx__) {                                               \
    const int x__ = L__ & 7, T__ = nby__ * nbx__;                                         \
    const int c0__ = (int)(((long)x__ * T__) >> 3), c1__ = (int)(((long)(x__ + 1) * T__) >> 3); \
    const int t__ = c0__ + m__;                                                           \
    if (t__ >= c1__) return;                                                              \
    const int st__ = P.g_strip > 0 ? P.g_strip : nbx__, per__ = st__ * nby__, s__ = t__ / per__; \
    const int rem__ = t__ - s__ * per__, w__ = (s__ + 1) * st__ <= nbx__ ? st__ : nbx__ - s__ * st__; \
    by__ = rem__ / w__; bxg__ = s__ * st__ + rem__ % w__;                                 \
  } else {                                                                                \
    int byl__;                                                                            \
    HALO_XCD_ORDER                                                                        \
    by__ = (L__ & 7) * rpx__ + byl__;                                                     \
    if (by__ >= nby__) return;                                                            \
  }                                                                                       \
  const int lane = g__ & 63;                                                              \
  const int i0 = (bxg__ * COL_WX + (int)threadIdx.y % COL_WX) * 62 + lane;                \
  const int j = by__ * ROWS__ + (int)threadIdx.y / COL_WX + 1;
static inline dim3 grid1_halo_r(const KP &P, int rows) {
  const int nwx = (P.iml + 61) / 62, nbx = (nwx + COL_WX - 1) / COL_WX, nby = (P.jml + rows - 1) / rows, rpx = (nby + 7) / 8;
  if (P.g_lin && 10 * nby < 72 * rpx) return dim3((unsigned)(8 * ((nby * nbx + 7) / 8)), 1, 1);
  return dim3((unsigned)(8 * rpx * nbx), 1, 1);
}
static inline dim3 grid1_halo(const KP &P) { return grid1_halo_r(P, COL_ROWS); }
static inline dim3 blk_col_r(int rows) { return dim3(64, rows * COL_WX, 1); }
static inline dim3 blk_col() { return dim3(64, COL_ROWS * COL_WX, 1); }
#define HALO_COL (int)(((blockIdx.x * blockDim.x + threadIdx.x) >> 6) * 62 + ((blockIdx.x * blockDim.x + threadIdx.x) & 63))
static inline dim3 grid2_halo(const KP &P) { return dim3((P.iml + 61) / 62, (P.jml + 3) / 4, 1); }

#define TID_I (int)(blockIdx.x * blockDim.x + threadIdx.x + 1)
#define TID_J (int)(blockIdx.y * blockDim.y + threadIdx.y + 1)
#define TID_K (int)(blockIdx.z * blockDim.z + threadIdx.z + 1)

#define POMGPU_SWITCHES(X)                                                                                                    \
  X(THOMAS_SCRATCH) X(NO_PAIR) X(EXT_SPLIT) X(ADVAVE_SEPARATE) X(EXT_RIM_KERNEL) X(EXT_LOOP) X(EXT_NOMARCH) X(EXT_MARCH)      \
  X(EXT_ROWS) X(EXT_NOPAIR) X(EXT_PAIR) X(EXT_ROWS2) X(EXT_TWO_SETS) X(EXT_AREAS_LOAD) X(BAROPG_CELLS) X(VERTVL_CELLS)        \
  X(NO_LIN) X(ADVQ_SINGLE) X(ADVT2_SINGLE) X(REALVERTVL_CELLS) X(RHO_ROUNDTRIP) X(TAU_ARRAYS) X(PROFQ_ROWS8) X(PROFQ_ROWS2)    \
  X(PROFQ_NOPACE) X(COL_STRIP) X(BAND_BYTES) X(PAD3) X(IO_SYNC) X(ADVCT_SPLIT) X(ADVQ_EXCHANGE) X(PROD_FULL) X(QFILTER_SPLIT) \
  X(NO_OVERLAP) X(NO_SIDE_COMM) X(WR_MAIN) X(WIDE_W) X(WIDE_FULL) X(DEBUG_ALLOC) X(TEST_SPLIT_FAIL_RANK)  \
  X(WR_NODEFER) X(EXT_RING_FIRST) X(TUNE_FORCE) X(RIM_MAIN) X(RIM_RESULTS_MAIN) X(SUM2D_OFF) X(ADVCT_ROWS4) X(ADVCT_ROWS8) \
  X(IO_CHUNK_KB) X(UV_NOFUSE) X(W_NOFUSE) X(UVMEAN_PASS) X(PROFT_TWIN) X(LD_EAGER) X(TR_NOPAIR)
enum pomgpu_sw {
#define POMGPU_SW_(name) SW_##name,
  POMGPU_SWITCHES(POMGPU_SW_)
#undef POMGPU_SW_
  SW__count
};
struct pomgpu_switches {
  unsigned char on[SW__count];
  long val[SW__count];
};
static const char *const POMGPU_SW_NAMES[SW__count] = {
#define POMGPU_SW_(name) #name,
  POMGPU_SWITCHES(POMGPU_SW_)
#undef POMGPU_SW_
};
static inline void pomgpu_switches_read(pomgpu_switches &s) {
  for (int n = 0; n < SW__count; n++) {
    char var[64] = "POMGPU_";
    size_t k = 7;
    for (const char *q = POMGPU_SW_NAMES[n]; *q && k + 1 < sizeof var; q++) var[k++] = *q;
    var[k] = 0;
    const char *e = getenv(var);
    s.on[n] = e ? 1 : 0;
    s.val[n] = e ? atol(e) : 0;
  }
}
static inline unsigned pomgpu_switches_collective_digest(const pomgpu_switches &s) {
  static const int coll[] = {SW_ADVCT_SPLIT, SW_ADVQ_EXCHANGE, SW_PROD_FULL, SW_QFILTER_SPLIT, SW_NO_OVERLAP,
                             SW_NO_SIDE_COMM, SW_WR_MAIN, SW_WIDE_W, SW_WIDE_FULL, SW_EXT_SPLIT, SW_ADVAVE_SEPARATE, SW_WR_NODEFER, SW_RIM_MAIN, SW_ADVT2_SINGLE, SW_RIM_RESULTS_MAIN, SW_SUM2D_OFF};
  unsigned h = 2166136261u;
  for (size_t n = 0; n < sizeof coll / sizeof coll[0]; n++) {
    h = (h ^ (unsigned)(s.on[coll[n]] ? 1 + coll[n] : 0)) * 16777619u;
    h = (h ^ (unsigned)s.val[coll[n]]) * 16777619u;
  }
  return h & 0x3fffffffu;
}
#define SW(c, NAME) ((c)->sw.on[SW_##NAME] != 0)
#define SWV(c, NAME) ((c)->sw.val[SW_##NAME])
struct ProfEntry { const char *name; long launches; double ms; };
struct pomgpu_ctx;

static const int POMGPU_OPP[8] = {1, 0, 3, 2, 7, 6, 5, 4};
struct pomgpu_transport {
  int on;
  int nbr[8];
  void (*fn)(void *, const double *const *, const size_t *, double *const *, const size_t *);
  void *user;
  void *rccl;
  double *send[8], *recv[8];
  size_t cap[8];
  double *send2[8], *recv2[8];
  size_t cap2[8];
  int fn_ordered;
  int side_agreed;
  int wr_side;
  long rounds_side;
  long rounds;
};
struct RectJob { const double *src; double *dst; int ld_s, ld_d, ni, nj; };
struct RectGroup { int first, count, mni, mnj; };
struct RectTable { RectJob *dev; int ngroups; RectGroup g[8]; };
struct pomgpu_wide {
  int on, w, ox, oy;
  pomgpu_ctx *x;
  RectTable gather_pack, gather_unpack, scatter;
  size_t scount[8], rcount[8];
  RectTable early_pack, early_unpack, late_pack, late_unpack;
  size_t e_scount[8], e_rcount[8], l_scount[8], l_rcount[8];
  int split;
  int pending;
  int static_done;
};
enum side_round { SIDE_WR, SIDE_R1, SIDE_R2, SIDE_R8, SIDE_RW, SIDE_RQ, SIDE_RTS, SIDE__count };

struct pomgpu_ctx {
  KP P;
  pomgpu_switches sw;
  int device;
  hipStream_t stream;
  bool own_stream;
  hipStream_t cur, side;
  hipEvent_t ev_fork, ev_early;
  struct { hipEvent_t ev; int pending; } side_ev[SIDE__count];
  int early_started;
  double *tune_block;
  size_t tune_front;
  int tune_kmax;
  size_t tune_a0, tune_amax;
  int dev3_handed;
  int broken;
  int wr_deferred;
  pom_blkcon con;
  int lramp;
  double *rec_t[POMGPU_MAXREC + 1], *rec_s[POMGPU_MAXREC + 1];
  const double *host2, *host3;
  void (*exch)(void *, double *const *, const int *, int);
  void *exch_user;
  void (*order)(void *, const double *, int, const double *, int, double *, double *);
  void *order_user;
  double *ord_send[2], *ord_recv[2];
  double *alt2[POMGPU_NGEN];
  double *alt3[POMGPU_NGEN];
  int ext_parity;
  int ext_deferred;
  int tau_known[2];
  double tau_val[2];
  double *rec_tau[POMGPU_MAXREC + 1];
  long tau_id[2], tau_gen;
  int tau_same, rate_in_f, tau_handed;
  int rho_rt_pending;
  int rst_pending;
  double rst_fold, rst_fnew;
  int wr_pending;
  int uvf_pending;
  int uvm_valid;
  double *uvb_bot[2];
  int wr_eager;
  double *d_vel;
  int *d_err;
  int *d_areas;
  int areas_checked;
  double *d_stats;
  double *frc_dev[3][4][2];
  int frc_n[3][4];
  double *lat_dev[4];
  int lat_n[4];
  int frc_on, lat_on;
  double *wat_dev[4];
  int wat_n[4];
  int wat_on;
  int sss_on;
  bool prof_on;
  ProfEntry prof[96];
  int nprof;
  void *prof_state;
  pomgpu_transport tp;
  pomgpu_wide wide;
  pomgpu_ctx *parent;
  int flags;
  unsigned *ext_bar;
  unsigned ext_bar_base;
  int ext_loop_off;
  void *io_job;
  int z_init, z_clim;
  int z_lbry;
  int lbry_sides;
  void *frc_files;
  int launch_err;
  double *mean_acc;
  size_t mean_off[9];
  int mean_count;
  int ntr;
  struct pomgpu_tracer { double *trb, *tr, *trf, *clim, *q, *wsurf, *surf, *bd[4]; int nbc; double lam; } trc[POMGPU_TRMAX];
  double *tr_zero3;
  char err[512];
};
static inline bool pomgpu_reg_kb(const pomgpu_ctx *c) { return c->P.kb >= 6 && c->P.kb <= 64 && !SW(c, THOMAS_SCRATCH); }

int pomgpu_prof_slot(pomgpu_ctx *c, const char *name);
void pomgpu_prof_pre(pomgpu_ctx *c);
void pomgpu_prof_post(pomgpu_ctx *c, int slot);
int pomgpu_fail(pomgpu_ctx *c, int code, const char *fmt, ...);
void pomgpu_launch_check(pomgpu_ctx *c, const char *name);

#define LAUNCH(c, kern, grid, block, ...)                                        \
  do {                                                                           \
    int _s = (c)->prof_on ? pomgpu_prof_slot((c), #kern) : -1;                   \
    if (_s >= 0) pomgpu_prof_pre(c);                                             \
    hipLaunchKernelGGL(kern, grid, block, 0, (c)->cur, __VA_ARGS__);             \
    pomgpu_launch_check((c), #kern);                                             \
    if (_s >= 0) pomgpu_prof_post((c), _s);                                      \
  } while (0)

#define LAUNCHN(c, name, kern, grid, block, ...)                                 \
  do {                                                                           \
    int _s = (c)->prof_on ? pomgpu_prof_slot((c), name) : -1;                    \
    if (_s >= 0) pomgpu_prof_pre(c);                                             \
    hipLaunchKernelGGL(kern, grid, block, 0, (c)->cur, __VA_ARGS__);             \
    pomgpu_launch_check((c), name);                                              \
    if (_s >= 0) pomgpu_prof_post((c), _s);                                      \
  } while (0)

static inline dim3 blk2() { return dim3(64, 4, 1); }
static inline dim3 grid2(const KP &P) { return dim3((P.iml + 63) / 64, (P.jml + 3) / 4, 1); }
static inline dim3 grid3(const KP &P, int nz) { return dim3((P.iml + 63) / 64, (P.jml + 3) / 4, nz); }
static inline dim3 gridm(const KP &P) {
  const long nbands = (P.jml + P.g_rb - 1) / P.g_rb;
  const long rounds = (nbands + 7) / 8;
  return dim3((unsigned)(8 * rounds * P.kb * P.g_bpl), 1, 1);
}
static inline void set_band_geometry(KP &P, const pomgpu_switches &sw) {
  long budget = 3L << 20;
  const bool e = sw.on[SW_BAND_BYTES] != 0;
  if (e && sw.val[SW_BAND_BYTES] >= 1024) budget = sw.val[SW_BAND_BYTES];
  long rows = budget / ((long)P.iml * 8 * 24);
  rows = (rows / 4) * 4;
  if (rows < 4) rows = 4;
  if (rows > ((P.jml + 3) / 4) * 4) rows = ((P.jml + 3) / 4) * 4;
  P.g_rb = (int)rows;
  P.g_nbx = (P.iml + 63) / 64;
  P.g_bpl = P.g_nbx * (int)(rows / 4);
  const int nbx = ((P.iml + 61) / 62 + COL_WX - 1) / COL_WX;
  const int nstr = (nbx + 11) / 12;
  P.g_strip = nbx >= 20 ? (nbx + nstr - 1) / nstr : 0;
  if (sw.on[SW_COL_STRIP]) P.g_strip = (int)sw.val[SW_COL_STRIP];
  P.g_lin = sw.on[SW_NO_LIN] ? 0 : 1;
  if (!e) {
    long best = -1, bslots = 0;
    for (long r = 4; r <= rows; r += 4) {
      const long nb = (P.jml + r - 1) / r, slots = (nb + 7) / 8 * 8 * r;
      if (best < 0 || slots < bslots || (slots == bslots && r > best)) { best = r; bslots = slots; }
    }
    P.g_rb = (int)best;
    P.g_bpl = P.g_nbx * (int)(best / 4);
  }
}

void launch_advave_a(pomgpu_ctx *c);
void launch_advave_b(pomgpu_ctx *c);
void launch_advave_c(pomgpu_ctx *c);
void launch_advave_fused(pomgpu_ctx *c);
void launch_advct_col(pomgpu_ctx *c, int sum2d);
void launch_advct_edge(pomgpu_ctx *c, double *to_e, double *to_n);
void launch_advct_fix(pomgpu_ctx *c, const double *from_w, const double *from_s);
void launch_advct_fix2d(pomgpu_ctx *c, int west, int south);
void launch_advt2x2_col(pomgpu_ctx *c, const double *tb, const double *t, const double *tc, double *tf, const double *sb, const double *s_,
                        const double *sc, double *sf);
void launch_advq2_col(pomgpu_ctx *c, const double *q, const double *qb, double *qf, const double *ql, const double *qlb, double *qlf, int zero_else);
#if POMGPU_W_FUSE
void launch_advq2w_col(pomgpu_ctx *c, const double *q, const double *qb, double *qf, const double *ql, const double *qlb, double *qlf, int zero_else);
#endif
void launch_advuv_col(pomgpu_ctx *c);
int launch_profuv_reg(pomgpu_ctx *c);
void launch_profuv_filter_reg(pomgpu_ctx *c, double *ubk, double *vbk);
void launch_uv_filter_rim(pomgpu_ctx *c);
void launch_uvf_copy(pomgpu_ctx *c);
void launch_advave_m2a(pomgpu_ctx *c);
void launch_advave_m2b(pomgpu_ctx *c);
void launch_vint(pomgpu_ctx *c, int only_aam, int ghost = 0);
void launch_modeint_tail(pomgpu_ctx *c);
void launch_ext_elf(pomgpu_ctx *c);
void launch_ext_uvaf(pomgpu_ctx *c, int interior);
void launch_ext_update(pomgpu_ctx *c);
void launch_ext_step(pomgpu_ctx *c, const KP &Q, int store_f, int fuse_adv);
void launch_check_areas(pomgpu_ctx *c);
int launch_ext_loop(pomgpu_ctx *c, const KP &Q, int first, int last);
int launch_ext_pair_ok(const pomgpu_switches &sw, const KP &Q);
int launch_ext_pair(pomgpu_ctx *c, const KP &Q, double *const *T, int store_f2);
void launch_copy2(pomgpu_ctx *c, double *dst, const double *src);
void launch_lat(pomgpu_ctx *c, int phase, const double *rec, double fold, double fnew);
void launch_frc_load(pomgpu_ctx *c, const double *ra, const double *rb, double *xf, double *yf);
void launch_frc_interp(pomgpu_ctx *c, double fold, double fnew, double *x, const double *xb, const double *xf, double *y, const double *yb,
                       const double *yf);
void launch_frc_load1(pomgpu_ctx *c, const double *ra, double *xf, double *xb);
void launch_frc_interp1(pomgpu_ctx *c, double fold, double fnew, double *x, const double *xb, const double *xf);
void launch_int_tail(pomgpu_ctx *c);
void launch_bcond1(pomgpu_ctx *c);
void launch_advct_a(pomgpu_ctx *c);
void launch_advct_b(pomgpu_ctx *c);
void launch_advct_c(pomgpu_ctx *c);
void launch_aam(pomgpu_ctx *c);
void launch_roundtrip(pomgpu_ctx *c, double *a, const double *b, int fix_kb);
void launch_roundtrip_level(pomgpu_ctx *c, double *a, const double *b, int k);
void launch_advq_flux(pomgpu_ctx *c, const double *q, const double *qb, double *xf, double *yf);
void launch_advq_step(pomgpu_ctx *c, const double *q, const double *qb, double *qf, const double *xf, const double *yf, int zero_else);
void launch_q_filter(pomgpu_ctx *c, int mask);
void launch_q_filter_rim(pomgpu_ctx *c);
void launch_mask_q(pomgpu_ctx *c);
void launch_advt1(pomgpu_ctx *c, double *fb, double *f, const double *fclim, double *ff);
void launch_copy_kb(pomgpu_ctx *c, double *f, double *g = NULL);
void launch_advt2_mass(pomgpu_ctx *c);
void launch_advt2_step(pomgpu_ctx *c, const double *fbmem, const double *f, const double *eta, double *ff, int itera);
void launch_mask3(pomgpu_ctx *c, double *a, const double *m2);
void launch_smol(pomgpu_ctx *c, const double *ff);
void launch_copy3(pomgpu_ctx *c, double *dst, const double *src);
void launch_advt2_diff(pomgpu_ctx *c, const double *fb, const double *fc, double *ff);
void launch_ts_update(pomgpu_ctx *c, double fold, double fnew, int rt, int store_rst);
void launch_restore_fields(pomgpu_ctx *c, double fold, double fnew);
void launch_mask_ts(pomgpu_ctx *c);
struct TrUpd { const double *ff, *fc; double *f, *fb; };
void launch_tr_update(pomgpu_ctx *c, const TrUpd *u, int nf, int rt);
void launch_mask_uv(pomgpu_ctx *c);
void launch_mask_w(pomgpu_ctx *c);
void launch_restore(pomgpu_ctx *c, double fold, double fnew);
void launch_restore_shift(pomgpu_ctx *c);
void launch_restore_load(pomgpu_ctx *c, const double *tr, const double *sr, double tau, const double *taur = NULL, int fill_tau = 1);
void launch_dens(pomgpu_ctx *c, const double *si, const double *ti, double *rhoo);
void launch_realvertvl(pomgpu_ctx *c, int etf_is_et = 0);
void launch_baropg(pomgpu_ctx *c, int sum2d);
void launch_baropg_mcc(pomgpu_ctx *c, int sum2d);
void launch_order_pack(pomgpu_ctx *c, double *send_e, double *send_n);
void launch_int_uvmean(pomgpu_ctx *c);
void launch_vertvl(pomgpu_ctx *c, int mask);
void launch_profq_bc(pomgpu_ctx *c);
void launch_profq_prod(pomgpu_ctx *c, int lines_only, int rho_rt = 0);
void launch_profq(pomgpu_ctx *c, int fuse_prod, int fuse_filter, int rho_rt = 0, int jfirst = 0, int jlast = -1, int store_ld = 1);
void launch_proft(pomgpu_ctx *c, double *f, const double *wfsurf, const double *fsurf, int nbc);
int launch_proft2(pomgpu_ctx *c, double *f0, const double *wfsurf0, const double *fsurf0, int nbc0, double *f1, const double *wfsurf1, const double *fsurf1, int nbc1);
void launch_advu_profu(pomgpu_ctx *c, int do_adv, int do_prof);
void launch_advv_profv(pomgpu_ctx *c, int do_adv, int do_prof);
void launch_uv_filter(pomgpu_ctx *c, int own = 0);
void launch_coef_static(pomgpu_ctx *c);
void launch_coef_dt(pomgpu_ctx *c);
void launch_coef_eta(pomgpu_ctx *c, int uvm = 0);
void launch_advt2_rows(pomgpu_ctx *c, const double *fb, const double *f, const double *fc, double *ff);
void launch_advq_col(pomgpu_ctx *c, const double *q, const double *qb, double *qf, int zero_else);
void launch_bcond4_edges(pomgpu_ctx *c);
void launch_bcond6_edges(pomgpu_ctx *c);
void launch_bcondorl3(pomgpu_ctx *c);
struct TrEdge { double *ff; const double *f, *be, *bw, *bn, *bs; };
void launch_tr_edges(pomgpu_ctx *c, const TrEdge *e, int nf);
void launch_tr_source(pomgpu_ctx *c, double *ff, const double *fb, const double *fc, const double *q, double lam);
int launch_halo_pack(pomgpu_ctx *c, double *const *dev, const int *nz, int count, int dir, double *to_lo, double *to_hi);
int launch_halo_pack8(pomgpu_ctx *c, double *const *dev, const int *nz, int count, double *const *to);
int launch_halo_unpack8(pomgpu_ctx *c, double *const *dev, const int *nz, int count, const double *const *from);
int launch_halo_unpack(pomgpu_ctx *c, double *const *dev, const int *nz, int count, int dir, const double *from_lo, const double *from_hi);
void launch_rect_jobs(pomgpu_ctx *c, const RectJob *jobs_dev, int njobs, int max_ni, int max_nj);
int pomgpu_tp_move(pomgpu_ctx *c, const size_t *scount, const size_t *rcount);
int pomgpu_tp_move_ptr(pomgpu_ctx *c, const double *const *send, const size_t *scount, double *const *recv, const size_t *rcount);
int pomgpu_tp_setup(pomgpu_ctx *c, const int *nbr8);
int pomgpu_tp_rccl(pomgpu_ctx *c, const void *id128, int rank, int nranks, const char *librccl_path);
void pomgpu_tp_free(pomgpu_ctx *c);
int pomgpu_tp_reserve(pomgpu_ctx *c, const size_t *need);
int pomgpu_tp_reserve2(pomgpu_ctx *c, const size_t *need);
void pomgpu_wr_materialize(pomgpu_ctx *c);
int pomgpu_materialize(pomgpu_ctx *c);
void pomgpu_mirrors_written(pomgpu_ctx *c);
void pomgpu_cold_tail(pomgpu_ctx *c, void (*update_initial)(pomgpu_ctx *), void (*sums)(pomgpu_ctx *));
int pomgpu_side_stream(pomgpu_ctx *c);
int pomgpu_tp_side_ok(pomgpu_ctx *c);
int pomgpu_tp_move_side(pomgpu_ctx *c, const size_t *scount, const size_t *rcount);
int pomgpu_ff_has(pomgpu_ctx *c, int src);
int pomgpu_ff_fetch_surface(pomgpu_ctx *c, int kind, int n);
int pomgpu_ff_fetch_lateral(pomgpu_ctx *c, int n);
int pomgpu_ff_fetch_restore(pomgpu_ctx *c, int n);
int pomgpu_ff_has_water(pomgpu_ctx *c);
int pomgpu_ff_fetch_water(pomgpu_ctx *c, int n);
int pomgpu_ff_rate_steady(pomgpu_ctx *c);
int pomgpu_ff_rate_have(pomgpu_ctx *c, int n);
int pomgpu_ff_fetch_rate(pomgpu_ctx *c, int n);
static inline void pomgpu_tau_touched(pomgpu_ctx *c, int which) {
  c->tau_known[which] = 0; c->tau_id[which] = 0; c->tau_same = 0;
  if (which) c->rate_in_f = 0;
}
void pomgpu_ff_free(pomgpu_ctx *c);
int launch_ztosig(pomgpu_ctx *c, double *t, const double *zs, int ks, const double *src);
void launch_ztosig_edges(pomgpu_ctx *c, double *t);
int launch_ztosig_line(pomgpu_ctx *c, int edge, const double *zs, int ks, const double *src, double *out);
void launch_mean_accum(pomgpu_ctx *c, const double *const *x);
void launch_probe_gpow15(pomgpu_ctx *c, long n, const double *x, double *out);
void launch_probe_divi(pomgpu_ctx *c, long n, const double *a, const double *b, double *out, int f32);
void launch_probe_rad_q(pomgpu_ctx *c, long n, const double *const *in, double *out);
void launch_check_velocity(pomgpu_ctx *c);
void launch_domain_stats(pomgpu_ctx *c, double *out_dev);
```

Baseline: 4.781 billion.

## Track per-cell roundtrip-change flags to skip clim/rmean loads in ts_update and profq

The advection column kernel now computes, for each cell, whether the (x-y)+y roundtrip against the climatology changes t or s. It packs these into ballot bitmasks stored in a new rt_words buffer. ts_update reads one bit per cell and loads tclim/sclim only where the roundtrip matters. Likewise baropg records per column whether any rho roundtrip against rmean changes bits, and profq uses that to skip loading rmean for unaffected columns. The cost is extra ballot and stores in the producers, a flag load in the consumers, and more state whose validity must be invalidated correctly.

```diff
diff --git a/extpom_amd/csrc/k_adv.hip b/extpom_amd/csrc/k_adv.hip
--- a/extpom_amd/csrc/k_adv.hip
+++ b/extpom_amd/csrc/k_adv.hip
@@ -392,14 +392,14 @@
 }
 
 __device__ __forceinline__ double dens_point(const KP &P, double si, double ti, int i, int j, int k);
-template <int TAU> __device__ __forceinline__ void c_ts_update(const KP &P, const int i, const int j, const int k, double fold, double fnew, int rt, int store_rst, double tau_b, double tau_f);
-template <int TAU> __global__ void k_ts_update(KP P, double fold, double fnew, int rt, int store_rst, double tau_b, double tau_f) {
-  MARCH3(c_ts_update<TAU>(P, i, j, k, fold, fnew, rt, store_rst, tau_b, tau_f))
-}
-__global__ void k_ts_update_same(KP P, double fold, double fnew, int rt, int store_rst) {
-  MARCH3(c_ts_update<2>(P, i, j, k, fold, fnew, rt, store_rst, 0., 0.))
-}
-template <int TAU> __device__ __forceinline__ void c_ts_update(const KP &P, const int i, const int j, const int k, double fold, double fnew, int rt, int store_rst, double tau_b, double tau_f) {
+template <int TAU> __device__ __forceinline__ void c_ts_update(const KP &P, const int i, const int j, const int k, double fold, double fnew, int rt, int store_rst, double tau_b, double tau_f, const unsigned long long *rtf);
+template <int TAU> __global__ void k_ts_update(KP P, double fold, double fnew, int rt, int store_rst, double tau_b, double tau_f, const unsigned long long *rtf) {
+  MARCH3(c_ts_update<TAU>(P, i, j, k, fold, fnew, rt, store_rst, tau_b, tau_f, rtf))
+}
+__global__ void k_ts_update_same(KP P, double fold, double fnew, int rt, int store_rst, const unsigned long long *rtf) {
+  MARCH3(c_ts_update<2>(P, i, j, k, fold, fnew, rt, store_rst, 0., 0., rtf))
+}
+template <int TAU> __device__ __forceinline__ void c_ts_update(const KP &P, const int i, const int j, const int k, double fold, double fnew, int rt, int store_rst, double tau_b, double tau_f, const unsigned long long *rtf) {
   const bool act = (i <= P.im && j <= P.jm), lev = (k <= P.kbm1);
   const pomgpu_ct m = F2(fsm, i, j);
   pomgpu_ct uf = F3(uf, i, j, k), vf = F3(vf, i, j, k);
@@ -408,7 +408,9 @@
     vf = vf * m;
   }
   pomgpu_ct tb = F3(tb, i, j, k), sb = F3(sb, i, j, k);
-  if (rt) {
+  bool rtc = rt != 0;
+  if (rtc && rtf && lev) rtc = ((rtf[RT_WORD(P, i, j, k)] >> RT_BIT(i)) & 1ull) != 0;
+  if (rtc) {
     const pomgpu_ct tc = F3(tclim, i, j, k), sc = F3(sclim, i, j, k);
     tb = (tb - tc) + tc;
     sb = (sb - sc) + sc;
@@ -879,13 +881,18 @@
 void launch_smol(pomgpu_ctx *c, const double *ff) { LAUNCH(c, k_smol, gridm(c->P), blk2(), c->P, ff); }
 void launch_copy3(pomgpu_ctx *c, double *dst, const double *src) { LAUNCH(c, k_copy3, gridm(c->P), blk2(), c->P, dst, src); }
 void launch_advt2_diff(pomgpu_ctx *c, const double *fb, const double *fc, double *ff) { LAUNCH(c, k_advt2_diff, gridm(c->P), blk2(), c->P, fb, fc, ff); }
-void launch_ts_update(pomgpu_ctx *c, double fold, double fnew, int rt, int store_rst) {
+void launch_ts_update(pomgpu_ctx *c, double fold, double fnew, int rt, int store_rst, int rt_flags) {
+  const unsigned long long *rtf = (rt && rt_flags) ? c->rt_words : NULL;
+  if (rtf && c->prof_on) {
+    const int s = pomgpu_prof_slot(c, "ts_rt_flags");
+    if (s >= 0) (c->parent ? c->parent : c)->prof[s].launches++;
+  }
   if (c->tau_known[0] && c->tau_known[1] && !c->tau_handed && !SW(c, TAU_ARRAYS))
-    LAUNCHN(c, "k_ts_update", (k_ts_update<1>), gridm(c->P), blk2(), c->P, fold, fnew, rt, store_rst, c->tau_val[0], c->tau_val[1]);
+    LAUNCHN(c, "k_ts_update", (k_ts_update<1>), gridm(c->P), blk2(), c->P, fold, fnew, rt, store_rst, c->tau_val[0], c->tau_val[1], rtf);
   else if (c->tau_same && !c->tau_handed && !SW(c, TAU_ARRAYS))
-    LAUNCH(c, k_ts_update_same, gridm(c->P), blk2(), c->P, fold, fnew, rt, store_rst);
+    LAUNCH(c, k_ts_update_same, gridm(c->P), blk2(), c->P, fold, fnew, rt, store_rst, rtf);
   else
-    LAUNCHN(c, "k_ts_update", (k_ts_update<0>), gridm(c->P), blk2(), c->P, fold, fnew, rt, store_rst, 0., 0.);
+    LAUNCHN(c, "k_ts_update", (k_ts_update<0>), gridm(c->P), blk2(), c->P, fold, fnew, rt, store_rst, 0., 0., rtf);
 }
 void launch_restore_fields(pomgpu_ctx *c, double fold, double fnew) { LAUNCH(c, k_restore_fields, gridm(c->P), blk2(), c->P, fold, fnew); }
 void launch_mask_ts(pomgpu_ctx *c) { LAUNCH(c, k_mask_ts, gridm(c->P), blk2(), c->P); }
diff --git a/extpom_amd/csrc/k_tile.hip b/extpom_amd/csrc/k_tile.hip
--- a/extpom_amd/csrc/k_tile.hip
+++ b/extpom_amd/csrc/k_tile.hip
@@ -55,7 +55,7 @@
   return CT(0.5) * ((m + fabs(m)) * lo + (m - fabs(m)) * hi);
 }
 struct FaceT { pomgpu_ct adv, dif; };
-struct TFields { const double *fb[2], *f[2], *fcl[2]; double *ff[2]; };
+struct TFields { const double *fb[2], *f[2], *fcl[2]; double *ff[2]; unsigned long long *rtf; };
 template <int NF> struct LevT { pomgpu_ct c[2 * NF + 2], o[2], h[ROWSHARE_SLOTS(2 * NF + 2)]; };
 template <int NS> struct NbrT { pomgpu_ct s[NS], n[NS]; };
 struct CoefT { pomgpu_ct cm, hs, msk, ds_num; InvDc den; };
@@ -76,7 +76,7 @@
 #if COL_WX != 1
 #error "the row-sharing column kernels keep one wavefront per workgroup row (COL_WX == 1)"
 #endif
-template <int NF, bool UM = false>
+template <int NF, bool UM = false, bool RTF = false>
 __global__ void __launch_bounds__(64 * LDS_ROWS) k_advt2_col(KP P, TFields A) {
   constexpr int NS = 2 * NF + 2, NH = ROWSHARE_SLOTS(NS), AM = 2 * NF, VV = 2 * NF + 1;
   HALO_XCD_DECODE_R(LDS_ROWS)
@@ -112,6 +112,9 @@
   for (int q = 0; q < NH; q++) mh[q] = UM ? rowshare_uvm<1, NS, LDS_ROWS>(P, S, q, VV, j0w, i) : uvm_none();
   const unsigned oc = BOFF2(i, jc), lvb = LVB;
   const unsigned ost = in ? oc : BOFF_NONE;
+  const int rt_nbx = RT_NBX(P);
+  const BufA brtf = buf2_of((const double *)A.rtf, RTF ? (size_t)P.kbm1 * P.jml * rt_nbx : 0);
+  const unsigned ortf = (RTF && jrow && lane == 0) ? (unsigned)((jc - 1) * rt_nbx + (i0 - lane) / 62) * 8u : BOFF_NONE, lvrtf = (unsigned)(P.jml * rt_nbx) * 8u;
 #ifndef POMGPU_EMU
   __shared__ pomgpu_ct slab[2][NS][ROWSHARE_ROWS][64];
 #else
@@ -153,6 +156,21 @@
     const pomgpu_ct am_w = halo_w(am_c, [&] { return F3(aam, iw, jc, L); });
     InvDc dzk; dzk.b = dzk.y = 0.;
     if (L >= 2) { dzk.b = F1(dz, L - 1); dzk.y = R1(dz, L - 1); }
+    if constexpr (RTF) {
+      bool ch = false;
+#pragma unroll
+      for (int f = 0; f < NF; f++) ch = ch || rt_changes(cur.c[f], cur.c[NF + f]);
+      const unsigned lvw = (unsigned)WAVE_UNIFORM(L - 1) * lvrtf;
+#ifndef POMGPU_EMU
+      bst2u(brtf, L <= kbm1 ? ortf : BOFF_NONE, lvw, __ballot(icol && ch));
+#else
+      if (L <= kbm1) {
+        unsigned long long &wd = A.rtf[RT_WORD(P, i, jc, L)];
+        wd = (lane == 1 ? 0ull : wd) | ((unsigned long long)ch << lane);
+      }
+      (void)brtf; (void)ortf; (void)lvw;
+#endif
+    }
 #pragma unroll
     for (int f = 0; f < NF; f++) {
       const pomgpu_ct fb_c = cur.c[f], fc_c = cur.c[NF + f];
@@ -829,7 +847,7 @@
 }
 void launch_advt2_rows(pomgpu_ctx *c, const double *fb, const double *f, const double *fc, double *ff) {
   {
-    TFields A; A.fb[0] = A.fb[1] = fb; A.f[0] = A.f[1] = f; A.fcl[0] = A.fcl[1] = fc; A.ff[0] = A.ff[1] = ff;
+    TFields A; A.fb[0] = A.fb[1] = fb; A.f[0] = A.f[1] = f; A.fcl[0] = A.fcl[1] = fc; A.ff[0] = A.ff[1] = ff; A.rtf = NULL;
 #if POMGPU_UVM_ONLOAD
     if (c->P.uvm) { LAUNCHN(c, "k_advt2_col", (k_advt2_col<1, true>), grid1_halo_r(c->P, LDS_ROWS), blk_col_r(LDS_ROWS), c->P, A); return; }
 #endif
@@ -837,8 +855,15 @@
   }
 }
 void launch_advt2x2_col(pomgpu_ctx *c, const double *tb, const double *t, const double *tc, double *tf, const double *sb, const double *s_,
-                        const double *sc, double *sf) {
-  TFields A; A.fb[0] = tb; A.f[0] = t; A.fcl[0] = tc; A.ff[0] = tf; A.fb[1] = sb; A.f[1] = s_; A.fcl[1] = sc; A.ff[1] = sf;
+                        const double *sc, double *sf, unsigned long long *rtf) {
+  TFields A; A.fb[0] = tb; A.f[0] = t; A.fcl[0] = tc; A.ff[0] = tf; A.fb[1] = sb; A.f[1] = s_; A.fcl[1] = sc; A.ff[1] = sf; A.rtf = rtf;
+  if (rtf) {
+#if POMGPU_UVM_ONLOAD
+    if (c->P.uvm) { LAUNCHN(c, "k_advt2x2_col", (k_advt2_col<2, true, true>), grid1_halo_r(c->P, LDS_ROWS), blk_col_r(LDS_ROWS), c->P, A); return; }
+#endif
+    LAUNCHN(c, "k_advt2x2_col", (k_advt2_col<2, false, true>), grid1_halo_r(c->P, LDS_ROWS), blk_col_r(LDS_ROWS), c->P, A);
+    return;
+  }
 #if POMGPU_UVM_ONLOAD
   if (c->P.uvm) { LAUNCHN(c, "k_advt2x2_col", (k_advt2_col<2, true>), grid1_halo_r(c->P, LDS_ROWS), blk_col_r(LDS_ROWS), c->P, A); return; }
 #endif
diff --git a/extpom_amd/csrc/k_vert.hip b/extpom_amd/csrc/k_vert.hip
--- a/extpom_amd/csrc/k_vert.hip
+++ b/extpom_amd/csrc/k_vert.hip
@@ -79,7 +79,7 @@
 #define BPG_ROWS 16
 #endif
 static_assert(COL_WX == 1, "k_baropg_rs / k_vertvl_rs take threadIdx.y as the row inside the workgroup: one wavefront per workgroup row");
-__global__ void __launch_bounds__(64 * BPG_ROWS) k_baropg_rs(KP P, int sum2d) {
+__global__ void __launch_bounds__(64 * BPG_ROWS) k_baropg_rs(KP P, int sum2d, unsigned *rtcol) {
   HALO_XCD_DECODE_R(BPG_ROWS)
   const int r = WAVE_UNIFORM((int)threadIdx.y);
   const bool jvalid = j <= P.jml;
@@ -112,10 +112,12 @@
     L.rho_s = bld(brho, osh, lv); L.rm_s = bld(brm, osh, lv);
   };
   double rc0 = 0., rw0 = 0., rs0 = 0., ax = 0., ay = 0., rx = 0., ry = 0.;
+  bool rtch = false;
   auto step = [&](const int k, const Lev &cur, Lev &nxt) {
     const int par = k & 1;
     load(nxt, k + 2 <= kbm1 ? k + 2 : kbm1);
     const double rc = cur.rho - cur.rm;
+    rtch = rtch || rt_changes(cur.rho, cur.rm);
 #ifndef POMGPU_EMU
     slab[par][r + 1][lane] = rc;
     if (r == 0) slab[par][0][lane] = cur.rho_s - cur.rm_s;
@@ -154,6 +156,7 @@
     if (k + 2 <= kbm1) step(k + 2, rc_, rb);
   }
   if (!own) return;
+  if (rtcol) rtcol[(size_t)(jc - 1) * P.iml + (i - 1)] = rtch ? 1u : 0u;
   if (in) {
     if (sum2d) { F2(drx2d, i, jc) = rx; F2(dry2d, i, jc) = ry; }
     F3(drhox, i, jc, P.kb) = P.ramp * F3(drhox, i, jc, P.kb);
@@ -462,7 +465,7 @@
 #define PROFQ_BIG 8
 #endif
 template <int FP, int FF, int ROWS, int LD = 1>
-__global__ void __launch_bounds__(64 * ROWS) k_profq(KP P, int rho_rt_pace, int jfirst, int jlast) {
+__global__ void __launch_bounds__(64 * ROWS) k_profq(KP P, int rho_rt_pace, int jfirst, int jlast, const unsigned *rtcol) {
 #ifndef POMGPU_EMU
   constexpr int KL = ROWS >= 8 ? PROFQ_KL : (PROFQ_KL < 9 ? PROFQ_KL : 9);
   __shared__ double evec[2 * KL][ROWS][64];
@@ -524,7 +527,8 @@
   const unsigned o_abs = ffil ? BOFF_NONE : oc;
   const unsigned o_fil = ffil ? oc : BOFF_NONE, o_uv = ffil ? BOFF_NONE : oc;
   const unsigned o_pr = (FP == 0 || (FP == 2 && !pin)) ? oc : BOFF_NONE;
-  const unsigned o_rm = rho_rt ? oc : BOFF_NONE;
+  unsigned o_rm = rho_rt ? oc : BOFF_NONE;
+  if (rho_rt_pace & 4) o_rm = (rho_rt && rtcol[(size_t)(j - 1) * P.iml + (i - 1)]) ? oc : BOFF_NONE;
 #ifdef PROFQ_OLDWALK
   const double vbot = P.kappa * (1 + F1(z, kbm1)) * dh * F3(q2, i, j, kbm1);
   const double ufbot = F3(uf, i, j, kb);
@@ -554,7 +558,7 @@
     const unsigned lv = (unsigned)WAVE_UNIFORM(k - 1) * lvb;
     const double kqp = cur.kq1;
     double cck = 0., rhok = 0.;
-    if (k <= kbm1) { cck = profq_cc_v(P, cur.t, cur.s, hij, k); rhok = rho_rt ? (cur.rho - cur.rm) + cur.rm : cur.rho; }
+    if (k <= kbm1) { cck = profq_cc_v(P, cur.t, cur.s, hij, k); rhok = (o_rm != BOFF_NONE) ? (cur.rho - cur.rm) + cur.rm : cur.rho; }
     double q2b = cur.q2b;
     double l, gh = 0.;
     double uck = 0., uek = 0., vck = 0., vnk = 0., bg = 0.;
@@ -674,7 +678,7 @@
     const unsigned lv = (unsigned)WAVE_UNIFORM(k - 1) * lvb;
     const double kqp = cur.kq1;
     double cck = 0., rhok = 0.;
-    if (PH != PH_KB) { cck = profq_cc_v(P, cur.t, cur.s, hij, k); rhok = rho_rt ? (cur.rho - cur.rm) + cur.rm : cur.rho; }
+    if (PH != PH_KB) { cck = profq_cc_v(P, cur.t, cur.s, hij, k); rhok = (o_rm != BOFF_NONE) ? (cur.rho - cur.rm) + cur.rm : cur.rho; }
     double q2b = cur.q2b;
     double l, gh = 0.;
     double uck = 0., uek = 0., vck = 0., vnk = 0., bg = 0.;
@@ -1645,9 +1649,10 @@
 static inline dim3 colgrid(const KP &P) { return dim3((P.iml + 63) / 64, (P.jml + 1) / 2, 1); }
 #define COLV_G(P) dim3(((P).iml + 63) / 64, ((P).jml + 3) / 4, 1)
 #define COLV_B dim3(64, 4, 1)
-void launch_baropg(pomgpu_ctx *c, int sum2d) {
-  if (SW(c, BAROPG_CELLS)) { LAUNCH(c, k_baropg, COLV_G(c->P), COLV_B, c->P, sum2d); return; }
-  LAUNCHN(c, "k_baropg", k_baropg_rs, grid1_halo_r(c->P, BPG_ROWS), blk_col_r(BPG_ROWS), c->P, sum2d);
+int launch_baropg(pomgpu_ctx *c, int sum2d, unsigned *rtcol) {
+  if (SW(c, BAROPG_CELLS)) { LAUNCH(c, k_baropg, COLV_G(c->P), COLV_B, c->P, sum2d); return 0; }
+  LAUNCHN(c, "k_baropg", k_baropg_rs, grid1_halo_r(c->P, BPG_ROWS), blk_col_r(BPG_ROWS), c->P, sum2d, rtcol);
+  return rtcol != NULL;
 }
 void launch_baropg_mcc(pomgpu_ctx *c, int sum2d) { LAUNCH(c, k_baropg_mcc, colgrid(c->P), colblk(), c->P, sum2d); }
 void launch_order_pack(pomgpu_ctx *c, double *send_e, double *send_n) {
@@ -1690,11 +1695,16 @@
   }
   const int nrows = jlast - jfirst + 1;
   const int rows8 = !SW(c, PROFQ_ROWS2) && (SW(c, PROFQ_ROWS8) || (long)((c->P.iml + 63) / 64) * ((c->P.jml + 7) / 8) >= 3 * 256);
-  rho_rt = (rho_rt ? 1 : 0) | (SW(c, PROFQ_NOPACE) ? 0 : 2);
+  const int cols = rho_rt && c->rho_rt_cols && !SW(c, RT_LOAD);
+  if (cols && c->prof_on) {
+    const int s = pomgpu_prof_slot(c, "profq_rm_flags");
+    if (s >= 0) (c->parent ? c->parent : c)->prof[s].launches++;
+  }
+  rho_rt = (rho_rt ? 1 : 0) | (SW(c, PROFQ_NOPACE) ? 0 : 2) | (cols ? 4 : 0);
 #define PQ(FP, FF, LD)                                                                                                                   \
   do {                                                                                                                                   \
-    if (rows8) LAUNCHN(c, "k_profq", (k_profq<FP, FF, PROFQ_BIG, LD>), dim3((c->P.iml + 63) / 64, (nrows + PROFQ_BIG - 1) / PROFQ_BIG, 1), dim3(64, PROFQ_BIG, 1), c->P, rho_rt, jfirst, jlast); \
-    else LAUNCHN(c, "k_profq", (k_profq<FP, FF, 2, LD>), dim3((c->P.iml + 63) / 64, (nrows + 1) / 2, 1), dim3(64, 2, 1), c->P, rho_rt, jfirst, jlast);       \
+    if (rows8) LAUNCHN(c, "k_profq", (k_profq<FP, FF, PROFQ_BIG, LD>), dim3((c->P.iml + 63) / 64, (nrows + PROFQ_BIG - 1) / PROFQ_BIG, 1), dim3(64, PROFQ_BIG, 1), c->P, rho_rt, jfirst, jlast, c->rt_cols); \
+    else LAUNCHN(c, "k_profq", (k_profq<FP, FF, 2, LD>), dim3((c->P.iml + 63) / 64, (nrows + 1) / 2, 1), dim3(64, 2, 1), c->P, rho_rt, jfirst, jlast, c->rt_cols); \
   } while (0)
   if (fuse_filter) { if (fuse_prod == 0) PQ(0, 1, 1); else if (fuse_prod == 1) { if (ld) PQ(1, 1, 1); else PQ(1, 1, 0); } else PQ(2, 1, 1); }
   else { if (fuse_prod == 0) PQ(0, 0, 1); else if (fuse_prod == 1) PQ(1, 0, 1); else PQ(2, 0, 1); }
diff --git a/extpom_amd/csrc/pomgpu_api.hip b/extpom_amd/csrc/pomgpu_api.hip
--- a/extpom_amd/csrc/pomgpu_api.hip
+++ b/extpom_amd/csrc/pomgpu_api.hip
@@ -207,7 +207,7 @@
 }
 static void rho_materialize(pomgpu_ctx *c) {
   if (!c->rho_rt_pending || (c->flags & POMGPU_CTX_2D)) return;
-  c->rho_rt_pending = 0;
+  c->rho_rt_pending = c->rho_rt_cols = 0;
   launch_roundtrip(c, SLOT3(c, P3_rho), SLOT3(c, P3_rmean), 2);
 }
 static void side_join(pomgpu_ctx *c);
@@ -239,6 +239,7 @@
          (k.mode == 4 || (k.nadv == 2 && c->P.nitera == 1 && !SW(c, ADVT2_SINGLE))) &&
          (!c->ntr || (k.nadv == 2 && c->P.nitera == 1));
 }
+static bool rt_one_tile(const pomgpu_ctx *c) { return !c->exch && !c->tp.on && !c->wide.on && !c->parent && !(c->flags & POMGPU_CTX_2D) && !c->wr_eager; }
 static bool ld_on_demand(const pomgpu_ctx *c) {
   return !c->exch && !c->tp.on && !c->wide.on && !c->parent && !(c->flags & POMGPU_CTX_2D) && !c->wr_eager && !SW(c, LD_EAGER);
 }
@@ -347,6 +348,10 @@
   for (int n = 0; n < POMGPU_NSCR3 && !only2d; n++) alloc(&P.s3[n], P.n3);
   for (int n = 0; n < POMGPU_NSCR2; n++) alloc(&P.s2[n], P.n2);
   for (int n = 0; n < 2 && !only2d; n++) alloc(&c->uvb_bot[n], P.n2);
+  if (!only2d) {
+    double *m = NULL; alloc(&m, (size_t)(P.kb > 1 ? P.kb - 1 : 1) * P.jml * RT_NBX(P)); c->rt_words = (unsigned long long *)m;
+    m = NULL; alloc(&m, (P.n2 + 1) / 2); c->rt_cols = (unsigned *)m;
+  }
   for (int n = 0; n < POMGPU_NCOEF2; n++) alloc(&P.c2[n], P.n2);
   alloc(&c->alt2[0], (size_t)POMGPU_NGEN * P.n2);
   for (int n = 1; n < POMGPU_NGEN && ok; n++) c->alt2[n] = c->alt2[0] + (size_t)n * P.n2;
@@ -402,6 +407,7 @@
   for (int n = 0; n < POMGPU_NSCR3; n++) (void)hipFree(P.s3[n]);
   for (int n = 0; n < POMGPU_NSCR2; n++) (void)hipFree(P.s2[n]);
   (void)hipFree(c->uvb_bot[0]); (void)hipFree(c->uvb_bot[1]);
+  (void)hipFree(c->rt_words); (void)hipFree(c->rt_cols);
   for (int n = 0; n < POMGPU_NCOEF2; n++) (void)hipFree(P.c2[n]);
   (void)hipFree(c->alt2[0]); (void)hipFree(c->alt3[0]);
   (void)hipFree(P.m8);
@@ -752,17 +758,18 @@
   launch_advct_c(c);
   xch(c, 1, D3(c, advy), P.kb);
 }
-static void seq_rho_roundtrip(pomgpu_ctx *c, int defer_rt) {
+static void seq_rho_roundtrip(pomgpu_ctx *c, int defer_rt, int cols = 0) {
   if (defer_rt) {
     launch_roundtrip_level(c, D3(c, rho), D3(c, rmean), c->P.kb);
     c->rho_rt_pending = 1;
+    c->rho_rt_cols = cols;
   } else {
     launch_roundtrip(c, D3(c, rho), D3(c, rmean), 0);
   }
 }
 static void seq_baropg(pomgpu_ctx *c, int sum2d = 0, int defer_rt = 0) {
-  launch_baropg(c, sum2d);
-  seq_rho_roundtrip(c, defer_rt);
+  const int cols = launch_baropg(c, sum2d, (defer_rt && rt_one_tile(c)) ? c->rt_cols : NULL);
+  seq_rho_roundtrip(c, defer_rt, cols);
 }
 static void seq_baropg_mcc(pomgpu_ctx *c, int sum2d = 0, int defer_rt = 0) {
   KP &P = c->P;
@@ -972,6 +979,7 @@
 }
 void pomgpu_mirrors_written(pomgpu_ctx *c) {
   c->uvm_valid = 0;
+  c->rho_rt_cols = 0;
   c->wide.static_done = 0;
   early_invalidate(c);
   refresh_coefs(c);
@@ -1624,12 +1632,14 @@
     }
     side_wait(c, SIDE_RW);
     if (k.mode != 4) {
+      bool ts_flags = false;
       if (k.nadv == 1) {
         seq_advt1(c, D3(c, tb), D3(c, t), D3(c, tclim), D3(c, uf));
         seq_advt1(c, D3(c, sb), D3(c, s), D3(c, sclim), D3(c, vf));
       } else if (k.nadv == 2) {
         if (P.nitera == 1 && !SW(c, ADVT2_SINGLE)) {
-          launch_advt2x2_col(c, D3(c, tb), D3(c, t), D3(c, tclim), D3(c, uf), D3(c, sb), D3(c, s), D3(c, sclim), D3(c, vf));
+          ts_flags = rt_one_tile(c);
+          launch_advt2x2_col(c, D3(c, tb), D3(c, t), D3(c, tclim), D3(c, uf), D3(c, sb), D3(c, s), D3(c, sclim), D3(c, vf), ts_flags ? c->rt_words : NULL);
           if (!lib_x) xch(c, 1, D3(c, uf), P.kbm1);
           if (!lib_x) xch(c, 1, D3(c, vf), P.kbm1);
           launch_copy_kb(c, D3(c, tb), D3(c, sb));
@@ -1651,8 +1661,8 @@
       double fold, fnew;
       int rc = restore_prepare(c, &fold, &fnew);
       if (rc) return rc;
-      launch_ts_update(c, fold, fnew, k.nadv == 2, 0);
-      c->rho_rt_pending = 0;
+      launch_ts_update(c, fold, fnew, k.nadv == 2, 0, ts_flags && !SW(c, RT_LOAD));
+      c->rho_rt_pending = c->rho_rt_cols = 0;
       c->rst_pending = 1; c->rst_fold = fold; c->rst_fnew = fnew;
       if (rts) {
         double *at[5] = {D3(c, t), D3(c, tb), D3(c, s), D3(c, sb), D3(c, rho)};
diff --git a/extpom_amd/csrc/pomgpu_internal.hpp b/extpom_amd/csrc/pomgpu_internal.hpp
--- a/extpom_amd/csrc/pomgpu_internal.hpp
+++ b/extpom_amd/csrc/pomgpu_internal.hpp
@@ -289,6 +289,32 @@
 static inline BufA buf2_of(const double *p, size_t) { BufA b; b.p = (double *)p; return b; }
 static inline double bld2(const BufA &b, unsigned voff, unsigned soff) { return voff >= 0xFFFFFFF0u ? 0. : b.p[((size_t)voff + soff) >> 3]; }
 static inline void bst2(const BufA &b, unsigned voff, unsigned soff, double x) { if (voff < 0xFFFFFFF0u) b.p[((size_t)voff + soff) >> 3] = x; }
+#endif
+#define RT_NBX(P) (((P).iml + 61) / 62)
+#define RT_WORD(P, i, j, k) ((size_t)((k) - 1) * (P).jml * RT_NBX(P) + (size_t)((j) - 1) * RT_NBX(P) + (size_t)(((i) - 1) / 62))
+#define RT_BIT(i) (((i) - 1) % 62 + 1)
+__device__ __forceinline__ bool rt_changes(double x, double y) {
+  const double rt = (x - y) + y;
+#ifndef POMGPU_EMU
+  return __double_as_longlong(rt) != __double_as_longlong(x);
+#else
+  return memcmp(&rt, &x, sizeof x) != 0;
+#endif
+}
+__device__ __forceinline__ bool rt_changes(float x, float y) {
+  const float rt = (x - y) + y;
+#ifndef POMGPU_EMU
+  return __float_as_uint(rt) != __float_as_uint(x);
+#else
+  return memcmp(&rt, &x, sizeof x) != 0;
+#endif
+}
+#ifndef POMGPU_EMU
+__device__ __forceinline__ void bst2u(const BufA &b, unsigned voff, unsigned soff, unsigned long long x) {
+  pomgpu_u32x2 v;
+  v.x = (unsigned)x; v.y = (unsigned)(x >> 32);
+  __builtin_amdgcn_raw_buffer_store_b64(v, b.r, (int)voff, (int)soff, 0);
+}
 #endif
 #define BOFF_NONE 0xFFFFFFF0u
 #define BUF3(p) buf_of((p), P.n3)
@@ -432,7 +458,7 @@
   X(PROFQ_NOPACE) X(COL_STRIP) X(BAND_BYTES) X(PAD3) X(IO_SYNC) X(ADVCT_SPLIT) X(ADVQ_EXCHANGE) X(PROD_FULL) X(QFILTER_SPLIT) \
   X(NO_OVERLAP) X(NO_SIDE_COMM) X(WR_MAIN) X(WIDE_W) X(WIDE_FULL) X(DEBUG_ALLOC) X(TEST_SPLIT_FAIL_RANK)  \
   X(WR_NODEFER) X(EXT_RING_FIRST) X(TUNE_FORCE) X(RIM_MAIN) X(RIM_RESULTS_MAIN) X(SUM2D_OFF) X(ADVCT_ROWS4) X(ADVCT_ROWS8) \
-  X(IO_CHUNK_KB) X(UV_NOFUSE) X(W_NOFUSE) X(UVMEAN_PASS) X(PROFT_TWIN) X(LD_EAGER) X(TR_NOPAIR)
+  X(IO_CHUNK_KB) X(UV_NOFUSE) X(W_NOFUSE) X(UVMEAN_PASS) X(PROFT_TWIN) X(LD_EAGER) X(TR_NOPAIR) X(RT_LOAD)
 enum pomgpu_sw {
 #define POMGPU_SW_(name) SW_##name,
   POMGPU_SWITCHES(POMGPU_SW_)
@@ -543,6 +569,9 @@
   long tau_id[2], tau_gen;
   int tau_same, rate_in_f, tau_handed;
   int rho_rt_pending;
+  unsigned long long *rt_words;
+  unsigned *rt_cols;
+  int rho_rt_cols;
   int rst_pending;
   double rst_fold, rst_fnew;
   int wr_pending;
@@ -659,7 +688,7 @@
 void launch_advct_fix(pomgpu_ctx *c, const double *from_w, const double *from_s);
 void launch_advct_fix2d(pomgpu_ctx *c, int west, int south);
 void launch_advt2x2_col(pomgpu_ctx *c, const double *tb, const double *t, const double *tc, double *tf, const double *sb, const double *s_,
-                        const double *sc, double *sf);
+                        const double *sc, double *sf, unsigned long long *rtf = NULL);
 void launch_advq2_col(pomgpu_ctx *c, const double *q, const double *qb, double *qf, const double *ql, const double *qlb, double *qlf, int zero_else);
 #if POMGPU_W_FUSE
 void launch_advq2w_col(pomgpu_ctx *c, const double *q, const double *qb, double *qf, const double *ql, const double *qlb, double *qlf, int zero_else);
@@ -709,7 +738,7 @@
 void launch_smol(pomgpu_ctx *c, const double *ff);
 void launch_copy3(pomgpu_ctx *c, double *dst, const double *src);
 void launch_advt2_diff(pomgpu_ctx *c, const double *fb, const double *fc, double *ff);
-void launch_ts_update(pomgpu_ctx *c, double fold, double fnew, int rt, int store_rst);
+void launch_ts_update(pomgpu_ctx *c, double fold, double fnew, int rt, int store_rst, int rt_flags = 0);
 void launch_restore_fields(pomgpu_ctx *c, double fold, double fnew);
 void launch_mask_ts(pomgpu_ctx *c);
 struct TrUpd { const double *ff, *fc; double *f, *fb; };
@@ -721,7 +750,7 @@
 void launch_restore_load(pomgpu_ctx *c, const double *tr, const double *sr, double tau, const double *taur = NULL, int fill_tau = 1);
 void launch_dens(pomgpu_ctx *c, const double *si, const double *ti, double *rhoo);
 void launch_realvertvl(pomgpu_ctx *c, int etf_is_et = 0);
-void launch_baropg(pomgpu_ctx *c, int sum2d);
+int launch_baropg(pomgpu_ctx *c, int sum2d, unsigned *rtcol = NULL);
 void launch_baropg_mcc(pomgpu_ctx *c, int sum2d);
 void launch_order_pack(pomgpu_ctx *c, double *send_e, double *send_n);
 void launch_int_uvmean(pomgpu_ctx *c);
```

Measured after the change: 4.859 billion (median of 6 runs). +1.6%, better.
